# PINTO0309/human-instance-segmentation

Measured on AMD Instinct MI355X. Metric: ROI-masks/sec (fwd) + train step/s, B0 640×480×8-ROI, 1/2/4/8 MI355X, higher is better.
Workload: dtype bf16; 1 GPU; C2: B0 inference 640x480, batch 32/GPU x 8 ROIs/img, ROI 64x48, mask 128x96; global_batch=32, parallelism=dp1 (images sharded, model replicated, no collective), schedule=2-stream pipeline (UNet of step k+1 overlaps head of step k)

## Files before the change

### human-instance-segmentation_amd/csrc/conv_hwc.hip

```cpp
#include "conv_common.h"

namespace hiseg {

#ifndef HISEG_CONV_HWC_MT
#define HISEG_CONV_HWC_MT 3
#endif

typedef unsigned hc_u4 __attribute__((ext_vector_type(4)));
typedef unsigned hc_u2 __attribute__((ext_vector_type(2)));
typedef __attribute__((address_space(3))) void hc_lds_void;

__device__ __forceinline__ void hc_dma16(__amdgpu_buffer_rsrc_t rsrc, unsigned lds_addr, unsigned voff) {
  asm volatile("s_mov_b32 m0, %0\n\ts_nop 0\n\tbuffer_load_dwordx4 %1, %2, 0 offen lds"
               :: "s"(__builtin_amdgcn_readfirstlane(lds_addr)), "v"(voff), "s"(rsrc) : "memory");
}

template <int ACT, bool RES, int NW, bool UP = false, int ABL = 0, bool RP = false, bool ST = false, int TWB = 1,
          bool BR = false, bool R3 = false>
__global__ void __launch_bounds__(NW * 64, NW == 4 ? 2 : 1) conv_hwc_kernel(ConvArgs a) {
  constexpr int NCG = NW / TWB;
  constexpr int BCO = 32 * NCG, TM = 2, NR = 16;
  constexpr int TW = 16 * TWB, HWD = TW + 2;
  constexpr int NHR = 18 * HWD;
  constexpr int PPW = ((NHR + 15) / 16 + NW - 1) / NW;
  constexpr int PH = (ABL & 512) ? PPW : (PPW + 1) / 2;
  constexpr int PROW = (ABL & 1024) ? 0 : 3;
  constexpr int HB = PPW * NW * 1024;
  constexpr int NPX = 256 * TWB;
  static_assert((NW == 4 || NW == 8) && (TWB == 1 || (TWB == 2 && NW == 4 && !RP)), "configuration");
  static_assert(!R3 || (NW == 4 && !RP && TWB == 1 && !ST && !BR), "R3: the plain / residual 128-Cout form");
  constexpr int NPMIN = ((NHR + 15) / 16 - 1 - (NW - 1)) / NW + 1;
  extern __shared__ __attribute__((aligned(16))) uint4 smem[];
  const hiseg_conv2d_desc& d = a.d;
  const int t = threadIdx.x;
  const int lane = t & 63;
  const int w = __builtin_amdgcn_readfirstlane(t >> 6);
  const int wc = w % NCG, pb = w / NCG;

  const int nco = d.Cout_pad / BCO;
  const int ntx = (d.W + TW - 1) / TW, nty = (d.H + 15) >> 4;
  const int nwg = gridDim.x;
  const int orig = blockIdx.x;
  const int q8 = nwg >> 3, r8 = nwg & 7, xcd = orig & 7, loc = orig >> 3;
  const int wg = (xcd < r8 ? xcd * (q8 + 1) : r8 * (q8 + 1) + (xcd - r8) * q8) + loc;
  const int co0 = (wg % nco) * BCO;
  int tl = wg / nco;
  const int tx = tl % ntx;
  tl /= ntx;
  const int ty = tl % nty;
  const int n = tl / nty;
  const int y0 = ty * 16, x0 = tx * TW;

  const unsigned OOB = 0x80000000u;
  const int nsl = a.Cin >> 5;
  const int ncb = a.Cin >> 6;
  const __amdgpu_buffer_rsrc_t rF = __builtin_amdgcn_make_buffer_rsrc(
      const_cast<void*>(d.weight_frag), (short)0, d.Cout_pad * 9 * a.Cin * 2, 0x00020000);
  constexpr int USH = UP ? 1 : 0;
  const __amdgpu_buffer_rsrc_t rA = __builtin_amdgcn_make_buffer_rsrc(
      const_cast<void*>(d.srcA), (short)0, d.N * (d.H >> USH) * (d.W >> USH) * d.a_cstride * 2, 0x00020000);
  const __amdgpu_buffer_rsrc_t rB = __builtin_amdgcn_make_buffer_rsrc(
      const_cast<void*>(d.Cb ? d.srcB : d.srcA), (short)0, d.Cb ? d.N * d.H * d.W * d.b_cstride * 2 : 0, 0x00020000);

  const unsigned a_ct = (unsigned)((co0 + wc * 32) >> 4) * (unsigned)ncb * 18u * 1024u;
  const unsigned a_ct_step = (unsigned)ncb * 18u * 1024u;
  auto load_blk = [&](hc_u4 (&af)[3][TM], int sl, int kx) __attribute__((always_inline)) {
    int ln = lane;
    asm volatile("" : "+v"(ln));
    const unsigned a_lane = a_ct + (unsigned)ln * 16u;
#pragma unroll
    for (int ky = 0; ky < 3; ++ky) {
      const unsigned so = __builtin_amdgcn_readfirstlane(
          (((unsigned)(sl >> 1) * 9u + (unsigned)(ky * 3 + kx)) * 2u + (unsigned)(sl & 1)) * 1024u);
#pragma unroll
      for (int i = 0; i < TM; ++i)
        af[ky][i] = __builtin_amdgcn_raw_buffer_load_b128(rF, a_lane + (unsigned)i * a_ct_step, so, 0);
    }
  };

  const unsigned lds_base = (unsigned)(uintptr_t)(hc_lds_void*)smem;
  auto hbuf = [&](int sl) __attribute__((always_inline)) -> int {
    if constexpr (RP) return ((nsl - 1 - sl) & 1) ? 32 * 1024 : 56 * 1024;
    else if constexpr (R3) return (sl % 3) * HB;
    else return (sl & 1) * HB;
  };
  auto piece_off = [&](int p, int sl) __attribute__((always_inline)) -> unsigned {
    int ln = lane;
    asm volatile("" : "+v"(ln));
    const int hr = 16 * (NW * p + w) + (ln >> 2);
    const int hy = hr / HWD, hx = hr - HWD * hy;
    const int iy = y0 + hy - 1, ix = x0 + hx - 1;
    const bool ok = hr < NHR && (unsigned)iy < (unsigned)d.H && (unsigned)ix < (unsigned)d.W;
    const int chunk = (ln & 3) ^ (((hx >> 2) & 1) << 1);
    const bool fb = 32 * sl >= d.Ca;
    const int cs = fb ? d.b_cstride : d.a_cstride, coff = fb ? d.b_coff + 32 * sl - d.Ca : d.a_coff + 32 * sl;
    if constexpr (UP) {
      const int ush = fb ? 0 : 1;
      return ok ? (unsigned)((((n * (d.H >> ush) + (iy >> ush)) * (d.W >> ush) + (ix >> ush)) * cs + coff + chunk * 8) * 2)
                : OOB;
    } else {
      return ok ? (unsigned)((((n * d.H + iy) * d.W + ix) * cs + coff + chunk * 8) * 2) : OOB;
    }
  };
  unsigned pofA[PPW];
#pragma unroll
  for (int p = 0; p < PPW; ++p) pofA[p] = 16 * (NW * p + w) < NHR ? piece_off(p, 0) : OOB;
  auto halo_dma = [&](int p, int sl, int boff) __attribute__((always_inline)) {
    if (16 * (NW * p + w) >= NHR) return;
    const bool fb = 32 * sl >= d.Ca;
    const unsigned off = fb ? piece_off(p, sl) : pofA[p] + 64u * (unsigned)sl;
    hc_dma16(fb ? rB : rA, lds_base + (unsigned)(boff + 1024 * (NW * p + w)), off);
  };
  const char* lds_c = reinterpret_cast<const char*>(smem);
// ... 81 lines not shown
#pragma unroll
          for (int k = 8 + 3 * KX; k < 11 + 3 * KX; ++k) res_dma(k);
        }
      }
      if constexpr (RP && RES) {
        if (sl == 0) {
#pragma unroll
          for (int k = 3 * KX; k < (KX == 2 ? 8 : 3 * KX + 3); ++k) res_dma(k);
        }
      }
    };
    int ln = lane;
    asm volatile("" : "+v"(ln));
    hc_u4 bq[3];
    if constexpr ((ABL & 4) == 0) {
      bq[0] = rdB(ln, buf, KX, 0);
      bq[1] = rdB(ln, buf, KX, 1);
    } else {
      bq[0] = bq[1] = bq[2] = af[0][0];
    }
    __builtin_amdgcn_s_setprio(1);
#pragma unroll
    for (int r = 0; r < NR + 2; ++r) {
      if (r == PROW) {
        __builtin_amdgcn_s_setprio(0);
        pieces();
        __builtin_amdgcn_s_setprio(1);
      }
      if ((ABL & 4) == 0 && r + 2 < NR + 2) bq[(r + 2) % 3] = rdB(ln, buf, KX, r + 2);
      __builtin_amdgcn_sched_barrier(0);
#pragma unroll
      for (int ky = 0; ky < 3; ++ky) {
        const int j = r - ky;
        if (j >= 0 && j < NR) {
#pragma unroll
          for (int i = 0; i < TM; ++i) {
            if constexpr ((ABL & 16) == 0)
              acc[i][j] = __builtin_amdgcn_mfma_f32_16x16x32_bf16(__builtin_bit_cast(bf16x8_t, af[ky][i]),
                                                                   __builtin_bit_cast(bf16x8_t, bq[r % 3]), acc[i][j], 0,
                                                                   0, 0);
            else
              acc[i][j][0] += __builtin_bit_cast(float, af[ky][i][0]) + __builtin_bit_cast(float, bq[r % 3][1]);
          }
        }
      }
    }
    __builtin_amdgcn_s_setprio(0);
    if constexpr (KX == 2 && (ABL & 8) == 0) {
      if constexpr (R3) {
        if (sl + 2 < nsl) asm volatile("s_waitcnt vmcnt(%0)" :: "n"(18 + NPMIN) : "memory");
        else if (more) asm volatile("s_waitcnt vmcnt(6)" ::: "memory");
        else asm volatile("s_waitcnt vmcnt(0)" ::: "memory");
      } else {
        if (more) asm volatile("s_waitcnt vmcnt(6)" ::: "memory");
        else asm volatile("s_waitcnt vmcnt(0)" ::: "memory");
      }
      __syncthreads();
    }
    if constexpr ((ABL & 1) == 0) {
#pragma unroll
      for (int ky = 0; ky < 3; ++ky)
#pragma unroll
        for (int i = 0; i < TM; ++i) af[ky][i] = an[ky][i];
    }
  };
  using K0 = std::integral_constant<int, 0>;
  using K1 = std::integral_constant<int, 1>;
  using K2 = std::integral_constant<int, 2>;
  for (int sl = 0; sl < nsl; ++sl) {
    block(sl, K0{});
    block(sl, K1{});
    block(sl, K2{});
  }

  if constexpr ((ABL & 32) != 0) {
    float* o = reinterpret_cast<float*>(d.out) + (long long)wg * 64 * 64 * NW + t;
#pragma unroll
    for (int i = 0; i < TM; ++i)
#pragma unroll
      for (int j = 0; j < NR; ++j) o[(i * NR + j) * 64 * NW] = acc[i][j][0] + acc[i][j][1] + acc[i][j][2] + acc[i][j][3];
    return;
  }
  char* tile = reinterpret_cast<char*>(smem);
  if constexpr (RES && !RP) {
#pragma unroll
    for (int k = 0; k < NRI; ++k) res_dma(k);
    asm volatile("s_waitcnt vmcnt(0)" ::: "memory");
    __syncthreads();
  } else if constexpr (RES) {
    res_dma(14);
    res_dma(15);
  }
  constexpr int NSTZ = NPX * CPR / (NW * 64);
  uint4 zpre[BR ? NSTZ : 1];
  if constexpr (BR) {
#pragma unroll
    for (int k = 0; k < NSTZ; ++k) {
      const int idx = t + NW * 64 * k;
      const int r = idx / CPR, c = idx % CPR;
      const int px = px_of(r), co = co0 + 8 * c;
      zpre[k] = (px >= 0 && co < d.Cout)
                    ? *reinterpret_cast<const uint4*>(reinterpret_cast<const uint16_t*>(d.bnb_z) +
                                                      (long long)px * d.bnb_z_cstride + d.bnb_z_coff + co)
                    : make_uint4(0u, 0u, 0u, 0u);
    }
  }
  floatx4 sc[TM], sh[TM];
#pragma unroll
  for (int i = 0; i < TM; ++i) {
    const int cl = wc * 32 + i * 16 + (lane >> 4) * 4;
    const int cc = co0 + cl < d.Cout ? co0 + cl : 0;
    sc[i] = *reinterpret_cast<const floatx4*>(d.scale + cc);
    sh[i] = *reinterpret_cast<const floatx4*>(d.shift + cc);
  }
  auto convert = [&](auto j0c, auto j1c) __attribute__((always_inline)) {
    constexpr int J0 = decltype(j0c)::value, J1 = decltype(j1c)::value;
#pragma unroll
    for (int i = 0; i < TM; ++i)
#pragma unroll
      for (int j = J0; j < J1; ++j) {
        const int cl = wc * 32 + i * 16 + (lane >> 4) * 4;
        const int r = j * TW + 16 * pb + (lane & 15);
        char* q = tile + r * EROWB + ((((cl >> 3) ^ (r & SWM)) << 4) | ((cl & 4) << 1));
        const floatx4 ac = acc[i][j];
        float v[4];
        uint2 rv = make_uint2(0u, 0u);
        if constexpr (RES) rv = *reinterpret_cast<const uint2*>(q);
#pragma unroll
        for (int e = 0; e < 4; ++e) {
          v[e] = ac[e] * sc[i][e] + sh[i][e];
          if constexpr (RES) v[e] += Quad<bf16_t>::get(rv, e);
          if constexpr (ACT == HISEG_ACT_RELU) v[e] = v[e] > 0.f ? v[e] : 0.f;
        }
        uint2 o;
        o.x = f2bf2(v[0], v[1]);
        o.y = f2bf2(v[2], v[3]);
        *reinterpret_cast<uint2*>(q) = o;
      }
  };
  if constexpr (RES && RP) {
    convert(std::integral_constant<int, 0>{}, std::integral_constant<int, 14>{});
    asm volatile("s_waitcnt vmcnt(0)" ::: "memory");
    __syncthreads();
    convert(std::integral_constant<int, 14>{}, std::integral_constant<int, NR>{});
  } else {
    convert(std::integral_constant<int, 0>{}, std::integral_constant<int, NR>{});
  }
  __syncthreads();
  constexpr int NST = NPX * CPR / (NW * 64);
  float sk[8], s1[8], s2[8];
  int sn = 0;
  float bfs[8], bfh[8], bmu[8], binv[8];
  if constexpr (BR) {
    static_assert(!RES && !ST && ACT == HISEG_ACT_NONE && NW == 4 && (CPR == 16 || CPR == 8), "fused BN backward");
    const int cb = co0 + 8 * (t % CPR);
#pragma unroll
    for (int e = 0; e < 8; ++e) {
      const int ch = cb + e < d.Cout ? cb + e : 0;
      bfs[e] = d.bnb_scale[ch];
      bfh[e] = d.bnb_shift[ch];
      bmu[e] = d.bnb_mean[ch];
      binv[e] = d.bnb_invstd[ch];
      sk[e] = s1[e] = s2[e] = 0.f;
    }
  }
  if constexpr (ST) {
    static_assert(!RES && ACT == HISEG_ACT_NONE && NW == 4, "fused statistics: the conv feeding a BatchNorm");
    static_assert(CPR == 16 || CPR == 8, "fused statistics: a wave's threads of one chunk are lanes CPR apart");
#pragma unroll
    for (int e = 0; e < 8; ++e) sk[e] = s1[e] = s2[e] = 0.f;
  }
  uint4 sv[NST];
#pragma unroll
  for (int k = 0; k < NST; ++k) {
    const int idx = t + NW * 64 * k;
    const int r = idx / CPR, c = idx % CPR;
    sv[k] = *reinterpret_cast<const uint4*>(tile + r * EROWB + ((c ^ (r & SWM)) << 4));
  }
  const __amdgpu_buffer_rsrc_t rO = __builtin_amdgcn_make_buffer_rsrc(d.out, (short)0, 0x7fffffff, 0x00020000);
#pragma unroll
  for (int k = 0; k < NST; ++k) {
    const int idx = t + NW * 64 * k;
    const int r = idx / CPR, c = idx % CPR;
    const int px = px_of(r), co = co0 + 8 * c;
    const uint4 v = sv[k];
    __builtin_amdgcn_raw_buffer_store_b128(
        __builtin_bit_cast(hc_u4, v), rO,
        (px >= 0 && co < d.Cout) ? (unsigned)((px * d.o_cstride + d.o_coff + co) * 2) : OOB, 0, 0);
    if constexpr (BR) {
      if (px >= 0 && co < d.Cout) {
        const uint4 zq = zpre[BR ? k : 0];
        const unsigned wv[4] = {v.x, v.y, v.z, v.w}, zw[4] = {zq.x, zq.y, zq.z, zq.w};
#pragma unroll
        for (int e = 0; e < 8; ++e) {
          const float g0 = __builtin_bit_cast(float, (e & 1) ? (wv[e >> 1] & 0xffff0000u) : (wv[e >> 1] << 16));
          const float zf = __builtin_bit_cast(float, (e & 1) ? (zw[e >> 1] & 0xffff0000u) : (zw[e >> 1] << 16));
          const float g = (d.bnb_act == HISEG_ACT_RELU && !(zf * bfs[e] + bfh[e] > 0.f)) ? 0.f : g0;
          const float xh = (zf - bmu[e]) * binv[e];
          sk[e] += g;
          s1[e] = fmaf(g, xh, s1[e]);
          s2[e] += xh;
        }
      }
    }
    if constexpr (ST) {
      if (px >= 0) {
        const unsigned wv[4] = {v.x, v.y, v.z, v.w};
#pragma unroll
        for (int e = 0; e < 8; ++e) {
          const float x = __builtin_bit_cast(float, (e & 1) ? (wv[e >> 1] & 0xffff0000u) : (wv[e >> 1] << 16));
          if (sn == 0) sk[e] = x;
          const float dx = x - sk[e];
          s1[e] += dx;
          s2[e] = fmaf(dx, dx, s2[e]);
        }
        ++sn;
      }
    }
  }
  if constexpr (ST) {
    float nn = (float)sn, mu[8], q2[8];
#pragma unroll
    for (int e = 0; e < 8; ++e) {
      mu[e] = sn ? sk[e] + s1[e] / nn : 0.f;
      q2[e] = sn ? fmaxf(s2[e] - s1[e] * s1[e] / nn, 0.f) : 0.f;
    }
#pragma unroll
    for (int m = CPR; m < 64; m <<= 1) {
      const float nb = __shfl_xor(nn, m, 64);
      const float nt = nn + nb;
      const float fb = nt > 0.f ? nb / nt : 0.f, fab = nt > 0.f ? nn * nb / nt : 0.f;
#pragma unroll
      for (int e = 0; e < 8; ++e) {
        const float mb = __shfl_xor(mu[e], m, 64), qb = __shfl_xor(q2[e], m, 64);
        const float dd = mb - mu[e];
        mu[e] += dd * fb;
        q2[e] += qb + dd * dd * fab;
      }
      nn = nt;
    }
    if (lane < CPR) {
      const long long C = d.Cout;
      float* part = a.d.stats_partial + ((long long)((n * nty + ty) * ntx + tx) * NW + w) * 3 * C;
#pragma unroll
      for (int e = 0; e < 8; ++e) {
        const int ch = co0 + 8 * lane + e;
        part[ch] = nn;
        part[C + ch] = mu[e];
        part[2 * C + ch] = q2[e];
      }
    }
  }
  if constexpr (BR) {
#pragma unroll
    for (int m = CPR; m < 64; m <<= 1) {
#pragma unroll
      for (int e = 0; e < 8; ++e) {
        sk[e] += __shfl_xor(sk[e], m, 64);
        s1[e] += __shfl_xor(s1[e], m, 64);
        s2[e] += __shfl_xor(s2[e], m, 64);
      }
    }
    if (lane < CPR) {
      const long long C = d.Cout;
      float* part = a.d.bnb_partial + ((long long)((n * nty + ty) * ntx + tx) * NW + w) * 3 * C;
#pragma unroll
      for (int e = 0; e < 8; ++e) {
        const int ch = co0 + 8 * lane + e;
        if (ch < C) {
          part[ch] = sk[e];
          part[C + ch] = s1[e];
          part[2 * C + ch] = s2[e];
        }
      }
    }
  }
}

template <int ACT, bool RES, int NW, bool UP = false, int ABL = 0, bool RP = false, bool ST = false, int TWB = 1,
          bool BR = false, bool R3 = false>
static int launch_hwc(const ConvArgs& a, hipStream_t s) {
  const hiseg_conv2d_desc& d = a.d;
  constexpr int BCO = 32 * NW / TWB, TW = 16 * TWB;
  constexpr int PPW = ((18 * (TW + 2) + 15) / 16 + NW - 1) / NW;
  constexpr size_t halo2 = (size_t)2 * PPW * NW * 1024, epi = (size_t)256 * TWB * BCO * 2;
  const int tiles = d.N * ((d.H + 15) / 16) * ((d.W + TW - 1) / TW);
  const int nco = d.Cout_pad / BCO;
  const size_t halo = R3 ? halo2 / 2 * 3 : halo2;
  const size_t lds = RP ? (size_t)80 * 1024 : (halo > epi ? halo : epi);
  auto kern = conv_hwc_kernel<ACT, RES, NW, UP, ABL, RP, ST, TWB, BR, R3>;
  static bool attr = false;
  if (!attr) {
    (void)hipFuncSetAttribute((const void*)kern, hipFuncAttributeMaxDynamicSharedMemorySize, (int)lds);
    attr = true;
  }
  hipLaunchKernelGGL(kern, dim3(tiles * nco), dim3(NW * 64), lds, s, a);
  return hiseg_check_launch("conv_hwc");
}

template <int ACT, bool RES, int TWB, int MT>
__global__ void __launch_bounds__(256, 2) conv_hwc_mt_kernel(ConvArgs a) {
  constexpr int NW = 4, NCG = NW / TWB;
  constexpr int BCO = 32 * NCG, TM = 2, NR = 16;
  constexpr int TW = 16 * TWB, HWD = TW + 2;
  constexpr int NHR = 18 * HWD;
  constexpr int PPW = ((NHR + 15) / 16 + NW - 1) / NW;
  constexpr int PH = (PPW + 1) / 2;
  constexpr int HB = PPW * NW * 1024;
  constexpr int NPX = 256 * TWB, HALF = NPX / 2;
  constexpr int EOFF = HB;
  static_assert(MT >= 2 && (TWB == 1 || TWB == 2), "multi-tile configuration");
  extern __shared__ __attribute__((aligned(16))) uint4 smem[];
  const hiseg_conv2d_desc& d = a.d;
  const int t = threadIdx.x;
  const int lane = t & 63;
  const int w = __builtin_amdgcn_readfirstlane(t >> 6);
  const int wc = w % NCG, pb = w / NCG;

  const int nco = d.Cout_pad / BCO;
  const int ntx = (d.W + TW - 1) / TW, nty = (d.H + 15) >> 4;
  const int total = d.N * nty * ntx * nco;
  const int G = gridDim.x;
  const int orig = blockIdx.x;
  const int q8 = G >> 3, r8 = G & 7, xcd = orig & 7, loc = orig >> 3;
  const int wg = (xcd < r8 ? xcd * (q8 + 1) : r8 * (q8 + 1) + (xcd - r8) * q8) + loc;

  const unsigned OOB = 0x80000000u;
  const int nsl = a.Cin >> 5;
  const int ncb = a.Cin >> 6;
  const __amdgpu_buffer_rsrc_t rF = __builtin_amdgcn_make_buffer_rsrc(
      const_cast<void*>(d.weight_frag), (short)0, d.Cout_pad * 9 * a.Cin * 2, 0x00020000);
  const __amdgpu_buffer_rsrc_t rA = __builtin_amdgcn_make_buffer_rsrc(
      const_cast<void*>(d.srcA), (short)0, d.N * d.H * d.W * d.a_cstride * 2, 0x00020000);
  const __amdgpu_buffer_rsrc_t rB = __builtin_amdgcn_make_buffer_rsrc(
      const_cast<void*>(d.Cb ? d.srcB : d.srcA), (short)0, d.Cb ? d.N * d.H * d.W * d.b_cstride * 2 : 0, 0x00020000);
  const unsigned a_ct_step = (unsigned)ncb * 18u * 1024u;

  struct Geo { int co0, n, y0, x0; unsigned a_ct; };
  auto geo = [&](int i) __attribute__((always_inline)) -> Geo {
    Geo g;
    g.co0 = (i % nco) * BCO;
    int tl = i / nco;
    g.x0 = (tl % ntx) * TW;
    tl /= ntx;
    g.y0 = (tl % nty) * 16;
    g.n = tl / nty;
    g.a_ct = (unsigned)((g.co0 + wc * 32) >> 4) * (unsigned)ncb * 18u * 1024u;
    return g;
  };
  auto load_blk = [&](hc_u4 (&af)[3][TM], unsigned a_ct, int sl, int kx) __attribute__((always_inline)) {
    int ln = lane;
    asm volatile("" : "+v"(ln));
    const unsigned a_lane = a_ct + (unsigned)ln * 16u;
#pragma unroll
    for (int ky = 0; ky < 3; ++ky) {
      const unsigned so = __builtin_amdgcn_readfirstlane(
          (((unsigned)(sl >> 1) * 9u + (unsigned)(ky * 3 + kx)) * 2u + (unsigned)(sl & 1)) * 1024u);
#pragma unroll
      for (int i = 0; i < TM; ++i)
        af[ky][i] = __builtin_amdgcn_raw_buffer_load_b128(rF, a_lane + (unsigned)i * a_ct_step, so, 0);
    }
  };
  auto piece_off = [&](const Geo& g, int p, int sl) __attribute__((always_inline)) -> unsigned {
    int ln = lane;
    asm volatile("" : "+v"(ln));
    const int hr = 16 * (NW * p + w) + (ln >> 2);
    const int hy = hr / HWD, hx = hr - HWD * hy;
    const int iy = g.y0 + hy - 1, ix = g.x0 + hx - 1;
    const bool ok = hr < NHR && (unsigned)iy < (unsigned)d.H && (unsigned)ix < (unsigned)d.W;
    const int chunk = (ln & 3) ^ (((hx >> 2) & 1) << 1);
    const bool fb = 32 * sl >= d.Ca;
    const int cs = fb ? d.b_cstride : d.a_cstride, coff = fb ? d.b_coff + 32 * sl - d.Ca : d.a_coff + 32 * sl;
    return ok ? (unsigned)((((g.n * d.H + iy) * d.W + ix) * cs + coff + chunk * 8) * 2) : OOB;
// ... 203 lines not shown
#pragma unroll
    for (int i = 0; i < TM; ++i)
#pragma unroll
      for (int j = 0; j < NR; ++j) acc[i][j] = floatx4{0.f, 0.f, 0.f, 0.f};
  }
}

template <int ACT, bool RES, int TWB, int MT>
static int launch_hwc_mt(const ConvArgs& a, hipStream_t s) {
  const hiseg_conv2d_desc& d = a.d;
  constexpr int BCO = 128 / TWB, TW = 16 * TWB;
  constexpr int PPW = ((18 * (TW + 2) + 15) / 16 + 3) / 4;
  constexpr size_t hb = (size_t)PPW * 4 * 1024;
  constexpr size_t lds = 2 * hb > hb + 32 * 1024 ? 2 * hb : hb + 32 * 1024;
  const long long items = (long long)d.N * ((d.H + 15) / 16) * ((d.W + TW - 1) / TW) * (d.Cout_pad / BCO);
  const int grid = (int)((items + MT - 1) / MT);
  auto kern = conv_hwc_mt_kernel<ACT, RES, TWB, MT>;
  static bool attr = false;
  if (!attr) {
    (void)hipFuncSetAttribute((const void*)kern, hipFuncAttributeMaxDynamicSharedMemorySize, (int)lds);
    attr = true;
  }
  hipLaunchKernelGGL(kern, dim3(grid), dim3(256), lds, s, a);
  return hiseg_check_launch("conv_hwc_mt");
}

template <int TWB, int MT>
static int launch_hwc_mt_act(const ConvArgs& a, hipStream_t s) {
  const bool res = a.d.residual != nullptr, relu = a.d.act == HISEG_ACT_RELU;
  return res ? (relu ? launch_hwc_mt<HISEG_ACT_RELU, true, TWB, MT>(a, s) : launch_hwc_mt<HISEG_ACT_NONE, true, TWB, MT>(a, s))
             : (relu ? launch_hwc_mt<HISEG_ACT_RELU, false, TWB, MT>(a, s)
                     : launch_hwc_mt<HISEG_ACT_NONE, false, TWB, MT>(a, s));
}

template <int NW, bool RP = false, int TWB = 1, bool R3 = false>
static int launch_hwc_nw(const ConvArgs& a, hipStream_t s) {
  const hiseg_conv2d_desc& d = a.d;
  if (d.a_up == 2)
    return launch_hwc<HISEG_ACT_RELU, false, NW, true, 0, false, false, TWB, false, R3>(a, s);
  const bool res = d.residual != nullptr, relu = d.act == HISEG_ACT_RELU;
  return res ? (relu ? launch_hwc<HISEG_ACT_RELU, true, NW, false, 0, RP, false, TWB, false, R3>(a, s)
                     : launch_hwc<HISEG_ACT_NONE, true, NW, false, 0, RP, false, TWB, false, R3>(a, s))
             : (relu ? launch_hwc<HISEG_ACT_RELU, false, NW, false, 0, false, false, TWB, false, R3>(a, s)
                     : launch_hwc<HISEG_ACT_NONE, false, NW, false, 0, false, false, TWB, false, R3>(a, s));
}

static bool conv_hwc_applies(const ConvArgs& a, int variant) {
  const hiseg_conv2d_desc& d = a.d;
  if (((variant < 104 || variant > 109) && variant != 102) || d.weight_frag == nullptr) return false;
  if ((variant == 109 || variant == 102) && (d.a_up != 1 || d.stats_partial || d.bnb_partial)) return false;
  if (d.dtype != HISEG_BF16 || d.out_dtype != HISEG_BF16) return false;
  if ((d.a_up != 1 && d.a_up != 2) || d.in_scale != nullptr || d.convT || d.mul != nullptr || d.out2 != nullptr)
    return false;
  if (d.KH != 3 || d.KW != 3 || d.stride != 1 || d.pad != 1 || d.Ho != d.H || d.Wo != d.W) return false;
  if (d.act != HISEG_ACT_NONE && d.act != HISEG_ACT_RELU) return false;
  if (d.Ca % 32 != 0 || d.Cb % 32 != 0 || (d.Ca + d.Cb) % 64 != 0 || d.Ca < 64 || d.K_pad != 9 * (d.Ca + d.Cb))
    return false;
  if ((d.a_cstride | d.a_coff) & 7) return false;
  if (d.Cb && (d.srcB == nullptr || ((d.b_cstride | d.b_coff) & 7))) return false;
  if ((d.Cout & (variant == 105 ? 255 : (variant == 107 || variant == 102) ? 63 : 127)) || d.Cout_pad != d.Cout ||
      ((d.o_cstride | d.o_coff) & 7) ||
      (d.residual && ((d.r_cstride | d.r_coff) & 7)))
    return false;
  if ((((uintptr_t)d.scale | (uintptr_t)d.shift | (uintptr_t)d.out | (uintptr_t)d.residual |
        (uintptr_t)d.weight_frag) & 15))
    return false;
  const long long span_a = (long long)d.N * (d.H / d.a_up) * (d.W / d.a_up) * d.a_cstride * 2;
  const long long span_b = d.Cb ? (long long)d.N * d.H * d.W * d.b_cstride * 2 : 0;
  const long long span_w = (long long)d.Cout_pad * d.K_pad * 2;
  const long long span_r = d.residual ? (long long)a.M * d.r_cstride * 2 : 0;
  const long long span_o = (long long)a.M * d.o_cstride * 2;
  if (span_a >= 0x7fffffffll || span_b >= 0x7fffffffll || span_w >= 0x7fffffffll || span_r >= 0x7fffffffll ||
      span_o >= 0x7fffffffll)
    return false;
  if ((long long)d.N * d.H * d.W >= (1ll << 29)) return false;
  if (d.a_up == 2 && (d.residual || d.act != (d.stats_partial ? HISEG_ACT_NONE : HISEG_ACT_RELU))) return false;
  if (d.stats_partial && ((variant != 104 && variant != 107) || d.residual || d.act != HISEG_ACT_NONE)) return false;
  if (d.bnb_partial &&
      ((variant != 104 && variant != 107) || d.residual || d.act != HISEG_ACT_NONE || d.stats_partial || d.a_up != 1 ||
       d.bnb_z == nullptr || ((d.bnb_z_cstride | d.bnb_z_coff) & 7) || ((uintptr_t)d.bnb_z & 15) ||
       !d.bnb_scale || !d.bnb_shift || !d.bnb_mean || !d.bnb_invstd ||
       (d.bnb_act != HISEG_ACT_RELU && d.bnb_act != HISEG_ACT_NONE)))
    return false;
  return true;
}

int conv_hwc_stats_tiles(const ConvArgs& a) {
  ConvArgs b = a;
  float dummy;
  if (b.d.bnb_partial == nullptr) b.d.stats_partial = &dummy;
  const int tw = conv_hwc_applies(b, 104) ? 16 : conv_hwc_applies(b, 107) ? 32 : 0;
  if (tw == 0) return 0;
  return a.d.N * ((a.d.H + 15) / 16) * ((a.d.W + tw - 1) / tw) * 4;
}

int conv_hwc_try(const ConvArgs& a, hipStream_t s, int variant) {
  const hiseg_conv2d_desc& d = a.d;
#ifdef HISEG_DIAG
  if (variant >= 150 && variant < 4300) {
    if (d.weight_frag == nullptr || !d.residual || d.act != HISEG_ACT_RELU || d.a_up != 1 || d.Cout % 128) return 0;
    int r;
    switch (variant - 150) {
      case 1: r = launch_hwc<HISEG_ACT_RELU, true, 4, false, 1>(a, s); break;
      case 2: r = launch_hwc<HISEG_ACT_RELU, true, 4, false, 2>(a, s); break;
      case 3: r = launch_hwc<HISEG_ACT_RELU, true, 4, false, 3>(a, s); break;
      case 4: r = launch_hwc<HISEG_ACT_RELU, true, 4, false, 4>(a, s); break;
      case 8: r = launch_hwc<HISEG_ACT_RELU, true, 4, false, 8>(a, s); break;
      case 15: r = launch_hwc<HISEG_ACT_RELU, true, 4, false, 15>(a, s); break;
      case 16: r = launch_hwc<HISEG_ACT_RELU, true, 4, false, 16>(a, s); break;
      case 32: r = launch_hwc<HISEG_ACT_RELU, true, 4, false, 32>(a, s); break;
      case 47: r = launch_hwc<HISEG_ACT_RELU, true, 4, false, 47>(a, s); break;
      case 64: r = launch_hwc<HISEG_ACT_RELU, true, 4, false, 64>(a, s); break;
      case 128: r = launch_hwc<HISEG_ACT_RELU, true, 4, false, 128>(a, s); break;
      case 512: r = launch_hwc<HISEG_ACT_RELU, true, 4, false, 512>(a, s); break;
      case 1024: r = launch_hwc<HISEG_ACT_RELU, true, 4, false, 1024>(a, s); break;
      case 1536: r = launch_hwc<HISEG_ACT_RELU, true, 4, false, 1536>(a, s); break;
      case 2048: r = launch_hwc<HISEG_ACT_RELU, true, 4, false, 2048>(a, s); break;
      case 4096: r = launch_hwc<HISEG_ACT_RELU, true, 4, false, 4096>(a, s); break;
      default: return 0;
    }
    return r < 0 ? r : 1;
  }
#endif
  if (!conv_hwc_applies(a, variant)) return 0;
  if (d.bnb_partial) {
    const int r = variant == 107 ? launch_hwc<HISEG_ACT_NONE, false, 4, false, 0, false, false, 2, true>(a, s)
                                 : launch_hwc<HISEG_ACT_NONE, false, 4, false, 0, false, false, 1, true>(a, s);
    return r < 0 ? r : 1;
  }
  if (d.stats_partial) {
    int r;
    if (variant == 107)
      r = d.a_up == 2 ? launch_hwc<HISEG_ACT_NONE, false, 4, true, 0, false, true, 2>(a, s)
                      : launch_hwc<HISEG_ACT_NONE, false, 4, false, 0, false, true, 2>(a, s);
    else
      r = d.a_up == 2 ? launch_hwc<HISEG_ACT_NONE, false, 4, true, 0, false, true>(a, s)
                      : launch_hwc<HISEG_ACT_NONE, false, 4, false, 0, false, true>(a, s);
    return r < 0 ? r : 1;
  }
  const int r = variant == 109 ? launch_hwc_mt_act<1, HISEG_CONV_HWC_MT>(a, s)
              : variant == 102 ? launch_hwc_mt_act<2, HISEG_CONV_HWC_MT>(a, s)
              : variant == 107 ? launch_hwc_nw<4, false, 2>(a, s)
              : variant == 108 ? launch_hwc_nw<4, false, 1, true>(a, s)
              : variant == 105 ? launch_hwc_nw<8>(a, s)
              : variant == 106 ? launch_hwc_nw<4, true>(a, s)
                               : launch_hwc_nw<4>(a, s);
  return r < 0 ? r : 1;
}

}
```

### human-instance-segmentation_amd/csrc/conv_igemm.hip

```cpp
#include <cstdlib>
#include "conv_common.h"

namespace hiseg {

typedef unsigned ig_u4 __attribute__((ext_vector_type(4)));

template <typename T, typename TO, int BCO, int BPX, int WCO, int WPX, bool SPLIT = false, int LIN = 0>
__global__ void __launch_bounds__(256) conv_igemm_kernel(ConvArgs a) {
  constexpr int KCH = Chunk<T>::N;
  constexpr int BK = 8 * KCH;
  constexpr int TM = BCO / (WCO * 16);
  constexpr int TN = BPX / (WPX * 16);
  constexpr int A_CH = (BPX * 8 + 255) / 256;
  constexpr int W_CH = (BCO * 8 + 255) / 256;
  constexpr int STAGE = (BCO + BPX) * 8;
  constexpr bool A_FULL = (BPX * 8) % 256 == 0;
  constexpr bool W_FULL = (BCO * 8) % 256 == 0;
  static_assert(WCO * WPX == 4, "4 waves");
  static_assert(TM >= 1 && TN >= 1, "tile");

  extern __shared__ __attribute__((aligned(16))) uint4 smem[];

  const hiseg_conv2d_desc& d = a.d;
  const int t = threadIdx.x;
// ... 325 lines not shown
        if (r) return r;
        const long long n = (long long)a.M * (a.d.Cout_pad >> 2);
        hipLaunchKernelGGL((conv_splitk_reduce_kernel<T, TO>), dim3((unsigned)((n + 255) / 256)), dim3(256), 0, s, a, splits);
        return hiseg_check_launch("conv_splitk_reduce");
      }
      if (lin == 1) hipLaunchKernelGGL((conv_igemm_kernel<T, TO, BCO, BPX, WCO, WPX, false, 1>), grid, dim3(256), lds, s, a);
      else hipLaunchKernelGGL((conv_igemm_kernel<T, TO, BCO, BPX, WCO, WPX, false, 2>), grid, dim3(256), lds, s, a);
      return hiseg_check_launch("conv_igemm");
    }
  }
  if (splits > 1) {
    hipLaunchKernelGGL((conv_igemm_kernel<T, TO, BCO, BPX, WCO, WPX, true>), grid, dim3(256), lds, s, a);
    const int r = hiseg_check_launch("conv_igemm_splitk");
    if (r) return r;
    const long long n = (long long)a.M * (a.d.Cout_pad >> 2);
    hipLaunchKernelGGL((conv_splitk_reduce_kernel<T, TO>), dim3((unsigned)((n + 255) / 256)), dim3(256), 0, s, a, splits);
    return hiseg_check_launch("conv_splitk_reduce");
  }
  hipLaunchKernelGGL((conv_igemm_kernel<T, TO, BCO, BPX, WCO, WPX>), grid, dim3(256), lds, s, a);
  return hiseg_check_launch("conv_igemm");
}

static int igemm_bco(int cp) {
  auto fits = [&](int bco) { return ((cp + bco - 1) / bco) * bco * 6 <= cp * 7; };
  auto padded = [&](int bco) { return ((cp + bco - 1) / bco) * bco; };
  if (cp >= 96 && fits(128)) return 128;
  if (cp >= 48 && fits(64)) return 64;
  if (cp >= 48) return padded(64) < padded(128) ? 64 : 128;
  if (fits(32)) return 32;
  return 16;
}

static int splitk_bco(int cp) { return cp >= 96 && igemm_bco(cp) == 128 ? 128 : 64; }

template <typename T, typename TO>
static int launch_typed(const ConvArgs& a, hipStream_t s, int splits = 1) {
  static const bool gated_wide = [] { const char* e = getenv("HISEG_GATED_WIDE"); return !(e && atoi(e) == 0); }();
  if (splits > 1 || (gated_wide && a.d.in_scale != nullptr)) {
    if (splitk_bco(a.d.Cout_pad) == 128) return launch_cfg<T, TO, 128, 128, 2, 2>(a, s, splits);
    return launch_cfg<T, TO, 64, 128, 2, 2>(a, s, splits);
  }
  const char* eb = getenv("HISEG_IGEMM_BCO");
  switch (eb ? atoi(eb) : igemm_bco(a.d.Cout_pad)) {
    case 128: return launch_cfg<T, TO, 128, 128, 2, 2>(a, s, splits);
    case 64: return launch_cfg<T, TO, 64, 128, 2, 2>(a, s, splits);
    case 32: return launch_cfg<T, TO, 32, 256, 1, 4>(a, s, splits);
    default: return launch_cfg<T, TO, 16, 256, 1, 4>(a, s, splits);
  }
}

static int splitk_plan(const ConvArgs& a) {
  const hiseg_conv2d_desc& d = a.d;
  if (d.dtype != HISEG_BF16 || d.convT || a.nK < 6) return 1;
  if (d.KH == 3 && d.KW == 3 && d.stride == 1 && d.a_up == 1 && (long long)d.Ho * d.Wo <= 256 && a.nK >= 24 &&
      d.in_scale == nullptr) {
    int sp = a.nK / 4;
    return sp > 8 ? 8 : sp;
  }
  if (d.KH != 1 || d.KW != 1) return 1;
  if (d.in_scale == nullptr && a.nK < 24) return 1;
  static const int forced = [] { const char* e = getenv("HISEG_SPLITK"); return e ? atoi(e) : 0; }();
  if (forced > 0) return forced < a.nK ? forced : a.nK;
  if ((long long)d.Ho * d.Wo > 1600) return 1;
  int sp = a.nK / 4;
  if (sp > 8) sp = 8;
  return sp >= 2 ? sp : 2;
}

static long long splitk_bytes(const ConvArgs& a, int splits) {
  return splits > 1 ? (long long)splits * a.M * a.d.Cout_pad * 4 : 0;
}

}

namespace hiseg {
int conv_fast_try(const ConvArgs& a, hipStream_t s, int variant);
int conv_wide_try(const ConvArgs& a, hipStream_t s, int variant);
int conv_hw_try(const ConvArgs& a, hipStream_t s, int variant);
int conv_pw_try(const ConvArgs& a, hipStream_t s, int variant);
int conv_hwr_try(const ConvArgs& a, hipStream_t s, int variant);
int conv_hwt_try(const ConvArgs& a, hipStream_t s, int variant);
int conv_hwc_try(const ConvArgs& a, hipStream_t s, int variant);
int conv_hwc_stats_tiles(const ConvArgs& a);
int conv_small_try(const ConvArgs& a, hipStream_t s, int variant);
int conv_rows_try(const ConvArgs& a, hipStream_t s, int variant);
bool conv_pw_applies(const ConvArgs& a);
int conv_pw_gate_images(const ConvArgs& a);
bool conv_rows_form(const ConvArgs& a);
}

using namespace hiseg;


static int conv2d_impl(const hiseg_conv2d_desc* d, hiseg_stream_t stream, int variant);

extern "C" int hiseg_conv2d_fwd(const hiseg_conv2d_desc* d, hiseg_stream_t stream) {
  return conv2d_impl(d, stream, 0);
}

static bool hwc64_mode() {
  const char* e = getenv("HISEG_CONV_HWC64");
  return !(e && atoi(e) == 0);
}

static bool hwc_r3_mode() {
  const char* e = getenv("HISEG_CONV_HWC_R3");
  return !(e && atoi(e) == 0);
}

#ifndef HISEG_CONV_HWC_MT_DEFAULT
#define HISEG_CONV_HWC_MT_DEFAULT(bco) false
#endif
static bool hwc_mt_mode(int bco) {
  const char* e = getenv("HISEG_CONV_HWC_MTW");
  if (e) return atoi(e) != 0;
  return HISEG_CONV_HWC_MT_DEFAULT(bco);
}

static bool release_variant(int v) {
  return v == -1 || v == 0 || (v >= 1 && v <= 8) || v == 50 || v == 51 || v == 52 || v == 54 || v == 58 ||
         (v >= 60 && v <= 69) || v == 70 || v == 71 || v == 72 || v == 74 || v == 80 || v == 82 || v == 84 || v == 86 ||
         v == 88 || v == 89 || v == 90 || (v >= 92 && v <= 101) || v == 103 || v == 102 || (v >= 104 && v <= 109);
}

extern "C" long long hiseg_conv2d_workspace_bytes(const hiseg_conv2d_desc* d) {
  if (d == nullptr || d->dtype != HISEG_BF16 || d->convT || d->N <= 0) return 0;
  const long long M = (long long)d->N * d->Ho * d->Wo;
  if (M >= (1ll << 31) || d->K_pad % 64) return 0;
  ConvArgs a;
  a.d = *d;
  a.M = (int)M;
  a.Cin = d->Ca + d->Cb;
  a.nK = d->K_pad / 64;
  a.Hs = d->H / (d->a_up > 0 ? d->a_up : 1);
  a.Ws = d->W / (d->a_up > 0 ? d->a_up : 1);
  if (conv_pw_applies(a)) return 0;
  if (d->in_scale && d->KH == 1 && d->KW == 1 && conv_pw_gate_images(a) > 0) return 0;
  return splitk_bytes(a, splitk_plan(a));
}

extern "C" int hiseg_conv2d_stats_tiles(const hiseg_conv2d_desc* d) {
  if (d == nullptr || d->dtype != HISEG_BF16 || d->convT || d->N <= 0) return 0;
  const long long M = (long long)d->N * d->Ho * d->Wo;
  if (M >= (1ll << 31)) return 0;
  ConvArgs a;
  a.d = *d;
  a.M = (int)M;
  a.Cin = d->Ca + d->Cb;
  a.nK = d->K_pad / 64;
  a.Hs = d->H / (d->a_up > 0 ? d->a_up : 1);
  a.Ws = d->W / (d->a_up > 0 ? d->a_up : 1);
  return conv_hwc_stats_tiles(a);
}

extern "C" int hiseg_conv2d_fwd_variant(const hiseg_conv2d_desc* d, int variant, hiseg_stream_t stream) {
#ifndef HISEG_DIAG
  HISEG_REQUIRE(release_variant(variant), HISEG_ERR_BAD_ARG,
                "conv2d: variant %d is not a release variant (diagnostic kernels need a DIAG=1 build)", variant);
#endif
  return conv2d_impl(d, stream, variant);
}

static int conv2d_impl(const hiseg_conv2d_desc* d, hiseg_stream_t stream, int variant) {
  HISEG_REQUIRE(d != nullptr, HISEG_ERR_BAD_ARG, "conv2d: null descriptor");
  HISEG_REQUIRE(d->dtype == HISEG_F32 || d->dtype == HISEG_BF16, HISEG_ERR_BAD_DTYPE, "conv2d: dtype %d", d->dtype);
  HISEG_REQUIRE(d->out_dtype == HISEG_F32 || d->out_dtype == HISEG_BF16, HISEG_ERR_BAD_DTYPE, "conv2d: out_dtype %d", d->out_dtype);
  HISEG_REQUIRE(d->srcA && d->weight && d->scale && d->shift && d->out, HISEG_ERR_BAD_ARG, "conv2d: null pointer");
  HISEG_REQUIRE(d->N > 0 && d->H > 0 && d->W > 0 && d->Ho > 0 && d->Wo > 0, HISEG_ERR_BAD_SHAPE, "conv2d: empty grid");
  HISEG_REQUIRE(d->KH > 0 && d->KW > 0 && d->stride > 0 && d->pad >= 0, HISEG_ERR_BAD_SHAPE, "conv2d: bad window");
  HISEG_REQUIRE(d->a_up == 1 || d->a_up == 2, HISEG_ERR_BAD_SHAPE, "conv2d: a_up must be 1 or 2");
  HISEG_REQUIRE(d->a_up == 1 || (d->H % 2 == 0 && d->W % 2 == 0), HISEG_ERR_BAD_SHAPE, "conv2d: upsampled grid must be even");
  HISEG_REQUIRE(d->Cb == 0 || d->srcB, HISEG_ERR_BAD_ARG, "conv2d: Cb > 0 needs srcB");
  HISEG_REQUIRE(d->Cout > 0 && d->Cout_pad >= d->Cout && d->Cout_pad % 16 == 0, HISEG_ERR_BAD_SHAPE,
                "conv2d: Cout %d Cout_pad %d (must be multiple of 16)", d->Cout, d->Cout_pad);
  const int kch = d->dtype == HISEG_BF16 ? 8 : 4;
  const int bk = 8 * kch;
  const int Cin = d->Ca + d->Cb;
  HISEG_REQUIRE(d->Ca > 0 && d->Ca % kch == 0 && d->Cb % kch == 0 && d->a_cstride % kch == 0 &&
                    d->a_coff % kch == 0 && (d->Cb == 0 || (d->b_cstride % kch == 0 && d->b_coff % kch == 0)),
                HISEG_ERR_BAD_SHAPE, "conv2d: input channels/strides must be multiples of %d", kch);
  HISEG_REQUIRE(d->K_pad % bk == 0 && d->K_pad >= d->KH * d->KW * Cin, HISEG_ERR_BAD_SHAPE,
                "conv2d: K_pad %d must be a multiple of %d and >= %d", d->K_pad, bk, d->KH * d->KW * Cin);
  HISEG_REQUIRE(al16(d->srcA) && al16(d->srcB) && al16(d->weight), HISEG_ERR_BAD_SHAPE, "conv2d: operands must be 16-B aligned");
  HISEG_REQUIRE(!d->convT || (d->KH == 1 && d->KW == 1 && d->stride == 1 && d->pad == 0 && d->Cout % 16 == 0 &&
                              d->Ho == d->H && d->Wo == d->W),
                HISEG_ERR_BAD_SHAPE, "conv2d: convT requires a 1x1 GEMM with Cout = 4*C, C %% 4 == 0");
  if (d->stats_partial || d->bnb_partial) {
    HISEG_REQUIRE(variant == 0 || variant == 104 || variant == 107, HISEG_ERR_BAD_ARG,
                  "conv2d: stats_partial / bnb_partial with variant %d", variant);
    HISEG_REQUIRE(al16(d->out) && al16(d->scale) && al16(d->shift), HISEG_ERR_BAD_SHAPE, "conv2d: alignment");
    ConvArgs a;
    a.d = *d;
    a.M = (int)((long long)d->N * d->Ho * d->Wo);
    a.Cin = Cin;
    a.nK = d->K_pad / bk;
    a.Hs = d->H / d->a_up;
    a.Ws = d->W / d->a_up;
    HISEG_REQUIRE(conv_hwc_stats_tiles(a) > 0, HISEG_ERR_BAD_ARG,
                  "conv2d: stats_partial / bnb_partial set but the layer has no fused kernel (hiseg_conv2d_stats_tiles)");
    const int r = conv_hwc_try(a, (hipStream_t)stream, d->Cout % 128 == 0 ? 104 : 107);
    HISEG_REQUIRE(r != 0, HISEG_ERR_BAD_ARG, "conv2d: the fused-statistics kernel declined the layer");
    return r < 0 ? r : HISEG_OK;
  }
  {
    const long long ea = d->dtype == HISEG_BF16 ? 2 : 4, eo = d->out_dtype == HISEG_BF16 ? 2 : 4;
    const long long in_px = (long long)(d->H / d->a_up) * (d->W / d->a_up);
    const long long out_px = (long long)d->Ho * d->Wo * (d->convT ? 4 : 1);
    long long per = in_px * d->a_cstride * ea;
    auto upd = [&](long long v) { if (v > per) per = v; };
    if (d->srcB) upd((long long)d->H * d->W * d->b_cstride * ea);
    if (d->residual) upd(out_px * d->r_cstride * ea);
    if (d->mul) upd(out_px * d->m_cstride * ea);
    upd(out_px * d->o_cstride * eo);
    if (d->out2) upd(out_px * d->o2_cstride * ea);
    const long long lim = (1ll << 31) - (1ll << 20);
    int step = 0;
    if (per * d->N > lim) {
      HISEG_REQUIRE(per <= lim, HISEG_ERR_BAD_SHAPE, "conv2d: one image's operand exceeds 2 GiB");
      step = (int)(lim / per);
    }
    if (variant == 0 && d->in_scale && d->dtype == HISEG_BF16 && d->KH == 1 && d->KW == 1) {
      ConvArgs ga;
      ga.d = *d;
      ga.M = (int)((long long)d->N * d->Ho * d->Wo < (1ll << 31) ? (long long)d->N * d->Ho * d->Wo : 0);
      ga.Cin = d->Ca + d->Cb;
      ga.nK = d->K_pad / (8 * kch);
      ga.Hs = d->H / d->a_up;
      ga.Ws = d->W / d->a_up;
      const int g = conv_pw_gate_images(ga);
      if (g > 0 && (step == 0 || g < step)) step = g;
    }
    if (step > 0 && step < d->N) {
      for (int n0 = 0; n0 < d->N; n0 += step) {
        hiseg_conv2d_desc c = *d;
        c.N = d->N - n0 < step ? d->N - n0 : step;
        auto at = [&](const void* p, long long bytes_per_image) {
          return p ? (const void*)((const char*)p + bytes_per_image * n0) : p;
        };
        c.srcA = at(d->srcA, in_px * d->a_cstride * ea);
        c.srcB = at(d->srcB, (long long)d->H * d->W * d->b_cstride * ea);
        c.residual = at(d->residual, out_px * d->r_cstride * ea);
        c.mul = at(d->mul, out_px * d->m_cstride * ea);
        c.out = const_cast<void*>(at(d->out, out_px * d->o_cstride * eo));
        c.out2 = const_cast<void*>(at(d->out2, out_px * d->o2_cstride * ea));
        if (d->in_scale) c.in_scale = d->in_scale + (long long)n0 * d->Ca;
        const int r = conv2d_impl(&c, stream, variant);
        if (r) return r;
      }
      return HISEG_OK;
    }
  }
  const long long M = (long long)d->N * d->Ho * d->Wo;
  HISEG_REQUIRE(M < (1ll << 31), HISEG_ERR_BAD_SHAPE, "conv2d: too many pixels");
  ConvArgs a;
  a.d = *d;
  a.M = (int)M;
  a.Cin = Cin;
  a.nK = d->K_pad / bk;
  a.Hs = d->H / d->a_up;
  a.Ws = d->W / d->a_up;
  hipStream_t s = (hipStream_t)stream;
  a.ins_vec = d->in_scale != nullptr && ((uintptr_t)d->in_scale & 15) == 0 && (d->Ca & 3) == 0;
  a.ws = static_cast<float*>(d->workspace);
  a.kper = a.nK;
  if (variant == 99 || variant == 0) {
    const int sp = splitk_plan(a);
    if (sp > 1 && d->workspace != nullptr && d->workspace_bytes >= splitk_bytes(a, sp) &&
        !(variant == 0 && conv_pw_applies(a))) {
      a.kper = (a.nK + sp - 1) / sp;
      const int spl = (a.nK + a.kper - 1) / a.kper;
      return d->out_dtype == HISEG_BF16 ? launch_typed<bf16_t, bf16_t>(a, s, spl) : launch_typed<bf16_t, float>(a, s, spl);
    }
    HISEG_REQUIRE(variant == 0, HISEG_ERR_BAD_ARG, "conv2d: variant 99 (split-K) does not apply to this layer / workspace");
  }
  if (variant == 98) {
    const int r = conv_rows_try(a, s, variant);
    if (r != 0) return r < 0 ? r : HISEG_OK;
  } else if (variant == 90 || (variant >= 190 && variant < 222)) {
    const int r = conv_pw_try(a, s, variant);
    if (r != 0) return r < 0 ? r : HISEG_OK;
  } else if ((variant >= 92 && variant <= 97) || variant == 100 || variant == 101 || (variant >= 110 && variant < 142)) {
    const int r = conv_hwr_try(a, s, variant);
    if (r != 0) return r < 0 ? r : HISEG_OK;
  } else if (variant == 102 || (variant >= 104 && variant <= 109) || (variant >= 150 && variant < 4300)) {
    const int r = conv_hwc_try(a, s, variant);
    if (r != 0) return r < 0 ? r : HISEG_OK;
  } else if (variant == 103) {
    const int r = conv_hwt_try(a, s, variant);
    if (r != 0) return r < 0 ? r : HISEG_OK;
  } else if (variant >= 80 && variant < 90) {
    const int r = conv_hw_try(a, s, variant);
    if (r != 0) return r < 0 ? r : HISEG_OK;
  } else if (variant >= 70 && variant < 80) {
    const int r = conv_wide_try(a, s, variant);
    if (r != 0) return r < 0 ? r : HISEG_OK;
  } else if (variant >= 60 && variant < 70) {
    const int r = conv_fast_try(a, s, variant);
    if (r != 0) return r < 0 ? r : HISEG_OK;
  } else if (variant >= 50) {
    const int r = conv_small_try(a, s, variant);
    if (r != 0) return r < 0 ? r : HISEG_OK;
  } else if (variant >= 0) {
    int v = variant;
    static const bool four_waves = [] { const char* e = getenv("HISEG_CONV_WAVES"); return e && atoi(e) == 4; }();
    static const bool halo = [] { const char* e = getenv("HISEG_CONV_HALO"); return !(e && atoi(e) == 0); }();
    if (v == 0 && d->KH == 1 && d->KW == 1) {
      const int r = conv_pw_try(a, s, 90);
      if (r != 0) return r < 0 ? r : HISEG_OK;
    }
    if (v == 0 && d->KH == 3 && d->KW == 3 && d->Cout_pad <= 32) {
      const int r = conv_rows_try(a, s, 98);
      if (r != 0) return r < 0 ? r : HISEG_OK;
      if (conv_rows_form(a)) {
        const int r2 = conv_small_try(a, s, 0);
        if (r2 != 0) return r2 < 0 ? r2 : HISEG_OK;
      }
    }
    if (v == 0 && !four_waves && halo && d->weight_frag != nullptr && d->Cout % 128 == 0 && hwc_mt_mode(128)) {
      const int r = conv_hwc_try(a, s, 109);
      if (r != 0) return r < 0 ? r : HISEG_OK;
    }
    if (v == 0 && !four_waves && halo && d->weight_frag != nullptr && d->Cout % 128 == 0) {
      const int r = conv_hwc_try(a, s, hwc_r3_mode() ? 108 : 104);
      if (r != 0) return r < 0 ? r : HISEG_OK;
    }
    if (v == 0 && !four_waves && halo && d->weight_frag != nullptr && d->Cout % 128 == 0) {
      const int r = conv_hwr_try(a, s, 97);
      if (r != 0) return r < 0 ? r : HISEG_OK;
    }
    if (v == 0 && !four_waves && halo && d->weight_frag != nullptr && d->Cout % 64 == 0 && hwc64_mode() &&
        hwc_mt_mode(64)) {
      const int r = conv_hwc_try(a, s, 102);
      if (r != 0) return r < 0 ? r : HISEG_OK;
    }
    if (v == 0 && !four_waves && halo && d->weight_frag != nullptr && d->Cout % 64 == 0 && hwc64_mode()) {
      const int r = conv_hwc_try(a, s, 107);
      if (r != 0) return r < 0 ? r : HISEG_OK;
    }
    if (v == 0 && !four_waves && halo && d->weight_frag != nullptr && d->Cout % 64 == 0) {
      const int r = conv_hwr_try(a, s, 100);
      if (r != 0) return r < 0 ? r : HISEG_OK;
    }
    if (v == 0 && !four_waves && halo) {
      const int r = conv_hw_try(a, s, d->Cout % 128 ? 89 : 86);
      if (r != 0) return r < 0 ? r : HISEG_OK;
    }
    if (v == 0 && d->Cout % 256 == 0 && d->KH * d->KW > 1 && !four_waves) {
// ... 17 lines not shown
```

### human-instance-segmentation_amd/csrc/conv_pw.hip

```cpp
#include "conv_common.h"

#ifndef HISEG_PW_PART
#define HISEG_PW_PART 1
#endif

namespace hiseg {

constexpr int kPwBlk = 32;
constexpr int kPwActRt = -1;

typedef unsigned pw_u4 __attribute__((ext_vector_type(4)));
typedef unsigned pw_u2 __attribute__((ext_vector_type(2)));

template <int NKSA, int EPI, int ACT, bool CONVT, int RB, bool INS>
__global__ void __launch_bounds__(256, 1) conv_pw_kernel(ConvArgs a, int nct, int nks_arg) {
  constexpr int NKS = NKSA < 0 ? -NKSA : NKSA;
  const int nks = NKSA < 0 ? nks_arg : NKSA;
  constexpr bool RES = EPI == 1, MUL = EPI == 2, XOP = EPI != 0;
  constexpr int CT = 16 * RB;
  constexpr int ROWC = NKS * 4 + 1;
  constexpr int NA = NKS == 9 ? 8 : NKS;
  constexpr unsigned OOB = 0x80000000u;
  extern __shared__ __attribute__((aligned(16))) uint4 smem[];
  const hiseg_conv2d_desc& d = a.d;
  const int t = threadIdx.x, lane = t & 63, w = t >> 6;
  const int ct = blockIdx.x % nct;
  const int grp = blockIdx.x / nct, ngrp = gridDim.x / nct;
  const int c0 = ct * CT;
  const int act = ACT == kPwActRt ? d.act : ACT;
#ifdef HISEG_DIAG
  const int abl = a.abl;
#else
  constexpr int abl = 0;
#endif

  uint4* wl = smem;
  float* ssc = reinterpret_cast<float*>(smem + CT * ROWC);
  float* ssh = ssc + CT;
  float* gl = ssh + CT;
  constexpr int kPwStage = 8;
  const int kc = d.K_pad >> 3;
  const int wch = nks * 4;
  const int nchunk = CT * wch;
  {
    const __amdgpu_buffer_rsrc_t rW = __builtin_amdgcn_make_buffer_rsrc(
        const_cast<void*>(d.weight), (short)0, (int)((long long)d.Cout_pad * kc * 16), 0x00020000);
    for (int i0 = t; i0 < ((abl & 1) ? 0 : nchunk); i0 += 256 * kPwStage) {
      pw_u4 v[kPwStage];
#pragma unroll
      for (int u = 0; u < kPwStage; ++u) {
        const int i = i0 + 256 * u;
        const int r = i / wch, c = i - r * wch;
        const unsigned off = i < nchunk ? (unsigned)(((c0 + r) * kc + c) * 16) : 0x80000000u;
        v[u] = __builtin_amdgcn_raw_buffer_load_b128(rW, off, 0, 0);
      }
#pragma unroll
      for (int u = 0; u < kPwStage; ++u) {
        const int i = i0 + 256 * u;
        const int r = i / wch, c = i - r * wch;
        if (i < nchunk) wl[r * ROWC + c] = make_uint4(v[u].x, v[u].y, v[u].z, v[u].w);
      }
    }
  }
  for (int i = t; i < CT; i += 256) {
    const int j = c0 + i < d.Cout ? c0 + i : 0;
    ssc[i] = d.scale[j];
    ssh[i] = d.shift[j];
  }
  if constexpr (INS) {
    const int n4 = d.N * d.Ca / 4;
    const __amdgpu_buffer_rsrc_t rG = __builtin_amdgcn_make_buffer_rsrc(
        const_cast<float*>(d.in_scale), (short)0, (int)(n4 * 16), 0x00020000);
    float4* gl4 = reinterpret_cast<float4*>(gl);
    for (int i0 = t; i0 < n4; i0 += 256 * kPwStage) {
      pw_u4 v[kPwStage];
#pragma unroll
      for (int u = 0; u < kPwStage; ++u) {
        const int i = i0 + 256 * u;
        v[u] = __builtin_amdgcn_raw_buffer_load_b128(rG, i < n4 ? (unsigned)(i * 16) : 0x80000000u, 0, 0);
      }
#pragma unroll
      for (int u = 0; u < kPwStage; ++u) {
        const int i = i0 + 256 * u;
        if (i < n4) gl4[i] = __builtin_bit_cast(float4, v[u]);
      }
    }
  }
  __syncthreads();

  const int M = a.M;
  const int nblk = (M + kPwBlk - 1) / kPwBlk;
  const int g = lane >> 4, pl = lane & 15;
  const long long out_px = (long long)M * (CONVT ? 4 : 1);
  const __amdgpu_buffer_rsrc_t rA = __builtin_amdgcn_make_buffer_rsrc(
      const_cast<void*>(d.srcA), (short)0, (int)((long long)M * d.a_cstride * 2), 0x00020000);
  const __amdgpu_buffer_rsrc_t rB = __builtin_amdgcn_make_buffer_rsrc(
      const_cast<void*>(NKS == 9 ? d.srcB : d.srcA), (short)0, NKS == 9 ? (int)((long long)M * d.b_cstride * 2) : 0,
      0x00020000);
  const __amdgpu_buffer_rsrc_t rO = __builtin_amdgcn_make_buffer_rsrc(d.out, (short)0,
                                                                     (int)(out_px * d.o_cstride * 2), 0x00020000);
  const void* xp = RES ? d.residual : MUL ? d.mul : d.out;
  const int x_cs = RES ? d.r_cstride : d.m_cstride, x_coff = RES ? d.r_coff : d.m_coff;
  const __amdgpu_buffer_rsrc_t rR = __builtin_amdgcn_make_buffer_rsrc(
      const_cast<void*>(xp), (short)0, XOP ? (int)(out_px * x_cs * 2) : 0, 0x00020000);
  const bool bch_ok = NKS == 9 && 8 * g < d.Cb;

  auto load_ks = [&](int b, int ks, uint4 (&bk)[2]) __attribute__((always_inline)) {
    if (abl & 2) {
      bk[0] = bk[1] = make_uint4(0u, 0u, 0u, 0u);
      return;
    }
    const bool ch_ok = 32 * ks + 8 * g < d.Ca;
#pragma unroll
    for (int j = 0; j < 2; ++j) {
      const int p = b * kPwBlk + 16 * j + pl;
      pw_u4 v;
      if (ks < NA) {
        const unsigned off = (p < M && ch_ok) ? (unsigned)((p * d.a_cstride + d.a_coff + 32 * ks + 8 * g) * 2) : OOB;
        v = __builtin_amdgcn_raw_buffer_load_b128(rA, off, 0, 0);
      } else {
        const unsigned off = (p < M && bch_ok) ? (unsigned)((p * d.b_cstride + d.b_coff + 8 * g) * 2) : OOB;
        v = __builtin_amdgcn_raw_buffer_load_b128(rB, off, 0, 0);
      }
      bk[j] = make_uint4(v.x, v.y, v.z, v.w);
    }
  };

  int pbase[2];
  auto set_block = [&](int b) __attribute__((always_inline)) {
#pragma unroll
    for (int j = 0; j < 2; ++j) {
      const int p = b * kPwBlk + 16 * j + pl;
      if constexpr (CONVT) {
        const int x = p % d.Wo, tt = p / d.Wo, y = tt % d.Ho, n = tt / d.Ho;
        pbase[j] = p < M ? (n * (2 * d.Ho) + 2 * y) * (2 * d.Wo) + 2 * x : -1;
      } else {
        pbase[j] = p < M ? p : -1;
      }
    }
  };
  auto offset = [&](int j, int i, int cs, int coff) __attribute__((always_inline)) -> unsigned {
    const int col = c0 + 16 * i + 4 * g;
    if (pbase[j] < 0 || col >= d.Cout) return OOB;
    if constexpr (CONVT) {
      const int C = d.Cout >> 2, q = col / C, co = col - q * C;
      const int op = pbase[j] + (q >> 1) * (2 * d.Wo) + (q & 1);
      return (unsigned)((op * cs + coff + co) * 2);
    } else {
      return (unsigned)((pbase[j] * cs + coff + col) * 2);
    }
  };
  const int hw = d.H * d.W;

  const int stride = ngrp * 4;
  int b = grp * 4 + w;
  uint4 b0[NKS][2], b1[NKS][2];
#pragma unroll
  for (int ks = 0; ks < NKS; ++ks)
    if (ks < nks) load_ks(b, ks, b0[ks]);
  auto process = [&](int b, uint4 (&bf)[NKS][2], uint4 (&bn)[NKS][2]) __attribute__((always_inline)) {
    const int nb = b + stride;
    if constexpr (INS) {
      int gofs[2];
#pragma unroll
      for (int j = 0; j < 2; ++j) {
        const int p = b * kPwBlk + 16 * j + pl;
        const int n = p < M ? p / hw : 0;
        gofs[j] = n * d.Ca;
      }
#pragma unroll
      for (int ks = 0; ks < NKS; ++ks) {
        if (ks >= nks) continue;
        const int ch = 32 * ks + 8 * g < d.Ca ? 32 * ks + 8 * g : d.Ca - 8;
#pragma unroll
        for (int j = 0; j < 2; ++j) {
          const float4* gp = reinterpret_cast<const float4*>(gl + gofs[j] + ch);
          const float4 s0 = gp[0], s1 = gp[1];
          float f[8];
          Chunk<bf16_t>::unpack(bf[ks][j], f);
          f[0] *= s0.x; f[1] *= s0.y; f[2] *= s0.z; f[3] *= s0.w;
          f[4] *= s1.x; f[5] *= s1.y; f[6] *= s1.z; f[7] *= s1.w;
          bf[ks][j] = Chunk<bf16_t>::pack(f);
        }
      }
    }
#pragma unroll
    for (int ks = 0; ks < NKS; ++ks)
      if (ks < nks) load_ks(nb, ks, bn[ks]);
    set_block(b);
    pw_u2 rv[XOP ? RB : 1][2];
    if constexpr (XOP) {
#pragma unroll
      for (int i = 0; i < RB; ++i)
#pragma unroll
        for (int j = 0; j < 2; ++j) rv[i][j] = __builtin_amdgcn_raw_buffer_load_b64(rR, offset(j, i, x_cs, x_coff), 0, 0);
    }
    int wofs = pl * ROWC + g;
    asm volatile("" : "+v"(wofs));
    const uint4* wrow = smem + wofs;
    floatx4 acc[RB][2];
#pragma unroll
    for (int i = 0; i < RB; ++i) acc[i][0] = acc[i][1] = floatx4{0.f, 0.f, 0.f, 0.f};
#pragma unroll
    for (int ks = 0; ks < NKS; ++ks) {
      if (ks >= nks) continue;
#pragma unroll
      for (int i = 0; i < RB; ++i) {
        if (abl & 4) continue;
        const uint4 af = wrow[16 * i * ROWC + 4 * ks];
        acc[i][0] = __builtin_amdgcn_mfma_f32_16x16x32_bf16(__builtin_bit_cast(bf16x8_t, af),
                                                            __builtin_bit_cast(bf16x8_t, bf[ks][0]), acc[i][0], 0, 0, 0);
        acc[i][1] = __builtin_amdgcn_mfma_f32_16x16x32_bf16(__builtin_bit_cast(bf16x8_t, af),
                                                            __builtin_bit_cast(bf16x8_t, bf[ks][1]), acc[i][1], 0, 0, 0);
      }
    }
#pragma unroll
    for (int i = 0; i < RB; ++i) {
      const int cl = 16 * i + 4 * g;
      const floatx4 sc = *reinterpret_cast<const floatx4*>(ssc + cl);
      const floatx4 sh = *reinterpret_cast<const floatx4*>(ssh + cl);
#pragma unroll
      for (int j = 0; j < 2; ++j) {
        float v[4];
#pragma unroll
        for (int e = 0; e < 4; ++e) {
          if (abl & 8) {
            v[e] = acc[i][j][e];
            continue;
          }
          v[e] = acc[i][j][e] * sc[e] + sh[e];
          if constexpr (RES) v[e] += Quad<bf16_t>::get(make_uint2(rv[i][j].x, rv[i][j].y), e);
          v[e] = apply_act(v[e], act);
          if constexpr (MUL) v[e] *= Quad<bf16_t>::get(make_uint2(rv[i][j].x, rv[i][j].y), e);
        }
        pw_u2 q;
        q.x = f2bf2(v[0], v[1]);
        q.y = f2bf2(v[2], v[3]);
        if (!(abl & 16)) __builtin_amdgcn_raw_buffer_store_b64(q, rO, offset(j, i, d.o_cstride, d.o_coff), 0, 0);
      }
    }
  };
  for (; b < nblk; b += 2 * stride) {
    process(b, b0, b1);
    if (b + stride >= nblk) break;
    process(b + stride, b1, b0);
  }
}

static int cu_count() {
  static int n = 0;
  if (!n) {
    int dev = 0;
    (void)hipGetDevice(&dev);
    if (hipDeviceGetAttribute(&n, hipDeviceAttributeMultiprocessorCount, dev) != hipSuccess || n <= 0) n = 256;
  }
  return n;
}

static size_t pw_lds_bytes(int NKS, int RB, bool ins, const hiseg_conv2d_desc& d) {
  return (size_t)16 * RB * (NKS * 4 + 1) * 16 + 2 * 16 * RB * 4 + (ins ? (size_t)d.N * d.Ca * 4 : 0);
}

template <int NKSA, int EPI, int ACT, bool CONVT, int RB, bool INS>
static int launch_pw(const ConvArgs& a, hipStream_t s, int nks) {
  const hiseg_conv2d_desc& d = a.d;
  const size_t lds = pw_lds_bytes(NKSA < 0 ? -NKSA : NKSA, RB, INS, d);
  auto kern = conv_pw_kernel<NKSA, EPI, ACT, CONVT, RB, INS>;
  static int occ = 0;
  static size_t occ_lds = 0;
  if (lds > occ_lds) {
    (void)hipFuncSetAttribute((const void*)kern, hipFuncAttributeMaxDynamicSharedMemorySize, 160 * 1024);
    int nb = 0;
    if (hipOccupancyMaxActiveBlocksPerMultiprocessor(&nb, (const void*)kern, 256, lds) != hipSuccess || nb < 1) nb = 1;
    occ = nb > 4 ? 4 : nb;
    occ_lds = lds;
  }
  const int nct = (d.Cout_pad + 16 * RB - 1) / (16 * RB);
  const int nblk = (a.M + kPwBlk - 1) / kPwBlk;
  int groups = cu_count() * occ / nct;
  const int need = (nblk + 3) / 4;
  if (groups > need) groups = need;
  if (groups < 1) groups = 1;
  hipLaunchKernelGGL(kern, dim3(groups * nct), dim3(256), lds, s, a, nct, nks);
  return hiseg_check_launch("conv_pw");
}

int launch_pw_narrow(const ConvArgs& a, hipStream_t s, int rb, int nks_max, int nks);

#if HISEG_PW_PART == 2
template <int RB, int NKS>
static int launch_pw_n2(const ConvArgs& a, hipStream_t s, int nks) {
  const hiseg_conv2d_desc& d = a.d;
  constexpr int N = HISEG_ACT_NONE, R = HISEG_ACT_RELU, SI = HISEG_ACT_SILU, RT = kPwActRt;
  const bool ins = d.in_scale != nullptr;
  const int act = d.act;
  if (ins) {
    if (d.residual) return act == N ? launch_pw<-NKS, 1, N, false, RB, true>(a, s, nks)
                                    : launch_pw<-NKS, 1, RT, false, RB, true>(a, s, nks);
    return act == N ? launch_pw<-NKS, 0, N, false, RB, true>(a, s, nks)
                    : launch_pw<-NKS, 0, RT, false, RB, true>(a, s, nks);
  }
  if (d.residual) return act == N ? launch_pw<-NKS, 1, N, false, RB, false>(a, s, nks)
                       : act == R ? launch_pw<-NKS, 1, R, false, RB, false>(a, s, nks)
                                  : launch_pw<-NKS, 1, RT, false, RB, false>(a, s, nks);
  return act == N ? launch_pw<-NKS, 0, N, false, RB, false>(a, s, nks)
       : act == R ? launch_pw<-NKS, 0, R, false, RB, false>(a, s, nks)
       : act == SI ? launch_pw<-NKS, 0, SI, false, RB, false>(a, s, nks)
                   : launch_pw<-NKS, 0, RT, false, RB, false>(a, s, nks);
}
template <int RB>
static int launch_pw_n1(const ConvArgs& a, hipStream_t s, int nks_max, int nks) {
  if (nks_max == 2) return launch_pw_n2<RB, 2>(a, s, nks);
  if (nks_max == 4) return launch_pw_n2<RB, 4>(a, s, nks);
  if constexpr (RB <= 4) {
    if (nks_max == 10) return launch_pw_n2<RB, 10>(a, s, nks);
  }
  return launch_pw_n2<RB, 8>(a, s, nks);
}
int launch_pw_narrow(const ConvArgs& a, hipStream_t s, int rb, int nks_max, int nks) {
  switch (rb) {
    case 1: return launch_pw_n1<1>(a, s, nks_max, nks);
    case 2: return launch_pw_n1<2>(a, s, nks_max, nks);
    case 4: return launch_pw_n1<4>(a, s, nks_max, nks);
    default: return launch_pw_n1<8>(a, s, nks_max, nks);
  }
}
#else
template <int NKS>
static int launch_pw_k(const ConvArgs& a, hipStream_t s, int nks) {
  const hiseg_conv2d_desc& d = a.d;
  constexpr int N = HISEG_ACT_NONE, R = HISEG_ACT_RELU, S = HISEG_ACT_SIGMOID, SI = HISEG_ACT_SILU;
  const int act = d.act;
  if constexpr (NKS == 9) {
    return act == R ? launch_pw<NKS, 0, R, false, 16, false>(a, s, nks) : launch_pw<NKS, 0, N, false, 16, false>(a, s, nks);
  } else {
    if (nks != NKS) {
      HISEG_REQUIRE(!(d.convT || d.residual || d.mul), HISEG_ERR_BAD_ARG,
                    "conv_pw: residual / mul / ConvTranspose forms need 2, 4 or 8 k-steps (pw_plan declines them)");
      return act == R ? launch_pw<-NKS, 0, R, false, 16, false>(a, s, nks)
           : act == S ? launch_pw<-NKS, 0, S, false, 16, false>(a, s, nks)
           : act == SI ? launch_pw<-NKS, 0, SI, false, 16, false>(a, s, nks)
                       : launch_pw<-NKS, 0, N, false, 16, false>(a, s, nks);
    }
    if (d.convT) return act == R ? launch_pw<NKS, 0, R, true, 16, false>(a, s, nks)
                                 : launch_pw<NKS, 0, N, true, 16, false>(a, s, nks);
    if (d.residual) return act == R ? launch_pw<NKS, 1, R, false, 16, false>(a, s, nks)
                                    : launch_pw<NKS, 1, N, false, 16, false>(a, s, nks);
    if (d.mul) return act == S ? launch_pw<NKS, 2, S, false, 16, false>(a, s, nks)
                               : launch_pw<NKS, 2, N, false, 16, false>(a, s, nks);
    return act == R ? launch_pw<NKS, 0, R, false, 16, false>(a, s, nks)
         : act == S ? launch_pw<NKS, 0, S, false, 16, false>(a, s, nks)
         : act == SI ? launch_pw<NKS, 0, SI, false, 16, false>(a, s, nks)
                     : launch_pw<NKS, 0, N, false, 16, false>(a, s, nks);
  }
}

static constexpr long long kPwGateBytes = 64 * 1024;
static bool pw_plan(const ConvArgs& a, int& rb, int& nks, int& nks_max) {
  const hiseg_conv2d_desc& d = a.d;
  if (d.dtype != HISEG_BF16 || d.out_dtype != HISEG_BF16) return false;
  if (d.KH != 1 || d.KW != 1 || d.stride != 1 || d.pad != 0 || d.a_up != 1) return false;
  if (d.out2) return false;
  if (d.residual && d.mul) return false;
  if (d.Ca % 8 || d.Cb % 8 || d.Cout % 4) return false;
  if (d.convT && (d.Cout / 4) % 4) return false;
  if (d.convT && d.residual) return false;
  nks = (a.Cin + 31) / 32;
  if (d.K_pad < nks * 32 || nks > 10) return false;
  static const bool eff = [] { const char* e = getenv("HISEG_PW_EFF"); return !(e && atoi(e) == 0); }();
  if (!eff && (d.Cout_pad % 256 || d.Ca % 32 || d.in_scale || (nks != 4 && nks != 8 && nks != 9))) return false;
  rb = 16;
  if (d.Cout_pad <= 128) rb = d.Cout_pad <= 16 ? 1 : d.Cout_pad <= 32 ? 2 : d.Cout_pad <= 64 ? 4 : 8;
  {
    static const int force_rb = [] { const char* e = getenv("HISEG_PW_RB"); return e ? atoi(e) : 0; }();
    const bool narrow_ok = !d.convT && !d.mul && d.act != HISEG_ACT_SWISH && d.Cb == 0;
    if (rb == 16 && narrow_ok) {
      int want = force_rb ? force_rb : (a.M <= 131072 ? 4 : 16);
      if (want != 1 && want != 2 && want != 4 && want != 8) want = 16;
      if (!(want > 4 && nks > 8)) rb = want;
    }
  }
  const bool comb = rb == 16 && nks == 9;
  if ((rb == 16 && nks > 9) || (rb > 4 && nks > 8)) return false;
  if (comb ? (d.Ca != 256 || d.Cb > 32 || d.convT || d.residual || d.mul || d.in_scale ||
              (d.act != HISEG_ACT_NONE && d.act != HISEG_ACT_RELU))
           : d.Cb != 0)
    return false;
  if (rb == 16) {
    if (d.in_scale) return false;
    if (d.act == HISEG_ACT_SIGMOID ? (d.convT || d.residual)
                                   : (d.act != HISEG_ACT_NONE && d.act != HISEG_ACT_RELU &&
                                      !(d.act == HISEG_ACT_SILU && !d.convT && !d.residual && !d.mul)))
      return false;
    if (d.mul && (d.act == HISEG_ACT_RELU || d.convT || ((d.m_cstride | d.m_coff) & 3))) return false;
  } else {
    if (d.convT || d.mul || d.act == HISEG_ACT_SWISH) return false;
    if (d.in_scale && (((uintptr_t)d.in_scale & 15) || (long long)d.N * d.Ca * 4 > kPwGateBytes)) return false;
  }
  const long long out_px = (long long)a.M * (d.convT ? 4 : 1);
  const long long lim = 0x7fffffffll;
  if ((long long)a.M * d.a_cstride * 2 >= lim || (d.Cb && (long long)a.M * d.b_cstride * 2 >= lim) ||
      out_px * d.o_cstride * 2 >= lim || (d.residual && out_px * d.r_cstride * 2 >= lim) ||
      (d.mul && out_px * d.m_cstride * 2 >= lim))
    return false;
  if ((d.a_cstride | d.a_coff) & 7) return false;
  if (d.Cb && ((d.b_cstride | d.b_coff) & 7)) return false;
  if (((d.o_cstride | d.o_coff) & 3) || (d.residual && ((d.r_cstride | d.r_coff) & 3))) return false;
  if (((uintptr_t)d.out | (uintptr_t)d.residual | (uintptr_t)d.mul) & 7) return false;
  nks_max = comb ? 9 : nks <= 2 ? 2 : nks <= 4 ? 4 : nks <= 8 ? 8 : 10;
  if (rb == 16 && !comb && nks != nks_max && (d.convT || d.residual || d.mul)) return false;
  return true;
}

bool conv_pw_applies(const ConvArgs& a) {
  int rb, nks, nks_max;
  return pw_plan(a, rb, nks, nks_max);
}

int conv_pw_gate_images(const ConvArgs& a) {
  const hiseg_conv2d_desc& d = a.d;
  if (!d.in_scale || d.Ca <= 0 || (long long)d.N * d.Ca * 4 <= kPwGateBytes) return 0;
  const int per = (int)(kPwGateBytes / (4ll * d.Ca));
  if (per < 1) return 0;
  ConvArgs one = a;
  one.d.N = per;
  one.M = per * d.Ho * d.Wo;
  int rb, nks, nks_max;
  return pw_plan(one, rb, nks, nks_max) ? per : 0;
}

int conv_pw_try(const ConvArgs& a0, hipStream_t s, int variant) {
#ifdef HISEG_DIAG
  const bool diag = variant >= 190 && variant < 222;
#else
  const bool diag = false;
#endif
  if (variant != 90 && !diag) return 0;
  ConvArgs a = a0;
  a.abl = diag ? variant - 190 : 0;
  int rb, nks, nks_max;
  if (!pw_plan(a, rb, nks, nks_max)) return 0;
  int r;
  if (rb < 16) {
    r = launch_pw_narrow(a, s, rb, nks_max, nks);
  } else {
    switch (nks_max) {
      case 2: r = launch_pw_k<2>(a, s, nks); break;
      case 4: r = launch_pw_k<4>(a, s, nks); break;
      case 8: r = launch_pw_k<8>(a, s, nks); break;
      default: r = launch_pw_k<9>(a, s, nks); break;
    }
  }
  return r < 0 ? r : 1;
}
#endif

}
```

### human-instance-segmentation_amd/csrc/misc.hip

```cpp
#include <float.h>
#include "common.h"

namespace hiseg {

static inline unsigned nblocks(long long n, int bs) { return (unsigned)((n + bs - 1) / bs); }

template <typename T>
__global__ void __launch_bounds__(256) maxpool2x2_kernel(const void* in, int N, int H, int W, int C, void* out) {
  constexpr int K = Chunk<T>::N;
  const int nch = C / K;
  const int Ho = H / 2, Wo = W / 2;
  const long long gid = (long long)blockIdx.x * 256 + threadIdx.x;
  const long long total = (long long)N * Ho * Wo * nch;
  if (gid >= total) return;
  const int ch = (int)(gid % nch);
  long long p = gid / nch;
  const int x = (int)(p % Wo); p /= Wo;
  const int y = (int)(p % Ho);
  const int n = (int)(p / Ho);
  const uint4* src = reinterpret_cast<const uint4*>(in);
  float m[K], v[K];
  for (int e = 0; e < K; ++e) m[e] = -FLT_MAX;
#pragma unroll
  for (int dy = 0; dy < 2; ++dy)
#pragma unroll
    for (int dx = 0; dx < 2; ++dx) {
      const long long pix = ((long long)n * H + 2 * y + dy) * W + 2 * x + dx;
      Chunk<T>::unpack(src[pix * nch + ch], v);
#pragma unroll
      for (int e = 0; e < K; ++e) m[e] = fmaxf(m[e], v[e]);
    }
  reinterpret_cast<uint4*>(out)[gid] = Chunk<T>::pack(m);
}

template <typename T>
__global__ void __launch_bounds__(256) attn_stats_kernel(const void* x, long long P, int C, float* stats) {
  constexpr int K = Chunk<T>::N;
  constexpr int G = 16;
  const int nch = C / K;
  const long long gid = (long long)blockIdx.x * 256 + threadIdx.x;
  const long long pix = gid / G;
  const int l = (int)(gid % G);
  float s = 0.f, m = -FLT_MAX, v[K];
  if (pix < P) {
    const uint4* src = reinterpret_cast<const uint4*>(x) + pix * nch;
    for (int ch = l; ch < nch; ch += G) {
      Chunk<T>::unpack(src[ch], v);
#pragma unroll
      for (int e = 0; e < K; ++e) { s += v[e]; m = fmaxf(m, v[e]); }
    }
  }
#pragma unroll
  for (int off = G / 2; off > 0; off >>= 1) {
    s += __shfl_xor(s, off, G);
    m = fmaxf(m, __shfl_xor(m, off, G));
  }
  if (pix < P && l == 0) {
    stats[pix * 2] = s / (float)C;
    stats[pix * 2 + 1] = m;
  }
}

__global__ void __launch_bounds__(256) attn_map_kernel(const float* stats, int N, int H, int W, const float* w, int k,
                                                       float* att) {
  const long long gid = (long long)blockIdx.x * 256 + threadIdx.x;
  const long long total = (long long)N * H * W;
  if (gid >= total) return;
  const int x = (int)(gid % W);
  const long long t = gid / W;
  const int y = (int)(t % H);
  const int n = (int)(t / H);
  const int r = k / 2;
  float acc = 0.f;
  for (int c = 0; c < 2; ++c)
    for (int ky = 0; ky < k; ++ky) {
      const int yy = y + ky - r;
      if (yy < 0 || yy >= H) continue;
      for (int kx = 0; kx < k; ++kx) {
        const int xx = x + kx - r;
        if (xx < 0 || xx >= W) continue;
        acc += w[(c * k + ky) * k + kx] * stats[(((long long)n * H + yy) * W + xx) * 2 + c];
      }
    }
  att[gid] = sigmoidf_(acc);
// ... 649 lines not shown
  (void)nq;
  if (gap == nullptr) return;
  __syncthreads();
  float* red = reinterpret_cast<float*>(dws);
#pragma unroll
  for (int e = 0; e < CP; ++e) red[t * CP + e] = gs[e];
  __syncthreads();
  if (it == 0 && live) {
    for (int r = 1; r < NG; ++r)
#pragma unroll
      for (int e = 0; e < CP; ++e) gs[e] += red[(r * NQ + qd) * CP + e];
    float* gp = gap + ((long long)n * gridDim.x + bt) * C + c;
#pragma unroll
    for (int e = 0; e < CP; ++e) gp[e] = gs[e];
  }
}

static int dw_quads_per_block(int nq) {
  int best = nq < 256 ? nq : 256, best_fill = 0;
  for (int d = 1; d <= 16; ++d) {
    const int ct = (nq + d - 1) / d;
    if (ct > 256) continue;
    const int fill = (256 / ct) * ct;
    if (fill > best_fill) { best = ct; best_fill = fill; }
    if (fill >= 230) return ct;
  }
  return best;
}

__device__ __forceinline__ unsigned ord_enc(float f) {
  const unsigned u = __float_as_uint(f);
  return (u & 0x80000000u) ? ~u : (u | 0x80000000u);
}
__device__ __forceinline__ float ord_dec(unsigned e) {
  return __uint_as_float((e & 0x80000000u) ? (e & 0x7fffffffu) : ~e);
}

__global__ void reset_max_kernel(unsigned* buf) { *buf = 0u; }

__global__ void __launch_bounds__(256) image_max_kernel(const float* x, long long n, unsigned* buf) {
  float m = -FLT_MAX;
  const long long gid = (long long)blockIdx.x * 256 + threadIdx.x, stride = (long long)gridDim.x * 256;
  long long head = 0;
  if ((reinterpret_cast<uintptr_t>(x) & 15) == 0) {
    const float4* x4 = reinterpret_cast<const float4*>(x);
    const long long n4 = n >> 2;
    long long i = gid;
    for (; i + 3 * stride < n4; i += 4 * stride) {
      const float4 a = x4[i], b = x4[i + stride], c = x4[i + 2 * stride], d = x4[i + 3 * stride];
      m = fmaxf(m, fmaxf(fmaxf(fmaxf(a.x, a.y), fmaxf(a.z, a.w)), fmaxf(fmaxf(b.x, b.y), fmaxf(b.z, b.w))));
      m = fmaxf(m, fmaxf(fmaxf(fmaxf(c.x, c.y), fmaxf(c.z, c.w)), fmaxf(fmaxf(d.x, d.y), fmaxf(d.z, d.w))));
    }
    for (; i < n4; i += stride) {
      const float4 a = x4[i];
      m = fmaxf(m, fmaxf(fmaxf(a.x, a.y), fmaxf(a.z, a.w)));
    }
    head = n4 << 2;
  }
  for (long long i = head + gid; i < n; i += stride) m = fmaxf(m, x[i]);
#pragma unroll
  for (int off = 32; off > 0; off >>= 1) m = fmaxf(m, __shfl_xor(m, off, 64));
  if ((threadIdx.x & 63) == 0) atomicMax(buf, ord_enc(m));
}

template <typename T>
__global__ void __launch_bounds__(256) input_norm_kernel(const float* x, int B, int C, int H, int W, const unsigned* maxbuf,
                                                         const float* mean, const float* stdv, void* out, int cpad) {
  const long long gid = (long long)blockIdx.x * 256 + threadIdx.x;
  const long long plane = (long long)H * W;
  if (gid >= (long long)B * plane) return;
  const long long b = gid / plane, pp = gid % plane;
  const bool div255 = ord_dec(*maxbuf) > 1.0f;
  for (int c = 0; c < cpad; ++c) {
    float v = 0.f;
    if (c < C) {
      v = x[(b * C + c) * plane + pp];
      if (div255) v = __fdiv_rn(v, 255.0f);
      v = __fdiv_rn(__fsub_rn(v, mean[c]), stdv[c]);
    }
    Elem<T>::store(out, gid * cpad + c, v);
  }
}

template <typename T>
__global__ void __launch_bounds__(256) hier_combine_kernel(const float* low, int N, int h, int w, const void* tfeat, int Ct,
                                                           const float* ut_w, const float* ut_scale, const float* ut_shift,
                                                           int ut_act, float ut_beta, int ut_ns, const float* u1_w,
                                                           const float* u1_b, const float* t_w, const float* t_b,
                                                           float* logits, float* bgfg, float* tn) {
  __shared__ float s_ut[2 * 32 * 4], s_us[32], s_ush[32], s_u1[64], s_tw[2 * 512];
  const int t = threadIdx.x;
  for (int i = t; i < 256; i += 256) s_ut[i] = ut_w[i];
  if (t < 32 && !ut_ns) { s_us[t] = ut_scale[t]; s_ush[t] = ut_shift[t]; }
  if (t < 64) s_u1[t] = u1_w[t];
  for (int i = t; i < 2 * Ct; i += 256) s_tw[i] = t_w[i];
  __syncthreads();
  const int H = 2 * h, W = 2 * w;
  const long long gid = (long long)blockIdx.x * 256 + t;
  const long long total = (long long)N * H * W;
  if (gid >= total) return;
  const int X = (int)(gid % W);
  const long long tt = gid / W;
  const int Y = (int)(tt % H);
  const int n = (int)(tt / H);
  const int dy = Y & 1, dx = X & 1;
  const float* lo = low + (((long long)n * h + (Y >> 1)) * w + (X >> 1)) * 2;
  const float l0 = lo[0], l1 = lo[1];
  float b0 = u1_b[0], b1 = u1_b[1];
  const float* usc = ut_ns ? ut_scale + (long long)n * ut_ns : s_us;
  const float* ush = ut_ns ? ut_shift + (long long)n * ut_ns : s_ush;
  for (int co = 0; co < 32; ++co) {
    float hsum = l0 * s_ut[((0 * 32 + co) * 2 + dy) * 2 + dx] + l1 * s_ut[((1 * 32 + co) * 2 + dy) * 2 + dx];
    hsum = apply_act(hsum * usc[co] + ush[co], ut_act, ut_beta);
    b0 += s_u1[co] * hsum;
    b1 += s_u1[32 + co] * hsum;
  }
  constexpr int K = Chunk<T>::N;
  float t0 = t_b[0], t1 = t_b[1], v[K];
  const uint4* tf = reinterpret_cast<const uint4*>(tfeat) + gid * (Ct / K);
  for (int ch = 0; ch < Ct / K; ++ch) {
    Chunk<T>::unpack(tf[ch], v);
#pragma unroll
    for (int e = 0; e < K; ++e) {
      t0 += s_tw[ch * K + e] * v[e];
      t1 += s_tw[Ct + ch * K + e] * v[e];
    }
  }
  const float mx = fmaxf(b0, b1);
  const float e0 = __expf(b0 - mx), e1 = __expf(b1 - mx);
  const float pfg = e1 / (e0 + e1);
  const long long plane = (long long)H * W;
  const long long pp = (long long)Y * W + X;
  float* L = logits + (long long)n * 3 * plane + pp;
  L[0] = b0;
  L[plane] = b1 + t0 * pfg;
  L[2 * plane] = b1 + t1 * pfg;
  if (bgfg) {
    float* G = bgfg + (long long)n * 2 * plane + pp;
    G[0] = b0; G[plane] = b1;
  }
  if (tn) {
    float* Tn = tn + (long long)n * 2 * plane + pp;
    Tn[0] = t0; Tn[plane] = t1;
  }
}

template <typename T>
__global__ void __launch_bounds__(256) nhwc_to_nchw_kernel(const void* in, int N, int H, int W, int C, int cstride, int coff,
                                                           float* out) {
  const long long gid = (long long)blockIdx.x * 256 + threadIdx.x;
  const long long plane = (long long)H * W;
  const long long total = (long long)N * C * plane;
  if (gid >= total) return;
  const long long pp = gid % plane;
  const long long nc = gid / plane;
  const int c = (int)(nc % C);
  const long long n = nc / C;
  out[gid] = Elem<T>::load(in, (n * plane + pp) * cstride + coff + c);
}

template <typename T>
__global__ void __launch_bounds__(256) nchw_to_nhwc_kernel(const float* in, int N, int C, int H, int W, void* out, int cpad) {
  const long long gid = (long long)blockIdx.x * 256 + threadIdx.x;
  const long long plane = (long long)H * W;
  if (gid >= (long long)N * plane) return;
  const long long n = gid / plane, pp = gid % plane;
  for (int c = 0; c < cpad; ++c) Elem<T>::store(out, gid * cpad + c, c < C ? in[(n * C + c) * plane + pp] : 0.f);
}

__device__ __forceinline__ float p_target(const float* L, long long plane) {
  const float a = L[0], b = L[plane], c = L[2 * plane];
  const float m = fmaxf(a, fmaxf(b, c));
  const float ea = __expf(a - m), eb = __expf(b - m), ec = __expf(c - m);
  return eb / (ea + eb + ec);
}

__global__ void __launch_bounds__(256) instance_mask_kernel(const float* logits, int N, int mh, int mw, int dil, float* inst) {
  const long long gid = (long long)blockIdx.x * 256 + threadIdx.x;
  const long long plane = (long long)mh * mw;
  if (gid >= (long long)N * plane) return;
  const long long n = gid / plane, pp = gid % plane;
  const int y = (int)(pp / mw), x = (int)(pp % mw);
  const float* L = logits + n * 3 * plane;
  float l0 = L[pp], l1 = L[plane + pp], l2 = L[2 * plane + pp];
  if (dil > 0) {
    const float p1 = p_target(L + pp, plane);
    float mx = -FLT_MAX;
    for (int yy = y - dil; yy <= y + dil; ++yy)
      for (int xx = x - dil; xx <= x + dil; ++xx)
        if (yy >= 0 && yy < mh && xx >= 0 && xx < mw) mx = fmaxf(mx, p_target(L + (long long)yy * mw + xx, plane));
    if (mx - p1 > 0.1f) l1 += 2.0f;
  }
  int cls = 0;
  float best = l0;
  if (l1 > best) { cls = 1; best = l1; }
  if (l2 > best) { cls = 2; }
  inst[gid] = cls == 1 ? 1.f : 0.f;
}

__global__ void __launch_bounds__(256) binary_mask_kernel(const float* u, int cs, long long P, const float* w, const float* b,
                                                          float* out) {
  const long long gid = (long long)blockIdx.x * 256 + threadIdx.x;
  if (gid >= P) return;
  const float v = u[gid * cs];
  const float a0 = w[0] * v + b[0], a1 = w[1] * v + b[1];
  const float m = fmaxf(a0, a1);
  const float e0 = __expf(a0 - m), e1 = __expf(a1 - m);
  out[gid] = e0 / (e0 + e1);
}

__global__ void __launch_bounds__(256) resize_bilinear_kernel(const float* in, int NC, int H, int W, float* out, int Ho,
                                                              int Wo) {
  const long long gid = (long long)blockIdx.x * 256 + threadIdx.x;
  const long long total = (long long)NC * Ho * Wo;
  if (gid >= total) return;
  const int x = (int)(gid % Wo);
  const long long t = gid / Wo;
  const int y = (int)(t % Ho);
  const long long nc = t / Ho;
  const float sh = (float)H / (float)Ho, sw = (float)W / (float)Wo;
  float sy = (y + 0.5f) * sh - 0.5f;
  float sx = (x + 0.5f) * sw - 0.5f;
  sy = sy < 0.f ? 0.f : sy;
  sx = sx < 0.f ? 0.f : sx;
  const int y0 = (int)sy, x0 = (int)sx;
  const int y1 = y0 + (y0 < H - 1 ? 1 : 0), x1 = x0 + (x0 < W - 1 ? 1 : 0);
  const float ly = sy - y0, lx = sx - x0;
  const float* p = in + nc * H * W;
  const float v = (1.f - ly) * ((1.f - lx) * p[y0 * W + x0] + lx * p[y0 * W + x1]) +
                  ly * ((1.f - lx) * p[y1 * W + x0] + lx * p[y1 * W + x1]);
  out[gid] = v;
}

__global__ void __launch_bounds__(256) distance_mask_kernel(const float* x, long long n, const float* thr, float* out) {
  const long long gid = (long long)blockIdx.x * 256 + threadIdx.x;
  if (gid >= n) return;
  out[gid] = sigmoidf_((x[gid] - thr[0]) * 10.0f);
}

__global__ void __launch_bounds__(256) output_conv_kernel(const float* u, int B, long long plane, const float* w,
                                                          const float* b, float* out) {
  const long long gid = (long long)blockIdx.x * 256 + threadIdx.x;
  if (gid >= (long long)B * plane) return;
  const long long n = gid / plane, p = gid % plane;
  const float v = u[gid];
  out[(n * 2) * plane + p] = w[0] * v + b[0];
  out[(n * 2 + 1) * plane + p] = w[1] * v + b[1];
}

}

using namespace hiseg;

#define DISPATCH_T(dtype, KERNEL, ...)                                                        \
  do {                                                                                        \
    if ((dtype) == HISEG_BF16) hipLaunchKernelGGL(KERNEL<bf16_t>, __VA_ARGS__);               \
    else if ((dtype) == HISEG_F32) hipLaunchKernelGGL(KERNEL<float>, __VA_ARGS__);            \
    else { hiseg_set_error("unsupported dtype %d", (int)(dtype)); return HISEG_ERR_BAD_DTYPE; } \
  } while (0)

static int chunk_of(int dtype) { return dtype == HISEG_BF16 ? 8 : 4; }

extern "C" int hiseg_maxpool2x2_fwd(int dtype, const void* in, int N, int H, int W, int C, void* out, hiseg_stream_t stream) {
  HISEG_REQUIRE(in && out && N > 0 && H >= 2 && W >= 2 && C > 0, HISEG_ERR_BAD_SHAPE, "maxpool2x2: bad args");
  HISEG_REQUIRE(C % chunk_of(dtype) == 0, HISEG_ERR_BAD_SHAPE, "maxpool2x2: C must be chunk aligned");
  const long long total = (long long)N * (H / 2) * (W / 2) * (C / chunk_of(dtype));
  DISPATCH_T(dtype, maxpool2x2_kernel, dim3(nblocks(total, 256)), dim3(256), 0, (hipStream_t)stream, in, N, H, W, C, out);
  return hiseg_check_launch("maxpool2x2");
}

extern "C" int hiseg_attn_spatial_fwd(int dtype, const void* x, int N, int H, int W, int C, const float* w7, int k,
                                      float* stats, float* att, void* out, hiseg_stream_t stream) {
  HISEG_REQUIRE(x && w7 && stats && att && out && N > 0 && H > 0 && W > 0 && C > 0 && (k & 1), HISEG_ERR_BAD_ARG,
                "attn_spatial: bad args");
  HISEG_REQUIRE(C % chunk_of(dtype) == 0, HISEG_ERR_BAD_SHAPE, "attn_spatial: C must be chunk aligned");
  hipStream_t s = (hipStream_t)stream;
  const long long P = (long long)N * H * W;
  DISPATCH_T(dtype, attn_stats_kernel, dim3(nblocks(P * 16, 256)), dim3(256), 0, s, x, P, C, stats);
  hipLaunchKernelGGL(attn_map_kernel, dim3(nblocks(P, 256)), dim3(256), 0, s, stats, N, H, W, w7, k, att);
  const long long tot = P * (C / chunk_of(dtype));
  DISPATCH_T(dtype, pixel_scale_kernel, dim3(nblocks(tot, 256)), dim3(256), 0, s, x, P, C, att, out);
  return hiseg_check_launch("attn_spatial");
}

extern "C" int hiseg_gap_splits(int HW) {
  int s = HW / 32;
  if (s < 1) s = 1;
  if (s > 64) s = 64;
  return s;
}

extern "C" int hiseg_se_gate_fwd(int dtype, const void* x, int N, int HW, int C, const float* w1, const float* b1, int Cr,
                                 const float* w2, const float* b2, int act, float act_beta, float* partial, float* gate,
                                 hiseg_stream_t stream) {
  HISEG_REQUIRE(x && w1 && w2 && partial && gate && N > 0 && HW > 0 && C > 0 && Cr > 0, HISEG_ERR_BAD_ARG,
                "se_gate: bad args");
  const int K = chunk_of(dtype);
  HISEG_REQUIRE(C % K == 0, HISEG_ERR_BAD_SHAPE, "se_gate: C must be chunk aligned");
  const int nch = C / K;
  const int splits = hiseg_gap_splits(HW);
  HISEG_REQUIRE((long long)splits * C >= Cr, HISEG_ERR_BAD_SHAPE, "se_gate: partial buffer below N * Cr");
  const size_t lds = nch >= 256 ? 0 : (size_t)(256 / nch) * C * sizeof(float);
  hipStream_t s = (hipStream_t)stream;
  DISPATCH_T(dtype, gap_partial_kernel, dim3(N, splits), dim3(256), lds, s, x, HW, C, splits, partial);
  if (se2_enabled() && se2_fits(splits, C, Cr)) {
    se_two_launch(partial, splits, N, HW, C, w1, b1, Cr, w2, b2, act, act_beta, gate, s);
    return hiseg_check_launch("se_gate");
  }
  hipLaunchKernelGGL(gap_reduce_kernel, dim3(N, (C + 63) / 64), dim3(256), 0, s, partial, splits, C, gate);
  se_mlp(w1, b1, Cr, w2, b2, act, act_beta, N, HW, C, partial, gate, s);
  return hiseg_check_launch("se_gate");
}

extern "C" int hiseg_channel_scale_fwd(int dtype, const void* x, int N, int HW, int C, const float* gate, void* out,
                                       hiseg_stream_t stream) {
  HISEG_REQUIRE(x && gate && out && N > 0 && HW > 0 && C % chunk_of(dtype) == 0, HISEG_ERR_BAD_ARG, "channel_scale: bad args");
  const long long total = (long long)N * HW * (C / chunk_of(dtype));
  DISPATCH_T(dtype, channel_scale_kernel, dim3(nblocks(total, 256)), dim3(256), 0, (hipStream_t)stream, x, N, (long long)HW,
             C, gate, out);
  return hiseg_check_launch("channel_scale");
}

extern "C" int hiseg_dw_gap_tiles(int N, int Ho, int Wo) {
  const int strips = Ho * ((Wo + kDwXS - 1) / kDwXS);
  int t = 2048 / (N > 0 ? N : 1);
  if (t < 1) t = 1;
  int by_len = strips / 2;
  if (by_len < 1) by_len = 1;
  return t < by_len ? t : by_len;
}

static bool dw_q_enabled() {
  const char* e = getenv("HISEG_DWCONV_Q");
  return !(e && atoi(e) == 0);
}

static bool dw_use_tiles(int dtype, int C, int K, int stride) {
  const char* e = getenv("HISEG_DWCONV_T");
  const int m = e ? atoi(e) : 1;
  if (dtype != HISEG_BF16 || m == 0 || !dw_q_enabled()) return false;
  return m == 2 || (C < 2048 && ((stride == 1 && C >= 64) || (K == 5 && C >= 192)));
}

extern "C" int hiseg_dw_gap_parts(int dtype, int N, int Ho, int Wo, int C, int K, int stride) {
  if (dw_use_tiles(dtype, C, K, stride)) return ((Ho + kDwTH - 1) / kDwTH) * ((Wo + kDwTW - 1) / kDwTW);
  return hiseg_dw_gap_tiles(N, Ho, Wo);
}

static size_t dw_lds(int KS, int ST) {
  const size_t win = (size_t)((kDwTH - 1) * ST + KS) * ((kDwTW - 1) * ST + KS) * kDwPS;
  return win > 256 * 4 * sizeof(float) ? win : 256 * 4 * sizeof(float);
}

static int dw_xcd_remap() {
  const char* e = getenv("HISEG_DWCONV_XCD");
  return e ? atoi(e) : 2;
}

static bool dw_zero_pad_q(int K, int stride) {
  const char* e = getenv("HISEG_DWCONV_QZP");
  return !(e && e[0] == '0') && (K == 3 || stride == 2);
}

static int dw_xcd_remap_q() {
  const char* e = getenv("HISEG_DWCONV_QXCD");
// ... 80 lines not shown
      hipLaunchKernelGGL((dwconv_kernel<float, KS, ST>), grid, dim3(256), 0, s, in, H, W, C, w, scale, shift,  \
                         act, out, Ho, Wo, gap);                                                              \
    else                                                                                                      \
      hipLaunchKernelGGL((dwconv_kernel<bf16_t, KS, ST>), grid, dim3(256), 0, s, in, H, W, C, w, scale, shift, \
                         act, out, Ho, Wo, gap);                                                              \
  } while (0)
  if (K == 3 && stride == 1) DW_L(3, 1);
  else if (K == 3) DW_L(3, 2);
  else if (stride == 1) DW_L(5, 1);
  else DW_L(5, 2);
#undef DW_L
  return hiseg_check_launch("dwconv");
}

extern "C" int hiseg_dwconv_fwd(int dtype, const void* in, int N, int H, int W, int C, int K, int stride, const float* w,
                                const float* scale, const float* shift, int act, void* out, int Ho, int Wo,
                                hiseg_stream_t stream) {
  return dwconv_launch(dtype, in, N, H, W, C, K, stride, w, scale, shift, act, out, Ho, Wo, nullptr,
                       (hipStream_t)stream);
}

extern "C" int hiseg_dwconv_gap_fwd(int dtype, const void* in, int N, int H, int W, int C, int K, int stride,
                                    const float* w, const float* scale, const float* shift, int act, void* out, int Ho,
                                    int Wo, float* gap_partial, hiseg_stream_t stream) {
  HISEG_REQUIRE(gap_partial, HISEG_ERR_BAD_ARG, "dwconv_gap: null partial buffer");
  return dwconv_launch(dtype, in, N, H, W, C, K, stride, w, scale, shift, act, out, Ho, Wo, gap_partial,
                       (hipStream_t)stream);
}

extern "C" int hiseg_se_gate_partials_fwd(float* partial, int splits, int N, int HW, int C, const float* w1,
                                          const float* b1, int Cr, const float* w2, const float* b2, int act, float* gate,
                                          hiseg_stream_t stream) {
  HISEG_REQUIRE(partial && w1 && w2 && gate && splits > 0 && N > 0 && HW > 0 && C > 0 && Cr > 0, HISEG_ERR_BAD_ARG,
                "se_gate_partials: bad args");
  hipStream_t s = (hipStream_t)stream;
  HISEG_REQUIRE(act != HISEG_ACT_SWISH, HISEG_ERR_BAD_ARG, "se_gate_partials: Swish(beta) is not an EfficientNet act");
  if (se2_enabled() && se2_fits(splits, C, Cr)) {
    se_two_launch(partial, splits, N, HW, C, w1, b1, Cr, w2, b2, act, 1.f, gate, s);
    return hiseg_check_launch("se_gate_partials");
  }
  HISEG_REQUIRE((long long)splits * C >= Cr, HISEG_ERR_BAD_SHAPE, "se_gate_partials: partial buffer below N * Cr");
  hipLaunchKernelGGL(gap_reduce_kernel, dim3(N, (C + 63) / 64), dim3(256), 0, s, partial, splits, C, gate);
  se_mlp(w1, b1, Cr, w2, b2, act, 1.f, N, HW, C, partial, gate, s);
  return hiseg_check_launch("se_gate_partials");
}

extern "C" int hiseg_image_max_fwd(const float* x, long long n, float* maxbuf, hiseg_stream_t stream) {
  HISEG_REQUIRE(x && maxbuf && n > 0, HISEG_ERR_BAD_ARG, "image_max: bad args");
  hipStream_t s = (hipStream_t)stream;
  unsigned* buf = reinterpret_cast<unsigned*>(maxbuf);
  hipLaunchKernelGGL(reset_max_kernel, dim3(1), dim3(1), 0, s, buf);
  long long blocks = (n + 255) / 256;
  if (blocks > 2048) blocks = 2048;
  hipLaunchKernelGGL(image_max_kernel, dim3((unsigned)blocks), dim3(256), 0, s, x, n, buf);
  return hiseg_check_launch("image_max");
}

extern "C" int hiseg_input_norm_fwd(int dtype, const float* x, int B, int C, int H, int W, const float* maxbuf,
                                    const float* mean, const float* stdv, void* out, int cpad, hiseg_stream_t stream) {
  HISEG_REQUIRE(x && maxbuf && mean && stdv && out && B > 0 && C > 0 && cpad >= C, HISEG_ERR_BAD_ARG, "input_norm: bad args");
  const long long total = (long long)B * H * W;
  DISPATCH_T(dtype, input_norm_kernel, dim3(nblocks(total, 256)), dim3(256), 0, (hipStream_t)stream, x, B, C, H, W,
             reinterpret_cast<const unsigned*>(maxbuf), mean, stdv, out, cpad);
  return hiseg_check_launch("input_norm");
}

extern "C" int hiseg_hier_combine_fwd(int dtype, const float* low, int N, int h, int w, const void* tfeat, int Ct,
                                      const float* ut_w, const float* ut_scale, const float* ut_shift, int ut_act,
                                      float ut_beta, int ut_per_sample, const float* u1_w, const float* u1_b,
                                      const float* t_w, const float* t_b, float* logits, float* bgfg, float* tn,
                                      hiseg_stream_t stream) {
  HISEG_REQUIRE(low && tfeat && ut_w && ut_scale && ut_shift && u1_w && u1_b && t_w && t_b && logits, HISEG_ERR_BAD_ARG,
                "hier_combine: null pointer");
  HISEG_REQUIRE(N >= 0 && h > 0 && w > 0 && Ct > 0 && Ct <= 512 && Ct % chunk_of(dtype) == 0, HISEG_ERR_BAD_SHAPE,
                "hier_combine: bad shape (Ct %d)", Ct);
  if (N == 0) return HISEG_OK;
  const long long total = (long long)N * 4 * h * w;
  DISPATCH_T(dtype, hier_combine_kernel, dim3(nblocks(total, 256)), dim3(256), 0, (hipStream_t)stream, low, N, h, w, tfeat,
             Ct, ut_w, ut_scale, ut_shift, ut_act, ut_beta, ut_per_sample ? 32 : 0, u1_w, u1_b, t_w, t_b, logits, bgfg,
             tn);
  return hiseg_check_launch("hier_combine");
}

__global__ void __launch_bounds__(256) ubf_ln_tables_kernel(const float* low, int h, int w, const float* ut_w,
                                                            const float* ut_b, const float* gamma, const float* beta,
                                                            float eps, int fold_bias, float* mean, float* invstd,
                                                            float* scale, float* shift) {
  __shared__ double s1[256], s2[256];
  __shared__ float s_mi[2];
  const int n = blockIdx.x, t = threadIdx.x, c = t & 31, r = t >> 5;
  float wa[4], wb[4];
#pragma unroll
  for (int q = 0; q < 4; ++q) { wa[q] = ut_w[c * 4 + q]; wb[q] = ut_w[(32 + c) * 4 + q]; }
  const float bc = ut_b ? ut_b[c] : 0.f;
  double a1 = 0.0, a2 = 0.0;
  const int PL = h * w;
  const float* lo = low + (long long)n * PL * 2;
  for (int p = r; p < PL; p += 8) {
    const float l0 = lo[p * 2], l1 = lo[p * 2 + 1];
#pragma unroll
    for (int q = 0; q < 4; ++q) {
      const double z = (double)(l0 * wa[q] + l1 * wb[q] + bc);
      a1 += z; a2 += z * z;
    }
  }
  s1[t] = a1; s2[t] = a2;
  __syncthreads();
  for (int st = 128; st > 0; st >>= 1) {
    if (t < st) { s1[t] += s1[t + st]; s2[t] += s2[t + st]; }
    __syncthreads();
  }
  if (t == 0) {
    const double M = 128.0 * PL;
    const double m = s1[0] / M;
    double var = s2[0] / M - m * m;
    if (var < 0.0) var = 0.0;
    const float inv = (float)(1.0 / sqrt(var + (double)eps));
    s_mi[0] = (float)m; s_mi[1] = inv;
    if (mean) mean[n] = (float)m;
    if (invstd) invstd[n] = inv;
  }
  __syncthreads();
  if (t < 32) {
    const float k = (gamma ? gamma[t] : 1.f) * s_mi[1];
    const float m = fold_bias && ut_b ? s_mi[0] - ut_b[t] : s_mi[0];
    scale[n * 32 + t] = k;
    shift[n * 32 + t] = (beta ? beta[t] : 0.f) - m * k;
  }
}

extern "C" int hiseg_ubf_ln_tables(const float* low, int N, int h, int w, const float* ut_w, const float* ut_b,
                                   const float* gamma, const float* beta, float eps, int fold_bias, float* mean,
                                   float* invstd, float* scale, float* shift, hiseg_stream_t stream) {
  HISEG_REQUIRE(low && ut_w && scale && shift && N >= 0 && h > 0 && w > 0, HISEG_ERR_BAD_ARG, "ubf_ln_tables: bad args");
  if (N == 0) return HISEG_OK;
  hipLaunchKernelGGL(ubf_ln_tables_kernel, dim3(N), dim3(256), 0, (hipStream_t)stream, low, h, w, ut_w, ut_b, gamma,
                     beta, eps, fold_bias, mean, invstd, scale, shift);
  return hiseg_check_launch("ubf_ln_tables");
}

extern "C" int hiseg_nhwc_to_nchw_fwd(int dtype, const void* in, int N, int H, int W, int C, int cstride, int coff, float* out,
                                      hiseg_stream_t stream) {
  HISEG_REQUIRE(in && out && N >= 0 && C > 0 && cstride >= coff + C, HISEG_ERR_BAD_ARG, "nhwc_to_nchw: bad args");
  const long long total = (long long)N * C * H * W;
  if (total == 0) return HISEG_OK;
  DISPATCH_T(dtype, nhwc_to_nchw_kernel, dim3(nblocks(total, 256)), dim3(256), 0, (hipStream_t)stream, in, N, H, W, C, cstride,
             coff, out);
  return hiseg_check_launch("nhwc_to_nchw");
}

extern "C" int hiseg_nchw_to_nhwc_fwd(int dtype, const float* in, int N, int C, int H, int W, void* out, int cpad,
                                      hiseg_stream_t stream) {
  HISEG_REQUIRE(in && out && N >= 0 && C > 0 && cpad >= C, HISEG_ERR_BAD_ARG, "nchw_to_nhwc: bad args");
  const long long total = (long long)N * H * W;
  if (total == 0) return HISEG_OK;
  DISPATCH_T(dtype, nchw_to_nhwc_kernel, dim3(nblocks(total, 256)), dim3(256), 0, (hipStream_t)stream, in, N, C, H, W, out, cpad);
  return hiseg_check_launch("nchw_to_nhwc");
}

extern "C" int hiseg_instance_masks_fwd(const float* logits, int N, int mh, int mw, int dilation, float* instance,
                                        hiseg_stream_t stream) {
  HISEG_REQUIRE(logits && instance && N >= 0 && mh > 0 && mw > 0 && dilation >= 0, HISEG_ERR_BAD_ARG, "instance_masks: bad args");
  const long long total = (long long)N * mh * mw;
  if (total == 0) return HISEG_OK;
  hipLaunchKernelGGL(instance_mask_kernel, dim3(nblocks(total, 256)), dim3(256), 0, (hipStream_t)stream, logits, N, mh, mw,
                     dilation, instance);
// ... 63 lines not shown
```

### human-instance-segmentation_amd/hiseg/_lib.py

```python
from __future__ import annotations

import contextlib
import ctypes
import os

import torch

_HERE = os.path.dirname(os.path.abspath(__file__))
LIB_PATH = os.environ.get("HISEG_LIB", os.path.join(_HERE, "libhiseg.so"))

HISEG_F32 = 0
HISEG_BF16 = 1
ACT_NONE, ACT_RELU, ACT_SIGMOID, ACT_SILU, ACT_GELU, ACT_SWISH = 0, 1, 2, 3, 4, 5


class ActCode(int):

    def __new__(cls, code: int, beta: float = 1.0):
        o = int.__new__(cls, code)
        o.beta = float(beta)
        return o

    def __repr__(self):
        return f"ActCode({int(self)}, beta={self.beta})"
# ... 11 lines not shown
STRICT_PTRS = os.environ.get("HISEG_STRICT_PTRS", "0") == "1"


class Desc(ctypes.Structure):

    _ptr_fields = frozenset()

    def __init_subclass__(cls, **kw):
        super().__init_subclass__(**kw)
        cls._ptr_fields = frozenset(n for n, t in cls.__dict__.get("_fields_", ()) if t is c_void_p)

    def __setattr__(self, name, value):
        if name in self._ptr_fields and value is not None and not isinstance(value, int):
            t = value if isinstance(value, torch.Tensor) else getattr(value, "t", None)
            if not isinstance(t, torch.Tensor):
                raise TypeError(f"{type(self).__name__}.{name}: expected a tensor / activation view, got {type(value)}")
            self.__dict__.setdefault("_held", {})[name] = value
            value = t.data_ptr()
        elif name in self._ptr_fields:
            if STRICT_PTRS and value:
                raise TypeError(f"{type(self).__name__}.{name}: raw address assigned (strict pointer mode): pass the "
                                "tensor so the descriptor keeps it alive")
            held = self.__dict__.get("_held")
            if held is not None:
                held.pop(name, None)
        super().__setattr__(name, value)

    def held(self):
        return dict(self.__dict__.get("_held", {}))

    def copy(self):
        c = type(self).from_buffer_copy(self)
        c.__dict__["_held"] = dict(self.__dict__.get("_held", {}))
        return c


@contextlib.contextmanager
def raw_pointers():
    global STRICT_PTRS
    old, STRICT_PTRS = STRICT_PTRS, False
    try:
        yield
    finally:
        STRICT_PTRS = old


class RoiAlignDesc(Desc):
    _fields_ = [
        ("feat", c_void_p), ("B", c_int), ("C", c_int), ("H", c_int), ("W", c_int),
        ("rois", c_void_p), ("N", c_int),
        ("oh", c_int), ("ow", c_int),
        ("scale_h", c_float), ("scale_w", c_float),
        ("aligned", c_int),
        ("aff_w", c_void_p), ("aff_b", c_void_p), ("n_aff", c_int),
        ("out", c_void_p), ("out_dtype", c_int), ("o_cstride", c_int), ("o_coff", c_int),
        ("o_nchw", c_int), ("zero_to", c_int),
    ]


class Conv2dDesc(Desc):
    _fields_ = [
        ("dtype", c_int), ("out_dtype", c_int),
        ("N", c_int), ("H", c_int), ("W", c_int),
        ("Ho", c_int), ("Wo", c_int),
        ("KH", c_int), ("KW", c_int), ("stride", c_int), ("pad", c_int),
        ("srcA", c_void_p), ("a_cstride", c_int), ("a_coff", c_int), ("Ca", c_int), ("a_up", c_int),
        ("srcB", c_void_p), ("b_cstride", c_int), ("b_coff", c_int), ("Cb", c_int),
        ("in_scale", c_void_p),
        ("weight", c_void_p), ("Cout", c_int), ("Cout_pad", c_int), ("K_pad", c_int),
        ("scale", c_void_p), ("shift", c_void_p),
        ("act", c_int),
        ("residual", c_void_p), ("r_cstride", c_int), ("r_coff", c_int),
        ("mul", c_void_p), ("m_cstride", c_int), ("m_coff", c_int),
        ("out", c_void_p), ("o_cstride", c_int), ("o_coff", c_int),
        ("out2", c_void_p), ("o2_cstride", c_int), ("o2_coff", c_int),
        ("convT", c_int),
        ("weight_frag", c_void_p),
        ("act_beta", c_float),
        ("workspace", c_void_p), ("workspace_bytes", ctypes.c_longlong),
        ("stats_partial", c_void_p),
        ("bnb_partial", c_void_p), ("bnb_z", c_void_p), ("bnb_z_cstride", c_int), ("bnb_z_coff", c_int),
        ("bnb_scale", c_void_p), ("bnb_shift", c_void_p), ("bnb_mean", c_void_p), ("bnb_invstd", c_void_p),
        ("bnb_act", c_int),
    ]


class WgradMap(Desc):
    _fields_ = [(n, c_int) for n in ("Cout", "KH", "KW", "ca", "ca_real", "cb", "cb_real", "convT", "Cg", "Kg",
                                     "want_bias")]


HISEG_PACK_FRAG = 8
HISEG_PACK_BIAS = 4


class PackEntry(Desc):
    _fields_ = [("src", c_void_p), ("dst", c_void_p), ("dtype", c_int), ("mode", c_int),
                ("Cout", c_int), ("Cin_real", c_int), ("KH", c_int), ("KW", c_int),
                ("ca", c_int), ("ca_real", c_int), ("cb", c_int), ("cb_real", c_int),
                ("rows", c_int), ("K_pad", c_int), ("cop", c_int), ("total", c_int)]


class BnApplyDesc(Desc):
    _fields_ = [("dtype", c_int), ("P", c_ll), ("HW", c_int), ("C", c_int),
                ("z", c_void_p), ("z_cstride", c_int), ("z_coff", c_int),
                ("scale", c_void_p), ("shift", c_void_p),
                ("residual", c_void_p), ("r_cstride", c_int), ("r_coff", c_int),
                ("act", c_int), ("chan_mul", c_void_p),
                ("y", c_void_p), ("y_cstride", c_int), ("y_coff", c_int),
                ("act_beta", c_float), ("per_sample", c_int)]


class BnBwdDesc(Desc):
    _fields_ = [("dtype", c_int), ("P", c_ll), ("HW", c_int), ("C", c_int),
                ("dy", c_void_p), ("dy_cstride", c_int), ("dy_coff", c_int),
                ("y", c_void_p), ("y_cstride", c_int), ("y_coff", c_int),
                ("z", c_void_p), ("z_cstride", c_int), ("z_coff", c_int),
                ("chan_mul", c_void_p), ("act", c_int),
                ("mean", c_void_p), ("invstd", c_void_p), ("gamma", c_void_p),
                ("partial", c_void_p),
                ("dgamma", c_void_p), ("dbeta", c_void_p), ("dconv_bias", c_void_p), ("accumulate_params", c_int),
                ("dz", c_void_p), ("dz_cstride", c_int), ("dz_coff", c_int),
                ("dres", c_void_p), ("dres_cstride", c_int), ("dres_coff", c_int), ("dres_accumulate", c_int),
                ("beta", c_void_p), ("fwd_scale", c_void_p), ("fwd_shift", c_void_p),
                ("act_beta", c_float), ("residual", c_void_p), ("r_cstride", c_int), ("r_coff", c_int),
                ("partial_splits", c_int)]


class LnBwdDesc(Desc):
    _fields_ = [("dtype", c_int), ("N", c_int), ("HW", c_int), ("C", c_int),
                ("dy", c_void_p), ("dy_cstride", c_int), ("dy_coff", c_int),
                ("z", c_void_p), ("z_cstride", c_int), ("z_coff", c_int),
                ("residual", c_void_p), ("r_cstride", c_int), ("r_coff", c_int),
                ("chan_mul", c_void_p), ("act", c_int), ("act_beta", c_float),
                ("mean", c_void_p), ("invstd", c_void_p), ("scale", c_void_p), ("shift", c_void_p),
                ("gamma", c_void_p),
                ("dgamma", c_void_p), ("dbeta", c_void_p), ("dconv_bias", c_void_p), ("accumulate_params", c_int),
                ("dz", c_void_p), ("dz_cstride", c_int), ("dz_coff", c_int),
                ("dres", c_void_p), ("dres_cstride", c_int), ("dres_coff", c_int), ("dres_accumulate", c_int),
                ("ws", c_void_p)]


class EwView(Desc):
    _fields_ = [("p", c_void_p), ("cstride", c_int), ("coff", c_int)]


class UbfDesc(Desc):
    _fields_ = [("dtype", c_int), ("low", c_void_p), ("N", c_int), ("h", c_int), ("w", c_int),
                ("ut_w", c_void_p), ("ut_b", c_void_p), ("gamma", c_void_p), ("beta", c_void_p),
                ("mean", c_void_p), ("invstd", c_void_p), ("scale", c_void_p), ("shift", c_void_p),
                ("u1_w", c_void_p), ("u1_b", c_void_p),
                ("tfeat", c_void_p), ("Ct", c_int), ("t_w", c_void_p), ("t_b", c_void_p),
                ("logits", c_void_p), ("bgfg", c_void_p), ("tn", c_void_p),
                ("act", c_int), ("act_beta", c_float), ("layernorm", c_int)]


class UbfGrads(Desc):
    _fields_ = [(n, c_void_p) for n in ("dut_w", "dut_b", "dgamma", "dbeta", "du1_w", "du1_b")]


class LossCfg(ctypes.Structure):
    _fields_ = [(n, c_float) for n in ("bg_weight", "fg_weight", "target_weight", "consistency_weight", "dice_weight",
                                       "ce_weight", "boundary_aware_weight", "contour_weight", "distance_weight")] + \
               [(n, c_int) for n in ("use_dynamic_weights", "use_boundary_aware", "use_contour", "use_distance",
                                     "contour_ks")]


class DistillCfg(ctypes.Structure):
    _fields_ = [(n, c_float) for n in ("temperature", "kl_weight", "task_weight", "pos_weight")] + \
               [(n, c_int) for n in ("distill_terms", "distill_in_total", "use_dice", "has_target")] + \
               [("dev_scalars", c_void_p)]


DISTILL_NOUT = 5


class RoiTargetDesc(ctypes.Structure):
    _fields_ = [("mask_offset", c_ll)] + [(n, c_int) for n in ("n_inst", "target", "h0", "w0", "x1", "y1", "x2",
                                                                 "y2", "img_w", "img_h")]


class HisegError(RuntimeError):
    """Raised when a libhiseg entry point returns a non-zero status."""


_lib = None
_load_error = None


def _declare(lib):
    P = c_void_p
    sigs = {
        "hiseg_version": ([], c_int),
        "hiseg_last_error_string": ([], ctypes.c_char_p),
        "hiseg_built_for_gfx950": ([], c_int),
        "hiseg_stream_create_cu_mask": ([ctypes.POINTER(ctypes.c_uint), c_int, ctypes.POINTER(c_void_p)], c_int),
        "hiseg_stream_destroy": ([P], c_int),
        "hiseg_comm_load": ([ctypes.c_char_p], c_int),
        "hiseg_comm_unique_id": ([P], c_int),
        "hiseg_comm_init": ([ctypes.POINTER(c_void_p), c_int, P, c_int, c_int], c_int),
        "hiseg_comm_all_reduce": ([P, P, c_ll, c_int, c_int, P], c_int),
        "hiseg_comm_destroy": ([P], c_int),
        "hiseg_roi_align_fwd": ([ctypes.POINTER(RoiAlignDesc), P], c_int),
        "hiseg_conv2d_fwd": ([ctypes.POINTER(Conv2dDesc), P], c_int),
        "hiseg_conv2d_fwd_variant": ([ctypes.POINTER(Conv2dDesc), c_int, P], c_int),
        "hiseg_conv2d_workspace_bytes": ([ctypes.POINTER(Conv2dDesc)], c_ll),
        "hiseg_maxpool2x2_fwd": ([c_int, P, c_int, c_int, c_int, c_int, P, P], c_int),
        "hiseg_attn_spatial_fwd": ([c_int, P, c_int, c_int, c_int, c_int, P, c_int, P, P, P, P], c_int),
        "hiseg_gap_splits": ([c_int], c_int),
        "hiseg_se_gate_fwd": ([c_int, P, c_int, c_int, c_int, P, P, c_int, P, P, c_int, c_float, P, P, P], c_int),
        "hiseg_channel_scale_fwd": ([c_int, P, c_int, c_int, c_int, P, P, P], c_int),
        "hiseg_dwconv_fwd": ([c_int, P, c_int, c_int, c_int, c_int, c_int, c_int, P, P, P, c_int, P,
                              c_int, c_int, P], c_int),
        "hiseg_dw_gap_tiles": ([c_int, c_int, c_int], c_int),
        "hiseg_dw_gap_parts": ([c_int, c_int, c_int, c_int, c_int, c_int, c_int], c_int),
        "hiseg_dwconv_gap_fwd": ([c_int, P, c_int, c_int, c_int, c_int, c_int, c_int, P, P, P, c_int, P,
                                  c_int, c_int, P, P], c_int),
        "hiseg_se_gate_partials_fwd": ([P, c_int, c_int, c_int, c_int, P, P, c_int, P, P, c_int, P, P], c_int),
        "hiseg_image_max_fwd": ([P, c_ll, P, P], c_int),
        "hiseg_input_norm_fwd": ([c_int, P, c_int, c_int, c_int, c_int, P, P, P, P, c_int, P], c_int),
        "hiseg_hier_combine_fwd": ([c_int, P, c_int, c_int, c_int, P, c_int, P, P, P, c_int, c_float, c_int, P, P,
                                    P, P, P, P, P, P], c_int),
        "hiseg_ubf_ln_tables": ([P, c_int, c_int, c_int, P, P, P, P, c_float, c_int, P, P, P, P, P], c_int),
        "hiseg_nhwc_to_nchw_fwd": ([c_int, P, c_int, c_int, c_int, c_int, c_int, c_int, P, P], c_int),
        "hiseg_nchw_to_nhwc_fwd": ([c_int, P, c_int, c_int, c_int, c_int, P, c_int, P], c_int),
        "hiseg_instance_masks_fwd": ([P, c_int, c_int, c_int, c_int, P, P], c_int),
        "hiseg_binary_masks_fwd": ([c_int, P, c_int, c_int, c_int, c_int, P, P, P, P], c_int),
        "hiseg_resize_bilinear_fwd": ([P, c_int, c_int, c_int, P, c_int, c_int, P], c_int),
        "hiseg_distance_mask_fwd": ([P, c_ll, P, P, P], c_int),
        "hiseg_output_conv_fwd": ([P, c_int, c_int, c_int, P, P, P, P], c_int),
        "hiseg_conv2d_wgrad_dims": ([ctypes.POINTER(Conv2dDesc), c_int, P, P, P], c_int),
        "hiseg_conv2d_wgrad": ([ctypes.POINTER(Conv2dDesc), P, c_int, c_int, c_int, P, c_int, P], c_int),
        "hiseg_wgrad_path_stats": ([ctypes.POINTER(c_ll), c_int], c_int),
        "hiseg_struct_sizes": ([ctypes.POINTER(c_ll), c_int], c_int),
        "hiseg_conv2d_stats_tiles": ([ctypes.POINTER(Conv2dDesc)], c_int),
        "hiseg_bn_finalize_n": ([P, c_int, c_int, c_ll, P, P, c_float, c_float, P, P, P, P, P, P, P], c_int),
        "hiseg_wgrad_last_path": ([], c_int),
        "hiseg_conv2d_wgrad_reduce": ([P, c_int, ctypes.POINTER(WgradMap), P, P, c_int, P], c_int),
        "hiseg_pack_weights": ([P, c_int, c_int, P], c_int),
        "hiseg_bn_partials": ([], c_int),
        "hiseg_bn_stats": ([c_int, P, c_ll, c_int, c_int, c_int, P, P], c_int),
        "hiseg_bn_finalize": ([P, c_int, c_ll, P, P, c_float, c_float, P, P, P, P, P, P, P], c_int),
        "hiseg_bn_apply": ([ctypes.POINTER(BnApplyDesc), P], c_int),
        "hiseg_bn_bwd": ([ctypes.POINTER(BnBwdDesc), P], c_int),
        "hiseg_dropout2d_mask": ([c_int, c_int, c_float, ctypes.c_ulonglong, P, P], c_int),
        "hiseg_dropout2d_mask_dev": ([c_int, c_int, c_float, P, ctypes.c_ulonglong, P, P], c_int),
        "hiseg_seed_advance": ([P, P], c_int),
        "hiseg_relu_bwd": ([c_int, c_ll, c_int, c_int, EwView, EwView, P, EwView, P], c_int),
        "hiseg_sigmoid_bwd": ([c_int, c_ll, c_int, EwView, EwView, EwView, P], c_int),
        "hiseg_gate_fwd": ([c_int, c_ll, c_int, EwView, EwView, EwView, P], c_int),
        "hiseg_gate_bwd": ([c_int, c_ll, c_int, EwView, EwView, EwView, EwView, c_int, EwView, P], c_int),
        "hiseg_add_inplace": ([c_int, c_ll, c_int, EwView, EwView, P], c_int),
        "hiseg_act_bwd_cvt": ([c_int, c_ll, c_int, EwView, EwView, c_int, EwView, c_int, P], c_int),
        "hiseg_act_bwd_pre": ([c_int, c_ll, c_int, EwView, EwView, c_int, c_float, EwView, c_int, P], c_int),
        "hiseg_ln_ws": ([c_int, c_int, c_int], c_ll),
        "hiseg_ln_fwd_stats": ([c_int, P, c_int, c_int, c_int, c_int, c_int, P, P, c_float, P, P, P, P, P, P],
                               c_int),
        "hiseg_ln_bwd": ([ctypes.POINTER(LnBwdDesc), P], c_int),
        "hiseg_maxpool2x2_bwd": ([c_int, P, c_int, c_int, c_int, c_int, P, P, c_int, P], c_int),
        "hiseg_resize_bilinear_bwd": ([P, c_int, c_int, c_int, c_int, c_int, P, P], c_int),
        "hiseg_upsample2x_bwd": ([c_int, c_ll, c_int, c_int, c_int, EwView, EwView, c_int, P], c_int),
        "hiseg_dw_train_fwd": ([c_int, P, c_int, c_int, c_int, c_int, c_int, c_int, P, P, c_int, c_int, P], c_int),
        "hiseg_dw_bwd_data": ([c_int, P, c_int, c_int, c_int, c_int, c_int, c_int, P, c_int, c_int, P, c_int, P],
                              c_int),
        "hiseg_dw_bwd_weight_ws": ([c_int, c_int, c_int, c_int, c_int, c_int], c_ll),
        "hiseg_dw_bwd_weight": ([c_int, P, P, c_int, c_int, c_int, c_int, c_int, c_int, c_int, c_int, P, P, P],
                                c_int),
        "hiseg_se_train_ws": ([c_int, c_int, c_int], c_ll),
        "hiseg_se_train_fwd": ([c_int, P, c_int, c_int, c_int, P, P, c_int, P, P, c_int, P, P, P, P, P, P], c_int),
        "hiseg_se_train_bwd": ([c_int, P, c_int, c_int, c_int, P, c_int, P, c_int, P, P, P, P, P, P, P, P, P, P, P],
                               c_int),
        "hiseg_attn_spatial_train_fwd": ([c_int, P, c_int, c_int, c_int, c_int, P, c_int, P, P, P, P, P, P], c_int),
        "hiseg_attn_spatial_ws": ([c_int, c_int, c_int, c_int], c_int),
        "hiseg_attn_spatial_bwd": ([c_int, P, c_int, c_int, c_int, c_int, P, c_int, P, P, P, P, P, P, P, P, P], c_int),
        "hiseg_attn_channel_ws": ([c_int, c_int, c_int], c_int),
        "hiseg_attn_channel_train_fwd": ([c_int, P, c_int, c_int, c_int, P, c_int, P, c_int, c_float, P, P, P, P, P,
                                          P, P], c_int),
        "hiseg_attn_channel_bwd": ([c_int, P, c_int, c_int, c_int, P, c_int, P, c_int, c_float, P, P, P, P, P, P, P,
                                    P, P, P], c_int),
        "hiseg_ubf_ws": ([c_int], c_int),
        "hiseg_ubf_train_fwd": ([ctypes.POINTER(UbfDesc), c_float, c_float, P, P, P, P], c_int),
        "hiseg_ubf_train_bwd": ([ctypes.POINTER(UbfDesc), P, P, P, P, P, P, P, ctypes.POINTER(UbfGrads), P], c_int),
        "hiseg_pw2_ws": ([c_int], c_int),
        "hiseg_pw2_bwd": ([c_int, P, c_ll, c_int, P, P, P, P, P, P, P], c_int),
        "hiseg_roi_align_ws": ([c_int], c_int),
        "hiseg_roi_align_bwd_affine": ([ctypes.POINTER(RoiAlignDesc), P, c_int, c_int, c_int, P, P, P, P], c_int),
        "hiseg_loss_state_init": ([P, P], c_int),
        "hiseg_loss_ws": ([c_int, c_int, c_int], c_ll),
        "hiseg_loss_fwd": ([ctypes.POINTER(LossCfg), c_int, c_int, c_int, P, P, P, P, P, P, P, P, P, P], c_int),
        "hiseg_loss_fwd_begin": ([ctypes.POINTER(LossCfg), c_int, c_int, c_int, P, P, P, P], c_int),
        "hiseg_loss_fwd_end": ([ctypes.POINTER(LossCfg), c_int, c_int, c_int, P, P, P, P, P, P, P, P, P, P, P],
# ... 100 lines not shown
```

### human-instance-segmentation_amd/hiseg/engine.py

```python
from __future__ import annotations

from typing import Dict, Optional, Tuple

import torch
import torch.nn as nn

from . import _lib as L
from . import ops
from .effunet import DepthwiseSeparableConv, InvertedResidual
from .layers import LayerNorm2d, Swish
from .ops import Act, round_up

ACT_NONE, ACT_RELU, ACT_SIGMOID, ACT_SILU = L.ACT_NONE, L.ACT_RELU, L.ACT_SIGMOID, L.ACT_SILU
ACT_GELU, ACT_SWISH = L.ACT_GELU, L.ACT_SWISH


def act_code(m: nn.Module) -> int:
    if isinstance(m, nn.ReLU):
        return ACT_RELU
    if isinstance(m, nn.SiLU):
        return ACT_SILU
    if isinstance(m, Swish):
        return ACT_SILU if float(m.beta) == 1.0 else L.ActCode(ACT_SWISH, float(m.beta))
    if isinstance(m, nn.GELU):
# ... 22 lines not shown
def _signature(tensors):
    return tuple((t.data_ptr(), t._version) for t in tensors if t is not None)


def _bn_tensors(bn):
    if bn is None:
        return ()
    return (getattr(bn, "weight", None), getattr(bn, "bias", None), getattr(bn, "running_mean", None),
            getattr(bn, "running_var", None))


class Ctx:

    def __init__(self, root: nn.Module, dtype: torch.dtype, device: torch.device):
        if dtype not in (torch.float32, torch.bfloat16):
            raise TypeError(f"hiseg compute dtype must be float32 or bfloat16, got {dtype}")
        self.dtype, self.device = dtype, device
        cache = root.__dict__.get("_hiseg_plans")
        if cache is None or cache["dtype"] != dtype or cache["device"] != device:
            cache = {"dtype": dtype, "device": device, "plans": {}}
            root.__dict__["_hiseg_plans"] = cache
        self.plans: Dict = cache["plans"]

    def _get(self, key, build, deps=()):
        sig = _signature(deps)
        ent = self.plans.get(key)
        if ent is None or ent[0] != sig:
            ent = (sig, build())
            self.plans[key] = ent
        return ent[1]

    def conv(self, conv: nn.Conv2d, bn=None, act: int = ACT_NONE, split=None) -> ops.ConvPlan:
        def build():
            assert conv.groups == 1 and conv.dilation in ((1, 1), 1)
            assert conv.kernel_size[0] == conv.kernel_size[1] and conv.stride[0] == conv.stride[1]
            return ops.pack_conv(conv.weight, conv.bias, _bn(bn), act, self.dtype, self.device,
                                 stride=conv.stride[0], pad=conv.padding[0], split=split)
        return self._get(("conv", id(conv), act, split), build, (conv.weight, conv.bias) + _bn_tensors(bn))

    def convT(self, conv: nn.ConvTranspose2d, bn=None, act: int = ACT_NONE) -> ops.ConvPlan:
        def build():
            assert conv.kernel_size == (2, 2) and conv.stride == (2, 2) and conv.padding == (0, 0)
            return ops.pack_convT2x2(conv.weight, conv.bias, _bn(bn), act, self.dtype, self.device)
        return self._get(("convT", id(conv), act), build, (conv.weight, conv.bias) + _bn_tensors(bn))

    def f32(self, t: torch.Tensor, shape=None) -> torch.Tensor:
        def build():
            v = t.detach().to(device=self.device, dtype=torch.float32).contiguous()
            return v.view(shape) if shape is not None else v
        return self._get(("f32", id(t), shape), build, (t,))

    def affine(self, key, cout, bias, bn):
        def build():
            s, h = ops.fold_affine(cout, bias, _bn(bn), self.device)
            return s.contiguous(), h.contiguous()
        return self._get(("aff", key), build, (bias,) + _bn_tensors(bn))

    def dw(self, conv: nn.Conv2d, bn):
        def build():
            c, _, k, _ = conv.weight.shape
            w = conv.weight.detach().float().to(self.device).view(c, k * k).t().contiguous()
            s, h = ops.fold_affine(c, conv.bias, _bn(bn), self.device)
            return w, s.contiguous(), h.contiguous(), k, conv.stride[0]
        return self._get(("dw", id(conv)), build, (conv.weight, conv.bias) + _bn_tensors(bn))


def cna(E: Ctx, conv: nn.Module, norm: Optional[nn.Module], act: int, x: Act, xb: Optional[Act] = None, *,
        split=None, residual: Optional[Act] = None, out: Optional[Act] = None, convT: bool = False) -> Act:
    if isinstance(norm, LayerNorm2d):
        plan = E.convT(conv, None, ACT_NONE) if convT else E.conv(conv, None, ACT_NONE, split=split)
        z = ops.conv2d(plan, x, xb)
        C = z.C
        return ops.layernorm2d(z, E.f32(norm.weight, (C,)), E.f32(norm.bias, (C,)), norm.eps, act,
                               residual=residual, out=out)
    plan = E.convT(conv, norm, act) if convT else E.conv(conv, norm, act, split=split)
    return ops.conv2d(plan, x, xb, residual=residual, out=out)


def _check_input(x: torch.Tensor, what: str):
    if not x.is_cuda:
        raise RuntimeError(f"{what}: hiseg runs on the GPU only (got a CPU tensor); there is no CPU fallback")


def residual_block(E: Ctx, blk: nn.Module, x: Act, out: Optional[Act] = None) -> Act:
    a1 = act_code(blk.activation1 if hasattr(blk, "activation1") else blk.activation)
    a2 = act_code(blk.activation2 if hasattr(blk, "activation2") else blk.activation)
    h = cna(E, blk.conv1, blk.norm1, a1, x)
    return cna(E, blk.conv2, blk.norm2, a2, h, residual=x, out=out)


def rgb_feature_extractor(E: Ctx, seq: nn.Sequential, x: Act) -> Act:
    h = cna(E, seq[0], seq[1], act_code(seq[2]), x)
    h = residual_block(E, seq[3], h)
    h = cna(E, seq[4], seq[5], act_code(seq[6]), h)
    h = residual_block(E, seq[7], h)
    h = cna(E, seq[8], seq[9], act_code(seq[10]), h)
    h = residual_block(E, seq[11], h)
    return cna(E, seq[12], seq[13], act_code(seq[14]), h)


def enhanced_unet(E: Ctx, u: nn.Module, x: Act) -> Tuple[Act, Act]:
    d = u.depth
    if x.H % (1 << (d - 1)) or x.W % (1 << (d - 1)):
        raise NotImplementedError(
            f"ROI size {x.H}x{x.W} is not divisible by 2^{d - 1}: the reference's bilinear resize of the up-conv "
            "output (unet.py:408) is then not the identity; not supported on the hiseg path")
    feats = []
    for i in range(d):
        enc = u.encoders[i]
        if i == 0:
            x = cna(E, enc[0], enc[1], act_code(enc[2]), x)
            x = residual_block(E, enc[3], x)
            x = residual_block(E, enc[4], x)
        else:
            x = residual_block(E, enc[0], x)
            x = residual_block(E, enc[1], x)
            x = cna(E, enc[2], enc[3], act_code(enc[4]), x)
        feats.append(x)
        if i < d - 1:
            x = ops.maxpool2x2(x)
    b = u.bottleneck
    a = residual_block(E, b[0], x)
    a = residual_block(E, b[1], a)
    a = cna(E, b[2], b[3], act_code(b[4]), a)
    att = ops.conv2d(E.conv(b[5], None, ACT_SIGMOID), a)
    x = ops.conv2d(E.conv(u.bottleneck_conv), x, mul=att)
    for i in range(d - 1):
        up = ops.conv2d(E.convT(u.upconvs[i]), x)
        skip = feats[d - 2 - i]
        dec = u.decoders[i]
        x = cna(E, dec[0], dec[1], act_code(dec[2]), up, skip, split=(up.C, skip.C))
        x = residual_block(E, dec[3], x)
        x = residual_block(E, dec[4], x)
    f = u.final
    h = cna(E, f[0], f[1], act_code(f[2]), x)
    low = Act.new(h.N, h.H, h.W, 2, torch.float32, E.device, cpad=2, zero=False)
    low_t = Act.new(h.N, h.H, h.W, 2, E.dtype, E.device)
    ops.conv2d(E.conv(f[3]), h, out=low, out2=low_t)
    return low, low_t


def hier_head(E: Ctx, head: nn.Module, feat: Act, aux: str) -> Tuple[torch.Tensor, Dict[str, torch.Tensor]]:
    bh = head.base_head
    sf = bh.shared_features
    s = cna(E, sf[0], sf[1], act_code(sf[2]), feat)
    s = residual_block(E, sf[4], s)
    s = residual_block(E, sf[6], s)
    low, low_t = enhanced_unet(E, bh.bg_vs_fg_unet, s)
    fg = bh.fg_gate
    g = cna(E, fg[0], None, act_code(fg[1]), low_t)
    g = cna(E, fg[3], None, act_code(fg[4]), g)
    gated = ops.conv2d(E.conv(fg[5], None, ACT_SIGMOID), g, mul=s)
    tb = bh.target_vs_nontarget_branch
    if bh.use_attention_module:
        t = residual_block(E, tb[0], gated)
        t = ops.attn_spatial(t, E.f32(tb[1].conv.weight))
        t = cna(E, tb[3], tb[4], act_code(tb[5]), t, convT=True)
        ca = tb[6]
        gate = ops.se_gate(t, E.f32(ca.fc1.weight, (ca.fc1.out_channels, ca.fc1.in_channels)), None,
                           E.f32(ca.fc2.weight, (ca.fc2.out_channels, ca.fc2.in_channels)), None,
                           act_code(ca.activation))
        t = ops.channel_scale(t, gate)
        t = residual_block(E, tb[8], t)
        last = tb[9]
    else:
        t = residual_block(E, tb[0], gated)
        t = cna(E, tb[2], tb[3], act_code(tb[4]), t, convT=True)
        t = residual_block(E, tb[6], t)
        last = tb[7]
    mh, mw = bh.mask_height, bh.mask_width
    if (t.H, t.W) != (mh, mw) or (2 * low.H, 2 * low.W) != (mh, mw):
        raise NotImplementedError(f"mask size {mh}x{mw} must be 2x the ROI size {low.H}x{low.W} on the hiseg path")
    up = bh.upsample_bg_fg
    per_sample = isinstance(up[1], LayerNorm2d)
    if per_sample:
        ut_s = torch.empty(low.N * 32, dtype=torch.float32, device=E.device)
        ut_h = torch.empty_like(ut_s)
        L.check(L.lib().hiseg_ubf_ln_tables(low.t.data_ptr(), low.N, low.H, low.W, E.f32(up[0].weight).data_ptr(),
                                            E.f32(up[0].bias).data_ptr(), E.f32(up[1].weight, (32,)).data_ptr(),
                                            E.f32(up[1].bias, (32,)).data_ptr(), float(up[1].eps), 1, None, None,
                                            ut_s.data_ptr(), ut_h.data_ptr(), L.stream_ptr()), "ubf_ln_tables")
    else:
        ut_s, ut_h = E.affine(("ut", id(up[0])), up[0].out_channels, up[0].bias, up[1])
    want = aux == "full"
    logits, bgfg, tn = ops.hier_combine(
        low.t, low.N, low.H, low.W, t, E.f32(up[0].weight), ut_s, ut_h, act_code(up[2]),
        E.f32(up[3].weight, (2, up[3].in_channels)), E.f32(up[3].bias),
        E.f32(last.weight, (2, last.in_channels)), E.f32(last.bias), want, per_sample=per_sample)
    if head.use_boundary_refinement:
        logits = boundary_refine(E, head.boundary_refiner, logits)
    auxd: Dict[str, torch.Tensor] = {}
    if not want:
        return logits, auxd
    fg_att = ops.conv2d(E.conv(fg[5], None, ACT_SIGMOID), g)
    auxd.update({
        "bg_fg_logits": bgfg, "bg_fg_logits_low": low.to_nchw(), "target_nontarget_logits": tn,
        "fg_attention": fg_att.to_nchw(), "shared_features": s.to_nchw(),
    })
    lib = L.lib()
    if head.use_contour_detection:
        cb = head.contour_branch.contour_branch
        c = cna(E, cb[0], cb[1], act_code(cb[2]), s)
        c = cna(E, cb[3], cb[4], act_code(cb[5]), c)
        cm = Act.new(c.N, c.H, c.W, 1, torch.float32, E.device, cpad=1, zero=False)
        ops.conv2d(E.conv(cb[6], None, ACT_SIGMOID), c, out=cm)
        auxd["contours"] = _resize(cm.t.view(c.N, 1, c.H, c.W), mh, mw, lib)
    if head.use_distance_transform:
        dd = head.distance_decoder
        dh = dd.distance_head
        dx = cna(E, dh[0], dh[1], act_code(dh[2]), s)
        dx = residual_block(E, dh[3], dx)
        dm = Act.new(dx.N, dx.H, dx.W, 1, torch.float32, E.device, cpad=1, zero=False)
        ops.conv2d(E.conv(dh[4]), dx, out=dm)
        dmap = dm.t.view(dx.N, 1, dx.H, dx.W)
        dmask = torch.empty_like(dmap)
        L.check(lib.hiseg_distance_mask_fwd(dmap.data_ptr(), dmap.numel(), E.f32(dd.threshold).data_ptr(),
                                            dmask.data_ptr(), L.stream_ptr()), "distance_mask")
        auxd["distance_mask"] = _resize(dmask, mh, mw, lib)
        auxd["distance_map"] = _resize(dmap, mh, mw, lib)
    return logits, auxd


def refine_fused_eligible(mod: nn.Module, dtype: torch.dtype) -> bool:
    import os
    ec = mod.edge_conv
    return (dtype == torch.bfloat16 and not mod.training and os.environ.get("HISEG_REFINE_FUSED", "1") != "0"
            and isinstance(ec[1], nn.BatchNorm2d) and isinstance(ec[4], nn.BatchNorm2d)
            and isinstance(ec[2], nn.ReLU) and isinstance(ec[5], nn.ReLU)
            and tuple(ec[0].weight.shape) == (32, 3, 3, 3) and tuple(ec[3].weight.shape) == (32, 32, 3, 3)
            and tuple(ec[6].weight.shape) == (3, 32, 1, 1) and ec[6].bias is not None)


def boundary_refine(E: Ctx, mod: nn.Module, logits: torch.Tensor, want_edges: bool = False):
    if mod.training:
        raise NotImplementedError("hiseg executes the inference (eval-mode) forward; call .eval()")
    ec = mod.edge_conv
    if not want_edges and refine_fused_eligible(mod, E.dtype):
        em = ops.edge_map(logits)
        s1, t1 = E.affine(("refine1", id(ec[0])), 32, ec[0].bias, ec[1])
        s2, t2 = E.affine(("refine2", id(ec[3])), 32, ec[3].bias, ec[4])
        w2f = E._get(("refine_w2", id(ec[3])), lambda: ops.pack_refine_conv2(ec[3].weight, E.device),
                     (ec[3].weight,))
        return ops.boundary_refine_fused(em, E.f32(mod.blend_weight, (1,)), E.f32(ec[0].weight, (32, 27)), s1, t1,
                                         w2f, s2, t2, E.f32(ec[6].weight, (3, 32)), E.f32(ec[6].bias))
    em = ops.edge_map(logits, cl_dtype=E.dtype)
    h = cna(E, ec[0], ec[1], act_code(ec[2]), em.x_cl)
    h = cna(E, ec[3], ec[4], act_code(ec[5]), h)
    R = Act.new(h.N, h.H, h.W, 3, torch.float32, E.device)
    ops.conv2d(E.conv(ec[6]), h, out=R)
    out, edges = ops.boundary_blend(em, R, E.f32(mod.blend_weight, (1,)), want_edges)
    return (out, edges) if want_edges else out


def _resize(x: torch.Tensor, H: int, W: int, lib) -> torch.Tensor:
    N, C, h, w = x.shape
    if (h, w) == (H, W):
        return x
    out = torch.empty(N, C, H, W, dtype=torch.float32, device=x.device)
    L.check(lib.hiseg_resize_bilinear_fwd(x.data_ptr(), N * C, h, w, out.data_ptr(), H, W, L.stream_ptr()),
            "resize_bilinear")
    return out


def _se(E: Ctx, se: nn.Module, h: Act) -> torch.Tensor:
    rd, c = se.conv_reduce.out_channels, se.conv_reduce.in_channels
    return ops.se_gate(h, E.f32(se.conv_reduce.weight, (rd, c)), E.f32(se.conv_reduce.bias),
                       E.f32(se.conv_expand.weight, (c, rd)), E.f32(se.conv_expand.bias), ACT_SILU)


def _dw(E: Ctx, conv: nn.Conv2d, bn, x: Act, act: int) -> Act:
    w, s, h, k, stride = E.dw(conv, bn)
# ... 211 lines not shown
```

### human-instance-segmentation_amd/hiseg/ops.py

```python
from __future__ import annotations

import ctypes
from dataclasses import dataclass
from typing import Optional

import torch

from . import _lib as L

_TORCH_TO_HISEG = {torch.float32: L.HISEG_F32, torch.bfloat16: L.HISEG_BF16}


def chunk_elems(dtype: torch.dtype) -> int:
    return 8 if dtype == torch.bfloat16 else 4


def round_up(x: int, m: int) -> int:
    return (x + m - 1) // m * m


def hdtype(dtype: torch.dtype) -> int:
    try:
        return _TORCH_TO_HISEG[dtype]
    except KeyError:
# ... 131 lines not shown
    pad: int
    ca: int
    cb: int
    cout: int
    gemm_cols: int
    cout_pad: int
    k_pad: int
    act: int
    convT: bool = False
    weight_frag: Optional[torch.Tensor] = None


def pack_conv(weight: torch.Tensor, bias: Optional[torch.Tensor], bn: Optional[torch.nn.BatchNorm2d], act: int,
              dtype: torch.dtype, device, stride: int = 1, pad: int = 0, split=None) -> ConvPlan:
    ce = chunk_elems(dtype)
    w = weight.detach().float()
    cout, cin, kh, kw = w.shape
    ca_r, cb_r = split[:2] if split is not None else (cin, 0)
    assert ca_r + cb_r == cin
    ca, cb = round_up(ca_r, ce), round_up(cb_r, ce)
    if split is not None and len(split) > 2:
        cb = max(cb, int(split[2]))
    wk = torch.zeros(cout, kh, kw, ca + cb, dtype=torch.float32, device=w.device)
    wt = w.permute(0, 2, 3, 1)
    wk[..., :ca_r] = wt[..., :ca_r]
    if cb_r:
        wk[..., ca:ca + cb_r] = wt[..., ca_r:]
    k = kh * kw * (ca + cb)
    k_pad = round_up(k, 64)
    cout_pad = round_up(cout, 16)
    wp = torch.zeros(cout_pad, k_pad, dtype=torch.float32, device=w.device)
    wp[:cout, :k] = wk.reshape(cout, k)
    scale, shift = fold_affine(cout, bias, bn, w.device)
    sc = torch.zeros(cout_pad, dtype=torch.float32, device=w.device)
    sh = torch.zeros(cout_pad, dtype=torch.float32, device=w.device)
    sc[:cout], sh[:cout] = scale, shift
    frag = None
    if dtype == torch.bfloat16 and kh == 3 and kw == 3 and stride == 1 and ca % 64 == 0 and cb % 64 == 0 and k == k_pad:
        frag = frag_pack(wp, kh * kw, ca + cb).to(device=device, dtype=dtype).contiguous()
    return ConvPlan(wp.to(device=device, dtype=dtype).contiguous(), sc.to(device), sh.to(device), kh, kw, stride, pad,
                    ca, cb, cout, cout, cout_pad, k_pad, act, weight_frag=frag)


def frag_pack(wp: torch.Tensor, taps: int, cin: int) -> torch.Tensor:
    cp = wp.shape[0]
    v = wp.reshape(cp // 16, 16, taps, cin // 64, 2, 4, 8)
    v = v.permute(0, 3, 2, 4, 5, 1, 6)
    return v.reshape(-1)


def pack_convT2x2(weight: torch.Tensor, bias: Optional[torch.Tensor], bn, act: int, dtype, device) -> ConvPlan:
    ce = chunk_elems(dtype)
    w = weight.detach().float()
    cin, cout, kh, kw = w.shape
    assert kh == 2 and kw == 2 and cout % 4 == 0
    ca = round_up(cin, ce)
    cols = 4 * cout
    k_pad = round_up(ca, 64)
    cout_pad = round_up(cols, 16)
    wp = torch.zeros(cout_pad, k_pad, dtype=torch.float32, device=w.device)
    wp[:cols, :cin] = w.permute(2, 3, 1, 0).reshape(cols, cin)
    scale, shift = fold_affine(cout, bias, bn, w.device)
    sc = torch.zeros(cout_pad, dtype=torch.float32, device=w.device)
    sh = torch.zeros(cout_pad, dtype=torch.float32, device=w.device)
    sc[:cols], sh[:cols] = scale.repeat(4), shift.repeat(4)
    return ConvPlan(wp.to(device=device, dtype=dtype).contiguous(), sc.to(device), sh.to(device), 1, 1, 1, 0,
                    ca, 0, cout, cols, cout_pad, k_pad, act, convT=True)


def fold_affine(cout: int, bias: Optional[torch.Tensor], bn, device):
    scale = torch.ones(cout, dtype=torch.float32, device=device)
    shift = torch.zeros(cout, dtype=torch.float32, device=device)
    if bias is not None:
        shift = bias.detach().float().to(device).clone()
    if bn is not None:
        g = bn.weight.detach().float() if bn.weight is not None else torch.ones(cout, device=device)
        b = bn.bias.detach().float() if bn.bias is not None else torch.zeros(cout, device=device)
        inv = g / torch.sqrt(bn.running_var.detach().float() + bn.eps)
        shift = (shift - bn.running_mean.detach().float()) * inv + b
        scale = inv
    return scale, shift


def conv2d(p: ConvPlan, xa: Act, xb: Optional[Act] = None, out: Optional[Act] = None, *, a_up: int = 1,
           residual: Optional[Act] = None, mul: Optional[Act] = None, out2: Optional[Act] = None,
           in_scale: Optional[torch.Tensor] = None, out_dtype: Optional[torch.dtype] = None,
           variant: int = 0, out_cpad: Optional[int] = None, split_k_3x3: bool = False) -> Act:
    dt = xa.dtype
    H, W = xa.H * a_up, xa.W * a_up
    if xb is not None:
        assert xb.dtype == dt and (xb.H, xb.W, xb.N) == (H, W, xa.N)
    if p.convT:
        Ho, Wo = H, W
        oH, oW = 2 * H, 2 * W
    else:
        Ho = (H + 2 * p.pad - p.kh) // p.stride + 1
        Wo = (W + 2 * p.pad - p.kw) // p.stride + 1
        oH, oW = Ho, Wo
    if out is None:
        out = Act.new(xa.N, oH, oW, p.cout, out_dtype or dt, xa.t.device, cpad=out_cpad,
                      zero=None if out_cpad is None else out_cpad != p.cout)
    assert (out.N, out.H, out.W) == (xa.N, oH, oW), ((out.N, out.H, out.W), (xa.N, oH, oW))
    assert xa.C <= p.ca and (xb is None or xb.C <= p.cb)
    d = L.Conv2dDesc()
    d.dtype, d.out_dtype = hdtype(dt), hdtype(out.dtype)
    d.N, d.H, d.W, d.Ho, d.Wo = xa.N, H, W, Ho, Wo
    d.KH, d.KW, d.stride, d.pad = p.kh, p.kw, p.stride, p.pad
    d.srcA, d.a_cstride, d.a_coff, d.Ca, d.a_up = xa, xa.cstride, xa.coff, p.ca, a_up
    if xb is not None:
        d.srcB, d.b_cstride, d.b_coff, d.Cb = xb, xb.cstride, xb.coff, p.cb
    if in_scale is not None:
        d.in_scale = in_scale
    d.weight, d.Cout, d.Cout_pad, d.K_pad = p.weight, p.gemm_cols, p.cout_pad, p.k_pad
    d.scale, d.shift, d.act, d.act_beta = p.scale, p.shift, int(p.act), L.act_beta(p.act)
    if residual is not None:
        d.residual, d.r_cstride, d.r_coff = residual, residual.cstride, residual.coff
    if mul is not None:
        d.mul, d.m_cstride, d.m_coff = mul, mul.cstride, mul.coff
    d.out, d.o_cstride, d.o_coff = out, out.cstride, out.coff
    if out2 is not None:
        assert out2.dtype == dt
        d.out2, d.o2_cstride, d.o2_coff = out2, out2.cstride, out2.coff
    d.convT = int(p.convT)
    if p.weight_frag is not None:
        d.weight_frag = p.weight_frag
    ws = None
    if dt == torch.bfloat16 and not p.convT and ((p.kh * p.kw == 1 and p.k_pad >= 384) or
                                                 (split_k_3x3 and p.kh * p.kw == 9)):
        nbytes = L.lib().hiseg_conv2d_workspace_bytes(ctypes.byref(d))
        if nbytes > 0:
            ws = torch.empty(nbytes, dtype=torch.uint8, device=xa.t.device)
            d.workspace, d.workspace_bytes = ws, nbytes
    if RECORD is not None:
        dc = d.copy()
        keep = [t for t in (xa, xb, out, residual, mul, out2, ws) if t is not None]
        flops = 2.0 * d.N * d.Ho * d.Wo * p.gemm_cols * p.kh * p.kw * (xa.C + (xb.C if xb is not None else 0))
        RECORD.append((dc, keep, p, flops))
    gate = GATE
    if gate is not None:
        flops = 2.0 * d.N * d.Ho * d.Wo * p.gemm_cols * p.kh * p.kw * (xa.C + (xb.C if xb is not None else 0))
        if flops >= gate.min_flops and not variant:
            gate.before()
            _launch_conv(d, p, xa, xb)
            gate.after()
            return out
        gate.light()
    _launch_conv(d, p, xa, xb, variant)
    return out


def _launch_conv(d, p, xa, xb, variant=0):
    if PROBE is not None:
        key = PROBE.select(d)
        if key is not None:
            flops = 2.0 * d.N * d.Ho * d.Wo * p.gemm_cols * p.kh * p.kw * (xa.C + (xb.C if xb is not None else 0))
            L.check(PROBE.around(key, flops, lambda: L.lib().hiseg_conv2d_fwd(ctypes.byref(d), L.stream_ptr())),
                    "conv2d")
            return
    if variant:
        L.check(L.lib().hiseg_conv2d_fwd_variant(ctypes.byref(d), variant, L.stream_ptr()), "conv2d")
    else:
        L.check(L.lib().hiseg_conv2d_fwd(ctypes.byref(d), L.stream_ptr()), "conv2d")


def maxpool2x2(x: Act) -> Act:
    assert x.coff == 0 and x.cstride == x.cpad
    out = Act.new(x.N, x.H // 2, x.W // 2, x.C, x.dtype, x.t.device, cpad=x.cstride, zero=False)
    L.check(L.lib().hiseg_maxpool2x2_fwd(hdtype(x.dtype), x.ptr(), x.N, x.H, x.W, x.cstride, out.ptr(),
                                         L.stream_ptr()), "maxpool2x2")
    return out


def attn_spatial(x: Act, w7: torch.Tensor) -> Act:
    assert x.coff == 0 and x.cstride == x.C
    P = x.N * x.H * x.W
    stats = torch.empty(P * 2, dtype=torch.float32, device=x.t.device)
    att = torch.empty(P, dtype=torch.float32, device=x.t.device)
    out = Act.new(x.N, x.H, x.W, x.C, x.dtype, x.t.device, zero=False)
    k = w7.shape[-1]
    L.check(L.lib().hiseg_attn_spatial_fwd(hdtype(x.dtype), x.ptr(), x.N, x.H, x.W, x.C, w7.data_ptr(), k,
                                           stats.data_ptr(), att.data_ptr(), out.ptr(), L.stream_ptr()),
            "attn_spatial")
    return out


def se_gate(x: Act, w1, b1, w2, b2, act: int) -> torch.Tensor:
    assert x.coff == 0 and x.cstride == x.C
    HW = x.H * x.W
    lib = L.lib()
    splits = lib.hiseg_gap_splits(HW)
    partial = torch.empty(x.N * splits * x.C, dtype=torch.float32, device=x.t.device)
    gate = torch.empty(x.N, x.C, dtype=torch.float32, device=x.t.device)
    cr = w1.shape[0]
    L.check(lib.hiseg_se_gate_fwd(hdtype(x.dtype), x.ptr(), x.N, HW, x.C, w1.data_ptr(), _ptr(b1), cr,
                                  w2.data_ptr(), _ptr(b2), int(act), L.act_beta(act), partial.data_ptr(), gate.data_ptr(),
                                  L.stream_ptr()), "se_gate")
    return gate


def channel_scale(x: Act, gate: torch.Tensor) -> Act:
    assert x.coff == 0 and x.cstride == x.C
    out = Act.new(x.N, x.H, x.W, x.C, x.dtype, x.t.device, zero=False)
    L.check(L.lib().hiseg_channel_scale_fwd(hdtype(x.dtype), x.ptr(), x.N, x.H * x.W, x.C, gate.data_ptr(),
                                            out.ptr(), L.stream_ptr()), "channel_scale")
    return out


def dwconv(x: Act, w: torch.Tensor, scale: torch.Tensor, shift: torch.Tensor, k: int, stride: int, act: int) -> Act:
    assert x.coff == 0 and x.cstride == x.C
    pad = k // 2
    Ho = (x.H + 2 * pad - k) // stride + 1
    Wo = (x.W + 2 * pad - k) // stride + 1
    out = Act.new(x.N, Ho, Wo, x.C, x.dtype, x.t.device, zero=False)
    L.check(L.lib().hiseg_dwconv_fwd(hdtype(x.dtype), x.ptr(), x.N, x.H, x.W, x.C, k, stride, w.data_ptr(),
                                     scale.data_ptr(), shift.data_ptr(), act, out.ptr(), Ho, Wo, L.stream_ptr()),
            "dwconv")
    return out


def dwconv_se_gate(x: Act, w: torch.Tensor, scale: torch.Tensor, shift: torch.Tensor, k: int, stride: int, act: int,
                   w1, b1, w2, b2, se_act: int):
    assert x.coff == 0 and x.cstride == x.C
    pad = k // 2
    Ho = (x.H + 2 * pad - k) // stride + 1
    Wo = (x.W + 2 * pad - k) // stride + 1
    lib = L.lib()
    out = Act.new(x.N, Ho, Wo, x.C, x.dtype, x.t.device, zero=False)
    tiles = lib.hiseg_dw_gap_parts(hdtype(x.dtype), x.N, Ho, Wo, x.C, k, stride)
    partial = torch.empty(x.N * tiles * x.C, dtype=torch.float32, device=x.t.device)
    L.check(lib.hiseg_dwconv_gap_fwd(hdtype(x.dtype), x.ptr(), x.N, x.H, x.W, x.C, k, stride, w.data_ptr(),
                                     scale.data_ptr(), shift.data_ptr(), act, out.ptr(), Ho, Wo, partial.data_ptr(),
                                     L.stream_ptr()), "dwconv_gap")
    gate = torch.empty(x.N, x.C, dtype=torch.float32, device=x.t.device)
    L.check(lib.hiseg_se_gate_partials_fwd(partial.data_ptr(), tiles, x.N, Ho * Wo, x.C, w1.data_ptr(), _ptr(b1),
                                           w1.shape[0], w2.data_ptr(), _ptr(b2), se_act, gate.data_ptr(),
                                           L.stream_ptr()), "se_gate_partials")
    return out, gate


def input_norm(images: torch.Tensor, mean: torch.Tensor, std: torch.Tensor, dtype: torch.dtype) -> Act:
    _require_gpu(images)
    x = images.contiguous().float()
    B, C, H, W = x.shape
    lib = L.lib()
    maxbuf = torch.empty(1, dtype=torch.float32, device=x.device)
    L.check(lib.hiseg_image_max_fwd(x.data_ptr(), x.numel(), maxbuf.data_ptr(), L.stream_ptr()), "image_max")
    out = Act.new(B, H, W, C, dtype, x.device, zero=False)
    L.check(lib.hiseg_input_norm_fwd(hdtype(dtype), x.data_ptr(), B, C, H, W, maxbuf.data_ptr(), mean.data_ptr(),
                                     std.data_ptr(), out.ptr(), out.cstride, L.stream_ptr()), "input_norm")
    return out


def hier_combine(low: torch.Tensor, N: int, h: int, w: int, tfeat: Act, ut_w, ut_scale, ut_shift, ut_act, u1_w, u1_b,
                 t_w, t_b, want_aux: bool, per_sample: bool = False):
    assert tfeat.coff == 0 and tfeat.cstride == tfeat.C and (tfeat.H, tfeat.W) == (2 * h, 2 * w)
    dev = low.device
    logits = torch.empty(N, 3, 2 * h, 2 * w, dtype=torch.float32, device=dev)
    bgfg = torch.empty(N, 2, 2 * h, 2 * w, dtype=torch.float32, device=dev) if want_aux else None
    tn = torch.empty(N, 2, 2 * h, 2 * w, dtype=torch.float32, device=dev) if want_aux else None
    L.check(L.lib().hiseg_hier_combine_fwd(hdtype(tfeat.dtype), low.data_ptr(), N, h, w, tfeat.ptr(), tfeat.C,
                                           ut_w.data_ptr(), ut_scale.data_ptr(), ut_shift.data_ptr(), int(ut_act),
                                           L.act_beta(ut_act), int(per_sample), u1_w.data_ptr(), u1_b.data_ptr(), t_w.data_ptr(), t_b.data_ptr(),
                                           logits.data_ptr(), _ptr(bgfg), _ptr(tn), L.stream_ptr()), "hier_combine")
    return logits, bgfg, tn


def layernorm2d(z: Act, weight: torch.Tensor, bias: torch.Tensor, eps: float, act: int,
                residual: Optional[Act] = None, out: Optional[Act] = None) -> Act:
    lib = L.lib()
    dev = z.t.device
    N, HW, C = z.N, z.H * z.W, z.C
    ws = torch.empty(int(lib.hiseg_ln_ws(N, HW, C)), dtype=torch.float32, device=dev)
    mean = torch.empty(N, dtype=torch.float32, device=dev)
    invstd = torch.empty_like(mean)
    scale = torch.empty(N * C, dtype=torch.float32, device=dev)
    shift = torch.empty_like(scale)
    L.check(lib.hiseg_ln_fwd_stats(hdtype(z.dtype), z.ptr(), N, HW, C, z.cstride, z.coff, weight.data_ptr(),
                                   bias.data_ptr(), float(eps), ws.data_ptr(), mean.data_ptr(), invstd.data_ptr(),
                                   scale.data_ptr(), shift.data_ptr(), L.stream_ptr()), "ln_fwd_stats")
    y = out if out is not None else Act.new(N, z.H, z.W, C, z.dtype, dev, cpad=z.cstride)
    d = L.BnApplyDesc()
    d.dtype, d.P, d.HW, d.C = hdtype(z.dtype), N * HW, HW, C
    d.z, d.z_cstride, d.z_coff = z, z.cstride, z.coff
    d.scale, d.shift, d.per_sample = scale, shift, 1
    if residual is not None:
        d.residual, d.r_cstride, d.r_coff = residual, residual.cstride, residual.coff
    d.act, d.act_beta = int(act), L.act_beta(act)
    d.y, d.y_cstride, d.y_coff = y, y.cstride, y.coff
    L.check(lib.hiseg_bn_apply(ctypes.byref(d), L.stream_ptr()), "ln_apply")
    return y


def instance_masks(logits: torch.Tensor, dilation: int = 0) -> torch.Tensor:
    N, _, mh, mw = logits.shape
    out = torch.empty(N, 1, mh, mw, dtype=torch.float32, device=logits.device)
    L.check(L.lib().hiseg_instance_masks_fwd(logits.contiguous().data_ptr(), N, mh, mw, int(dilation), out.data_ptr(),
                                             L.stream_ptr()), "instance_masks")
    return out


def binary_masks(u: torch.Tensor, oc_w: torch.Tensor, oc_b: torch.Tensor) -> torch.Tensor:
    B, _, H, W = u.shape
    out = torch.empty(B, 1, H, W, dtype=torch.float32, device=u.device)
    L.check(L.lib().hiseg_binary_masks_fwd(L.HISEG_F32, u.data_ptr(), 1, B, H, W, oc_w.data_ptr(), oc_b.data_ptr(),
                                           out.data_ptr(), L.stream_ptr()), "binary_masks")
    return out




def _post_planes(x: torch.Tensor, what: str):
    _require_gpu(x)
    if x.dim() < 2:
        raise ValueError(f"{what}: expected [..., H, W] planes, got shape {tuple(x.shape)}")
    x = x.to(torch.float32).contiguous()
    H, W = x.shape[-2:]
    return x, (x.numel() // (H * W) if H * W else 0), H, W


def _post_chunks(iterations: int, H: int, W: int, radius: int, force_tiled: bool):
    if iterations < 1:
        raise ValueError(f"iterations must be >= 1, got {iterations}")
    cap = L.lib().hiseg_post_max_iterations(H, W, radius, int(force_tiled))
    out = []
    while iterations > 0:
        out.append(min(iterations, cap))
        iterations -= out[-1]
    return out


def edge_smooth(x: torch.Tensor, threshold: float = 0.5, blur_strength: float = 3.0, iterations: int = 1, *,
                binarize_input: bool = False, _force_tiled: bool = False) -> torch.Tensor:
    x, NC, H, W = _post_planes(x, "edge_smooth")
    for n in _post_chunks(iterations, H, W, 1, _force_tiled):
        out = torch.empty_like(x)
        L.check(L.lib().hiseg_edge_smooth_fwd(x.data_ptr(), out.data_ptr(), NC, H, W, threshold, blur_strength, n,
                                              int(binarize_input), int(_force_tiled), L.stream_ptr()), "edge_smooth")
        x, binarize_input = out, False
    return x


def class_edge_smooth(scores: torch.Tensor, threshold: float = 0.5, blur_strength: float = 3.0, iterations: int = 1,
# ... 112 lines not shown
```

### include/hiseg.h

```cpp
#ifndef HISEG_H_
#define HISEG_H_

#ifdef __cplusplus
extern "C" {
#endif

typedef void* hiseg_stream_t;

enum hiseg_dtype { HISEG_F32 = 0, HISEG_BF16 = 1 };

enum hiseg_act { HISEG_ACT_NONE = 0, HISEG_ACT_RELU = 1, HISEG_ACT_SIGMOID = 2, HISEG_ACT_SILU = 3,
                 HISEG_ACT_GELU = 4, HISEG_ACT_SWISH = 5 };

enum hiseg_status {
  HISEG_OK = 0,
  HISEG_ERR_BAD_ARG = -1,
  HISEG_ERR_BAD_SHAPE = -2,
  HISEG_ERR_BAD_DTYPE = -3,
  HISEG_ERR_LAUNCH = -4
};

int hiseg_version(void);
const char* hiseg_last_error_string(void);
int hiseg_built_for_gfx950(void);
int hiseg_debug_fill_lds(unsigned pattern, int rounds, hiseg_stream_t stream);
int hiseg_placement_stats(long long* declined, long long* far, int reset);

int hiseg_stream_create_cu_mask(const unsigned* mask, int nwords, hiseg_stream_t* out);
int hiseg_stream_destroy(hiseg_stream_t s);

typedef struct hiseg_roi_align_desc {
  const float* feat; int B, C, H, W;
  const float* rois; int N;
  int oh, ow;
  float scale_h, scale_w;
  int aligned;
  const float* aff_w; const float* aff_b; int n_aff;
  void* out; int out_dtype; int o_cstride; int o_coff; int o_nchw; int zero_to;
} hiseg_roi_align_desc;
int hiseg_roi_align_fwd(const hiseg_roi_align_desc* d, hiseg_stream_t stream);

typedef struct hiseg_conv2d_desc {
  int dtype, out_dtype;
  int N, H, W;
  int Ho, Wo;
  int KH, KW, stride, pad;
  const void* srcA; int a_cstride, a_coff, Ca, a_up;
  const void* srcB; int b_cstride, b_coff, Cb;
  const float* in_scale;
  const void* weight; int Cout, Cout_pad, K_pad;
  const float* scale; const float* shift;
  int act;
  const void* residual; int r_cstride, r_coff;
  const void* mul; int m_cstride, m_coff;
  void* out; int o_cstride, o_coff;
  void* out2; int o2_cstride, o2_coff;
  int convT;
  const void* weight_frag;
  float act_beta;
  void* workspace; long long workspace_bytes;
  float* stats_partial;
  float* bnb_partial; const void* bnb_z; int bnb_z_cstride, bnb_z_coff;
  const float* bnb_scale; const float* bnb_shift; const float* bnb_mean; const float* bnb_invstd; int bnb_act;
} hiseg_conv2d_desc;
int hiseg_conv2d_fwd(const hiseg_conv2d_desc* d, hiseg_stream_t stream);
int hiseg_struct_sizes(long long* out, int n);
long long hiseg_conv2d_workspace_bytes(const hiseg_conv2d_desc* d);
int hiseg_conv2d_stats_tiles(const hiseg_conv2d_desc* d);
int hiseg_conv2d_fwd_variant(const hiseg_conv2d_desc* d, int variant, hiseg_stream_t stream);

int hiseg_maxpool2x2_fwd(int dtype, const void* in, int N, int H, int W, int C, void* out,
                         hiseg_stream_t stream);

int hiseg_attn_spatial_fwd(int dtype, const void* x, int N, int H, int W, int C, const float* w7,
                           int k, float* stats, float* att, void* out, hiseg_stream_t stream);

int hiseg_gap_splits(int HW);
int hiseg_se_gate_fwd(int dtype, const void* x, int N, int HW, int C, const float* w1,
                      const float* b1, int Cr, const float* w2, const float* b2, int act, float act_beta,
                      float* partial, float* gate, hiseg_stream_t stream);

int hiseg_channel_scale_fwd(int dtype, const void* x, int N, int HW, int C, const float* gate,
                            void* out, hiseg_stream_t stream);

int hiseg_dwconv_fwd(int dtype, const void* in, int N, int H, int W, int C, int K, int stride,
                     const float* w, const float* scale, const float* shift, int act, void* out,
                     int Ho, int Wo, hiseg_stream_t stream);
int hiseg_dw_gap_tiles(int N, int Ho, int Wo);
int hiseg_dw_gap_parts(int dtype, int N, int Ho, int Wo, int C, int K, int stride);
int hiseg_dwconv_gap_fwd(int dtype, const void* in, int N, int H, int W, int C, int K, int stride,
                         const float* w, const float* scale, const float* shift, int act, void* out,
                         int Ho, int Wo, float* gap_partial, hiseg_stream_t stream);
int hiseg_se_gate_partials_fwd(float* partial, int splits, int N, int HW, int C, const float* w1,
                               const float* b1, int Cr, const float* w2, const float* b2, int act,
                               float* gate, hiseg_stream_t stream);

int hiseg_image_max_fwd(const float* x, long long n, float* maxbuf, hiseg_stream_t stream);
int hiseg_input_norm_fwd(int dtype, const float* x, int B, int C, int H, int W, const float* maxbuf,
                         const float* mean, const float* std, void* out, int cpad,
                         hiseg_stream_t stream);

int hiseg_hier_combine_fwd(int dtype, const float* low, int N, int h, int w, const void* tfeat,
                           int Ct, const float* ut_w, const float* ut_scale, const float* ut_shift,
                           int ut_act, float ut_beta, int ut_per_sample, const float* u1_w,
                           const float* u1_b, const float* t_w, const float* t_b, float* logits,
                           float* bgfg, float* tn, hiseg_stream_t stream);
int hiseg_ubf_ln_tables(const float* low, int N, int h, int w, const float* ut_w, const float* ut_b,
                        const float* gamma, const float* beta, float eps, int fold_bias, float* mean,
                        float* invstd, float* scale, float* shift, hiseg_stream_t stream);

int hiseg_nhwc_to_nchw_fwd(int dtype, const void* in, int N, int H, int W, int C, int cstride,
                           int coff, float* out, hiseg_stream_t stream);
int hiseg_nchw_to_nhwc_fwd(int dtype, const float* in, int N, int C, int H, int W, void* out,
                           int cpad, hiseg_stream_t stream);

int hiseg_instance_masks_fwd(const float* logits, int N, int mh, int mw, int dilation,
                             float* instance, hiseg_stream_t stream);
int hiseg_binary_masks_fwd(int dtype, const void* u, int u_cstride, int B, int H, int W,
                           const float* oc_w, const float* oc_b, float* binary,
                           hiseg_stream_t stream);

int hiseg_resize_bilinear_fwd(const float* in, int NC, int H, int W, float* out, int Ho, int Wo,
                              hiseg_stream_t stream);

int hiseg_distance_mask_fwd(const float* x, long long n, const float* threshold, float* out,
                            hiseg_stream_t stream);

int hiseg_output_conv_fwd(const float* u, int B, int H, int W, const float* w, const float* b, float* out,
                          hiseg_stream_t stream);

#ifdef __cplusplus
}
#endif
#endif
```

Baseline: 16100 ROI-masks/s.

## Fuse 2-channel head projection into residual conv epilogue and spatial attention into ConvTranspose

Adds a head2 epilogue to the 128-Cout residual HWC conv. It projects the bf16 tile onto two output channels and writes a float2 per pixel, so the 128-channel feature map is never stored and hier_combine reads the precomputed pair. It also adds a px_scale path to the pointwise ConvTranspose kernel, which multiplies the inputs by a per-pixel attention map on load in place of a separate pixel_scale pass. Both paths are gated by applicability checks and fall back otherwise, at the cost of more template variants and extra register use in the conv kernels.

```diff
diff --git a/human-instance-segmentation_amd/csrc/conv_hwc.hip b/human-instance-segmentation_amd/csrc/conv_hwc.hip
--- a/human-instance-segmentation_amd/csrc/conv_hwc.hip
+++ b/human-instance-segmentation_amd/csrc/conv_hwc.hip
@@ -1,4 +1,5 @@
 #include "conv_common.h"
+#include "head2.h"
 
 namespace hiseg {
 
@@ -16,7 +17,7 @@
 }
 
 template <int ACT, bool RES, int NW, bool UP = false, int ABL = 0, bool RP = false, bool ST = false, int TWB = 1,
-          bool BR = false, bool R3 = false>
+          bool BR = false, bool R3 = false, bool H2 = false>
 __global__ void __launch_bounds__(NW * 64, NW == 4 ? 2 : 1) conv_hwc_kernel(ConvArgs a) {
   constexpr int NCG = NW / TWB;
   constexpr int BCO = 32 * NCG, TM = 2, NR = 16;
@@ -29,6 +30,7 @@
   constexpr int NPX = 256 * TWB;
   static_assert((NW == 4 || NW == 8) && (TWB == 1 || (TWB == 2 && NW == 4 && !RP)), "configuration");
   static_assert(!R3 || (NW == 4 && !RP && TWB == 1 && !ST && !BR), "R3: the plain / residual 128-Cout form");
+  static_assert(!H2 || (NW == 4 && TWB == 1 && !ST && !BR && !UP && !RP && ABL == 0), "H2: the 128-Cout one-block form");
   constexpr int NPMIN = ((NHR + 15) / 16 - 1 - (NW - 1)) / NW + 1;
   extern __shared__ __attribute__((aligned(16))) uint4 smem[];
   const hiseg_conv2d_desc& d = a.d;
@@ -276,6 +278,8 @@
     return;
   }
   char* tile = reinterpret_cast<char*>(smem);
+  typedef const __attribute__((address_space(4))) float* h2_cptr;
+  h2_cptr h2w = (h2_cptr)(uintptr_t)d.head2_w;
   if constexpr (RES && !RP) {
 #pragma unroll
     for (int k = 0; k < NRI; ++k) res_dma(k);
@@ -341,6 +345,24 @@
     convert(std::integral_constant<int, 0>{}, std::integral_constant<int, NR>{});
   }
   __syncthreads();
+  if constexpr (H2) {
+    const int px = px_of(t);
+    float t0 = d.head2_b[0], t1 = d.head2_b[1];
+#pragma unroll
+    for (int c = 0; c < CPR; ++c) {
+      float v[8];
+      Chunk<bf16_t>::unpack(*reinterpret_cast<const uint4*>(tile + t * EROWB + ((c ^ (t & SWM)) << 4)), v);
+      float w0[8], w1[8];
+#pragma unroll
+      for (int e = 0; e < 8; ++e) {
+        w0[e] = h2w[8 * c + e];
+        w1[e] = h2w[BCO + 8 * c + e];
+      }
+      head2_acc<8>(t0, t1, w0, w1, v);
+    }
+    if (px >= 0) *reinterpret_cast<float2*>(d.head2_out + 2ll * px) = make_float2(t0, t1);
+    return;
+  }
   constexpr int NST = NPX * CPR / (NW * 64);
   float sk[8], s1[8], s2[8];
   int sn = 0;
@@ -472,7 +494,7 @@
 }
 
 template <int ACT, bool RES, int NW, bool UP = false, int ABL = 0, bool RP = false, bool ST = false, int TWB = 1,
-          bool BR = false, bool R3 = false>
+          bool BR = false, bool R3 = false, bool H2 = false>
 static int launch_hwc(const ConvArgs& a, hipStream_t s) {
   const hiseg_conv2d_desc& d = a.d;
   constexpr int BCO = 32 * NW / TWB, TW = 16 * TWB;
@@ -482,7 +504,7 @@
   const int nco = d.Cout_pad / BCO;
   const size_t halo = R3 ? halo2 / 2 * 3 : halo2;
   const size_t lds = RP ? (size_t)80 * 1024 : (halo > epi ? halo : epi);
-  auto kern = conv_hwc_kernel<ACT, RES, NW, UP, ABL, RP, ST, TWB, BR, R3>;
+  auto kern = conv_hwc_kernel<ACT, RES, NW, UP, ABL, RP, ST, TWB, BR, R3, H2>;
   static bool attr = false;
   if (!attr) {
     (void)hipFuncSetAttribute((const void*)kern, hipFuncAttributeMaxDynamicSharedMemorySize, (int)lds);
@@ -852,7 +874,15 @@
        !d.bnb_scale || !d.bnb_shift || !d.bnb_mean || !d.bnb_invstd ||
        (d.bnb_act != HISEG_ACT_RELU && d.bnb_act != HISEG_ACT_NONE)))
     return false;
+  if (d.head2_out &&
+      ((variant != 104 && variant != 108) || d.Cout != 128 || !d.residual || d.a_up != 1 || d.stats_partial ||
+       d.bnb_partial || !d.head2_w || !d.head2_b || ((uintptr_t)d.head2_out & 7)))
+    return false;
   return true;
+}
+
+bool conv_hwc_head2_applies(const ConvArgs& a, bool r3) {
+  return a.d.head2_out != nullptr && conv_hwc_applies(a, r3 ? 108 : 104);
 }
 
 int conv_hwc_stats_tiles(const ConvArgs& a) {
@@ -908,6 +938,16 @@
                       : launch_hwc<HISEG_ACT_NONE, false, 4, false, 0, false, true>(a, s);
     return r < 0 ? r : 1;
   }
+  if (d.head2_out) {
+    const bool relu = d.act == HISEG_ACT_RELU;
+    const int r =
+        variant == 108
+            ? (relu ? launch_hwc<HISEG_ACT_RELU, true, 4, false, 0, false, false, 1, false, true, true>(a, s)
+                    : launch_hwc<HISEG_ACT_NONE, true, 4, false, 0, false, false, 1, false, true, true>(a, s))
+            : (relu ? launch_hwc<HISEG_ACT_RELU, true, 4, false, 0, false, false, 1, false, false, true>(a, s)
+                    : launch_hwc<HISEG_ACT_NONE, true, 4, false, 0, false, false, 1, false, false, true>(a, s));
+    return r < 0 ? r : 1;
+  }
   const int r = variant == 109 ? launch_hwc_mt_act<1, HISEG_CONV_HWC_MT>(a, s)
               : variant == 102 ? launch_hwc_mt_act<2, HISEG_CONV_HWC_MT>(a, s)
               : variant == 107 ? launch_hwc_nw<4, false, 2>(a, s)
diff --git a/human-instance-segmentation_amd/csrc/conv_igemm.hip b/human-instance-segmentation_amd/csrc/conv_igemm.hip
--- a/human-instance-segmentation_amd/csrc/conv_igemm.hip
+++ b/human-instance-segmentation_amd/csrc/conv_igemm.hip
@@ -431,6 +431,7 @@
 int conv_hwt_try(const ConvArgs& a, hipStream_t s, int variant);
 int conv_hwc_try(const ConvArgs& a, hipStream_t s, int variant);
 int conv_hwc_stats_tiles(const ConvArgs& a);
+bool conv_hwc_head2_applies(const ConvArgs& a, bool r3);
 int conv_small_try(const ConvArgs& a, hipStream_t s, int variant);
 int conv_rows_try(const ConvArgs& a, hipStream_t s, int variant);
 bool conv_pw_applies(const ConvArgs& a);
@@ -502,6 +503,22 @@
   return conv_hwc_stats_tiles(a);
 }
 
+extern "C" int hiseg_conv2d_fused_ok(const hiseg_conv2d_desc* d) {
+  if (d == nullptr || d->dtype != HISEG_BF16 || d->N <= 0 || (!d->px_scale && !d->head2_out) ||
+      (d->px_scale && d->head2_out) || d->stats_partial || d->bnb_partial || d->a_up != 1 || d->K_pad % 64)
+    return 0;
+  const long long M = (long long)d->N * d->Ho * d->Wo;
+  if (M >= (1ll << 31)) return 0;
+  ConvArgs a;
+  a.d = *d;
+  a.M = (int)M;
+  a.Cin = d->Ca + d->Cb;
+  a.nK = d->K_pad / 64;
+  a.Hs = d->H;
+  a.Ws = d->W;
+  return d->px_scale ? (conv_pw_applies(a) ? 1 : 0) : (conv_hwc_head2_applies(a, hwc_r3_mode()) ? 1 : 0);
+}
+
 extern "C" int hiseg_conv2d_fwd_variant(const hiseg_conv2d_desc* d, int variant, hiseg_stream_t stream) {
 #ifndef HISEG_DIAG
   HISEG_REQUIRE(release_variant(variant), HISEG_ERR_BAD_ARG,
@@ -514,7 +531,11 @@
   HISEG_REQUIRE(d != nullptr, HISEG_ERR_BAD_ARG, "conv2d: null descriptor");
   HISEG_REQUIRE(d->dtype == HISEG_F32 || d->dtype == HISEG_BF16, HISEG_ERR_BAD_DTYPE, "conv2d: dtype %d", d->dtype);
   HISEG_REQUIRE(d->out_dtype == HISEG_F32 || d->out_dtype == HISEG_BF16, HISEG_ERR_BAD_DTYPE, "conv2d: out_dtype %d", d->out_dtype);
-  HISEG_REQUIRE(d->srcA && d->weight && d->scale && d->shift && d->out, HISEG_ERR_BAD_ARG, "conv2d: null pointer");
+  HISEG_REQUIRE(d->srcA && d->weight && d->scale && d->shift && (d->out || d->head2_out), HISEG_ERR_BAD_ARG,
+                "conv2d: null pointer");
+  HISEG_REQUIRE(!(d->px_scale || d->head2_out) || (variant == 0 && !d->stats_partial && !d->bnb_partial &&
+                                                   !(d->px_scale && d->head2_out)),
+                HISEG_ERR_BAD_ARG, "conv2d: px_scale / head2_out go with the automatic choice alone, one at a time");
   HISEG_REQUIRE(d->N > 0 && d->H > 0 && d->W > 0 && d->Ho > 0 && d->Wo > 0, HISEG_ERR_BAD_SHAPE, "conv2d: empty grid");
   HISEG_REQUIRE(d->KH > 0 && d->KW > 0 && d->stride > 0 && d->pad >= 0, HISEG_ERR_BAD_SHAPE, "conv2d: bad window");
   HISEG_REQUIRE(d->a_up == 1 || d->a_up == 2, HISEG_ERR_BAD_SHAPE, "conv2d: a_up must be 1 or 2");
@@ -593,6 +614,8 @@
         c.out = const_cast<void*>(at(d->out, out_px * d->o_cstride * eo));
         c.out2 = const_cast<void*>(at(d->out2, out_px * d->o2_cstride * ea));
         if (d->in_scale) c.in_scale = d->in_scale + (long long)n0 * d->Ca;
+        if (d->px_scale) c.px_scale = d->px_scale + n0 * in_px;
+        if (d->head2_out) c.head2_out = d->head2_out + 2 * n0 * out_px;
         const int r = conv2d_impl(&c, stream, variant);
         if (r) return r;
       }
@@ -612,6 +635,12 @@
   a.ins_vec = d->in_scale != nullptr && ((uintptr_t)d->in_scale & 15) == 0 && (d->Ca & 3) == 0;
   a.ws = static_cast<float*>(d->workspace);
   a.kper = a.nK;
+  if (d->px_scale || d->head2_out) {
+    const int r = d->px_scale ? conv_pw_try(a, s, 90) : conv_hwc_try(a, s, hwc_r3_mode() ? 108 : 104);
+    HISEG_REQUIRE(r != 0, HISEG_ERR_BAD_ARG,
+                  "conv2d: no kernel takes this layer with px_scale / head2_out (hiseg_conv2d_fused_ok)");
+    return r < 0 ? r : HISEG_OK;
+  }
   if (variant == 99 || variant == 0) {
     const int sp = splitk_plan(a);
     if (sp > 1 && d->workspace != nullptr && d->workspace_bytes >= splitk_bytes(a, sp) &&
diff --git a/human-instance-segmentation_amd/csrc/conv_pw.hip b/human-instance-segmentation_amd/csrc/conv_pw.hip
--- a/human-instance-segmentation_amd/csrc/conv_pw.hip
+++ b/human-instance-segmentation_amd/csrc/conv_pw.hip
@@ -12,7 +12,7 @@
 typedef unsigned pw_u4 __attribute__((ext_vector_type(4)));
 typedef unsigned pw_u2 __attribute__((ext_vector_type(2)));
 
-template <int NKSA, int EPI, int ACT, bool CONVT, int RB, bool INS>
+template <int NKSA, int EPI, int ACT, bool CONVT, int RB, bool INS, bool PXS = false>
 __global__ void __launch_bounds__(256, 1) conv_pw_kernel(ConvArgs a, int nct, int nks_arg) {
   constexpr int NKS = NKSA < 0 ? -NKSA : NKSA;
   const int nks = NKSA < 0 ? nks_arg : NKSA;
@@ -104,6 +104,15 @@
   const __amdgpu_buffer_rsrc_t rR = __builtin_amdgcn_make_buffer_rsrc(
       const_cast<void*>(xp), (short)0, XOP ? (int)(out_px * x_cs * 2) : 0, 0x00020000);
   const bool bch_ok = NKS == 9 && 8 * g < d.Cb;
+  const __amdgpu_buffer_rsrc_t rS = __builtin_amdgcn_make_buffer_rsrc(
+      const_cast<float*>(PXS ? d.px_scale : d.scale), (short)0, PXS ? (int)((long long)M * 4) : 0, 0x00020000);
+  auto load_ps = [&](int b, float (&ps)[2]) __attribute__((always_inline)) {
+#pragma unroll
+    for (int j = 0; j < 2; ++j) {
+      const int p = b * kPwBlk + 16 * j + pl;
+      ps[j] = __builtin_bit_cast(float, __builtin_amdgcn_raw_buffer_load_b32(rS, p < M ? (unsigned)(p * 4) : OOB, 0, 0));
+    }
+  };
 
   auto load_ks = [&](int b, int ks, uint4 (&bk)[2]) __attribute__((always_inline)) {
     if (abl & 2) {
@@ -155,11 +164,28 @@
   const int stride = ngrp * 4;
   int b = grp * 4 + w;
   uint4 b0[NKS][2], b1[NKS][2];
+  float ps0[2] = {0.f, 0.f}, ps1[2] = {0.f, 0.f};
 #pragma unroll
   for (int ks = 0; ks < NKS; ++ks)
     if (ks < nks) load_ks(b, ks, b0[ks]);
-  auto process = [&](int b, uint4 (&bf)[NKS][2], uint4 (&bn)[NKS][2]) __attribute__((always_inline)) {
+  if constexpr (PXS) load_ps(b, ps0);
+  auto process = [&](int b, uint4 (&bf)[NKS][2], uint4 (&bn)[NKS][2], float (&psf)[2], float (&psn)[2])
+      __attribute__((always_inline)) {
     const int nb = b + stride;
+    if constexpr (PXS) {
+#pragma unroll
+      for (int ks = 0; ks < NKS; ++ks) {
+        if (ks >= nks) continue;
+#pragma unroll
+        for (int j = 0; j < 2; ++j) {
+          float f[8];
+          Chunk<bf16_t>::unpack(bf[ks][j], f);
+#pragma unroll
+          for (int e = 0; e < 8; ++e) f[e] *= psf[j];
+          bf[ks][j] = Chunk<bf16_t>::pack(f);
+        }
+      }
+    }
     if constexpr (INS) {
       int gofs[2];
 #pragma unroll
@@ -187,6 +213,7 @@
 #pragma unroll
     for (int ks = 0; ks < NKS; ++ks)
       if (ks < nks) load_ks(nb, ks, bn[ks]);
+    if constexpr (PXS) load_ps(nb, psn);
     set_block(b);
     pw_u2 rv[XOP ? RB : 1][2];
     if constexpr (XOP) {
@@ -241,9 +268,9 @@
     }
   };
   for (; b < nblk; b += 2 * stride) {
-    process(b, b0, b1);
+    process(b, b0, b1, ps0, ps1);
     if (b + stride >= nblk) break;
-    process(b + stride, b1, b0);
+    process(b + stride, b1, b0, ps1, ps0);
   }
 }
 
@@ -261,11 +288,11 @@
   return (size_t)16 * RB * (NKS * 4 + 1) * 16 + 2 * 16 * RB * 4 + (ins ? (size_t)d.N * d.Ca * 4 : 0);
 }
 
-template <int NKSA, int EPI, int ACT, bool CONVT, int RB, bool INS>
+template <int NKSA, int EPI, int ACT, bool CONVT, int RB, bool INS, bool PXS = false>
 static int launch_pw(const ConvArgs& a, hipStream_t s, int nks) {
   const hiseg_conv2d_desc& d = a.d;
   const size_t lds = pw_lds_bytes(NKSA < 0 ? -NKSA : NKSA, RB, INS, d);
-  auto kern = conv_pw_kernel<NKSA, EPI, ACT, CONVT, RB, INS>;
+  auto kern = conv_pw_kernel<NKSA, EPI, ACT, CONVT, RB, INS, PXS>;
   static int occ = 0;
   static size_t occ_lds = 0;
   if (lds > occ_lds) {
@@ -342,6 +369,11 @@
            : act == SI ? launch_pw<-NKS, 0, SI, false, 16, false>(a, s, nks)
                        : launch_pw<-NKS, 0, N, false, 16, false>(a, s, nks);
     }
+    if constexpr (NKS == 8) {
+      if (d.convT && d.px_scale) return act == R ? launch_pw<NKS, 0, R, true, 16, false, true>(a, s, nks)
+                                                 : launch_pw<NKS, 0, N, true, 16, false, true>(a, s, nks);
+    }
+    HISEG_REQUIRE(!d.px_scale, HISEG_ERR_BAD_ARG, "conv_pw: px_scale needs the 8-k-step ConvTranspose form");
     if (d.convT) return act == R ? launch_pw<NKS, 0, R, true, 16, false>(a, s, nks)
                                  : launch_pw<NKS, 0, N, true, 16, false>(a, s, nks);
     if (d.residual) return act == R ? launch_pw<NKS, 1, R, false, 16, false>(a, s, nks)
@@ -380,6 +412,9 @@
       if (!(want > 4 && nks > 8)) rb = want;
     }
   }
+  if (d.px_scale && (!d.convT || rb != 16 || nks != 8 || d.Ca != 256 || d.in_scale || ((uintptr_t)d.px_scale & 3) ||
+                     (d.act != HISEG_ACT_NONE && d.act != HISEG_ACT_RELU)))
+    return false;
   const bool comb = rb == 16 && nks == 9;
   if ((rb == 16 && nks > 9) || (rb > 4 && nks > 8)) return false;
   if (comb ? (d.Ca != 256 || d.Cb > 32 || d.convT || d.residual || d.mul || d.in_scale ||
diff --git a/human-instance-segmentation_amd/csrc/head2.h b/human-instance-segmentation_amd/csrc/head2.h
--- /dev/null
+++ b/human-instance-segmentation_amd/csrc/head2.h
@@ -0,0 +1,15 @@
+#pragma once
+#include "common.h"
+
+namespace hiseg {
+
+template <int K>
+__device__ __forceinline__ void head2_acc(float& t0, float& t1, const float* w0, const float* w1, const float (&v)[K]) {
+#pragma unroll
+  for (int e = 0; e < K; ++e) {
+    t0 += w0[e] * v[e];
+    t1 += w1[e] * v[e];
+  }
+}
+
+}
diff --git a/human-instance-segmentation_amd/csrc/misc.hip b/human-instance-segmentation_amd/csrc/misc.hip
--- a/human-instance-segmentation_amd/csrc/misc.hip
+++ b/human-instance-segmentation_amd/csrc/misc.hip
@@ -1,5 +1,6 @@
 #include <float.h>
 #include "common.h"
+#include "head2.h"
 
 namespace hiseg {
 
@@ -815,7 +816,7 @@
   }
 }
 
-template <typename T>
+template <typename T, bool TN2 = false>
 __global__ void __launch_bounds__(256) hier_combine_kernel(const float* low, int N, int h, int w, const void* tfeat, int Ct,
                                                            const float* ut_w, const float* ut_scale, const float* ut_shift,
                                                            int ut_act, float ut_beta, int ut_ns, const float* u1_w,
@@ -826,7 +827,8 @@
   for (int i = t; i < 256; i += 256) s_ut[i] = ut_w[i];
   if (t < 32 && !ut_ns) { s_us[t] = ut_scale[t]; s_ush[t] = ut_shift[t]; }
   if (t < 64) s_u1[t] = u1_w[t];
-  for (int i = t; i < 2 * Ct; i += 256) s_tw[i] = t_w[i];
+  if constexpr (!TN2)
+    for (int i = t; i < 2 * Ct; i += 256) s_tw[i] = t_w[i];
   __syncthreads();
   const int H = 2 * h, W = 2 * w;
   const long long gid = (long long)blockIdx.x * 256 + t;
@@ -849,14 +851,19 @@
     b1 += s_u1[32 + co] * hsum;
   }
   constexpr int K = Chunk<T>::N;
-  float t0 = t_b[0], t1 = t_b[1], v[K];
-  const uint4* tf = reinterpret_cast<const uint4*>(tfeat) + gid * (Ct / K);
-  for (int ch = 0; ch < Ct / K; ++ch) {
-    Chunk<T>::unpack(tf[ch], v);
-#pragma unroll
-    for (int e = 0; e < K; ++e) {
-      t0 += s_tw[ch * K + e] * v[e];
-      t1 += s_tw[Ct + ch * K + e] * v[e];
+  float t0, t1;
+  if constexpr (TN2) {
+    const float2 tq = reinterpret_cast<const float2*>(tfeat)[gid];
+    t0 = tq.x;
+    t1 = tq.y;
+  } else {
+    t0 = t_b[0];
+    t1 = t_b[1];
+    float v[K];
+    const uint4* tf = reinterpret_cast<const uint4*>(tfeat) + gid * (Ct / K);
+    for (int ch = 0; ch < Ct / K; ++ch) {
+      Chunk<T>::unpack(tf[ch], v);
+      head2_acc<K>(t0, t1, s_tw + ch * K, s_tw + Ct + ch * K, v);
     }
   }
   const float mx = fmaxf(b0, b1);
@@ -1014,6 +1021,27 @@
   const long long tot = P * (C / chunk_of(dtype));
   DISPATCH_T(dtype, pixel_scale_kernel, dim3(nblocks(tot, 256)), dim3(256), 0, s, x, P, C, att, out);
   return hiseg_check_launch("attn_spatial");
+}
+
+extern "C" int hiseg_attn_map_fwd(int dtype, const void* x, int N, int H, int W, int C, const float* w7, int k,
+                                  float* stats, float* att, hiseg_stream_t stream) {
+  HISEG_REQUIRE(x && w7 && stats && att && N > 0 && H > 0 && W > 0 && C > 0 && (k & 1), HISEG_ERR_BAD_ARG,
+                "attn_map: bad args");
+  HISEG_REQUIRE(C % chunk_of(dtype) == 0, HISEG_ERR_BAD_SHAPE, "attn_map: C must be chunk aligned");
+  hipStream_t s = (hipStream_t)stream;
+  const long long P = (long long)N * H * W;
+  DISPATCH_T(dtype, attn_stats_kernel, dim3(nblocks(P * 16, 256)), dim3(256), 0, s, x, P, C, stats);
+  hipLaunchKernelGGL(attn_map_kernel, dim3(nblocks(P, 256)), dim3(256), 0, s, stats, N, H, W, w7, k, att);
+  return hiseg_check_launch("attn_map");
+}
+
+extern "C" int hiseg_pixel_scale_fwd(int dtype, const void* x, long long P, int C, const float* att, void* out,
+                                     hiseg_stream_t stream) {
+  HISEG_REQUIRE(x && att && out && P > 0 && C > 0, HISEG_ERR_BAD_ARG, "pixel_scale: bad args");
+  HISEG_REQUIRE(C % chunk_of(dtype) == 0, HISEG_ERR_BAD_SHAPE, "pixel_scale: C must be chunk aligned");
+  const long long tot = P * (C / chunk_of(dtype));
+  DISPATCH_T(dtype, pixel_scale_kernel, dim3(nblocks(tot, 256)), dim3(256), 0, (hipStream_t)stream, x, P, C, att, out);
+  return hiseg_check_launch("pixel_scale");
 }
 
 extern "C" int hiseg_gap_splits(int HW) {
@@ -1260,6 +1288,21 @@
   return hiseg_check_launch("hier_combine");
 }
 
+extern "C" int hiseg_hier_combine_tn_fwd(const float* low, int N, int h, int w, const float* tn2, const float* ut_w,
+                                         const float* ut_scale, const float* ut_shift, int ut_act, float ut_beta,
+                                         int ut_per_sample, const float* u1_w, const float* u1_b, float* logits,
+                                         float* bgfg, float* tn, hiseg_stream_t stream) {
+  HISEG_REQUIRE(low && tn2 && ut_w && ut_scale && ut_shift && u1_w && u1_b && logits, HISEG_ERR_BAD_ARG,
+                "hier_combine_tn: null pointer");
+  HISEG_REQUIRE(N >= 0 && h > 0 && w > 0 && ((uintptr_t)tn2 & 7) == 0, HISEG_ERR_BAD_SHAPE, "hier_combine_tn: bad shape");
+  if (N == 0) return HISEG_OK;
+  const long long total = (long long)N * 4 * h * w;
+  hipLaunchKernelGGL((hier_combine_kernel<float, true>), dim3(nblocks(total, 256)), dim3(256), 0, (hipStream_t)stream, low,
+                     N, h, w, (const void*)tn2, 0, ut_w, ut_scale, ut_shift, ut_act, ut_beta, ut_per_sample ? 32 : 0, u1_w,
+                     u1_b, (const float*)nullptr, (const float*)nullptr, logits, bgfg, tn);
+  return hiseg_check_launch("hier_combine_tn");
+}
+
 __global__ void __launch_bounds__(256) ubf_ln_tables_kernel(const float* low, int h, int w, const float* ut_w,
                                                             const float* ut_b, const float* gamma, const float* beta,
                                                             float eps, int fold_bias, float* mean, float* invstd,
diff --git a/human-instance-segmentation_amd/hiseg/_lib.py b/human-instance-segmentation_amd/hiseg/_lib.py
--- a/human-instance-segmentation_amd/hiseg/_lib.py
+++ b/human-instance-segmentation_amd/hiseg/_lib.py
@@ -117,6 +117,8 @@
         ("bnb_partial", c_void_p), ("bnb_z", c_void_p), ("bnb_z_cstride", c_int), ("bnb_z_coff", c_int),
         ("bnb_scale", c_void_p), ("bnb_shift", c_void_p), ("bnb_mean", c_void_p), ("bnb_invstd", c_void_p),
         ("bnb_act", c_int),
+        ("px_scale", c_void_p),
+        ("head2_w", c_void_p), ("head2_b", c_void_p), ("head2_out", c_void_p),
     ]
 
 
@@ -242,6 +244,11 @@
         "hiseg_conv2d_workspace_bytes": ([ctypes.POINTER(Conv2dDesc)], c_ll),
         "hiseg_maxpool2x2_fwd": ([c_int, P, c_int, c_int, c_int, c_int, P, P], c_int),
         "hiseg_attn_spatial_fwd": ([c_int, P, c_int, c_int, c_int, c_int, P, c_int, P, P, P, P], c_int),
+        "hiseg_attn_map_fwd": ([c_int, P, c_int, c_int, c_int, c_int, P, c_int, P, P, P], c_int),
+        "hiseg_pixel_scale_fwd": ([c_int, P, c_ll, c_int, P, P, P], c_int),
+        "hiseg_conv2d_fused_ok": ([ctypes.POINTER(Conv2dDesc)], c_int),
+        "hiseg_hier_combine_tn_fwd": ([P, c_int, c_int, c_int, P, P, P, P, c_int, c_float, c_int, P, P, P, P, P, P],
+                                      c_int),
         "hiseg_gap_splits": ([c_int], c_int),
         "hiseg_se_gate_fwd": ([c_int, P, c_int, c_int, c_int, P, P, c_int, P, P, c_int, c_float, P, P, P], c_int),
         "hiseg_channel_scale_fwd": ([c_int, P, c_int, c_int, c_int, P, P, P], c_int),
diff --git a/human-instance-segmentation_amd/hiseg/engine.py b/human-instance-segmentation_amd/hiseg/engine.py
--- a/human-instance-segmentation_amd/hiseg/engine.py
+++ b/human-instance-segmentation_amd/hiseg/engine.py
@@ -128,10 +128,13 @@
         raise RuntimeError(f"{what}: hiseg runs on the GPU only (got a CPU tensor); there is no CPU fallback")
 
 
-def residual_block(E: Ctx, blk: nn.Module, x: Act, out: Optional[Act] = None) -> Act:
+def residual_block(E: Ctx, blk: nn.Module, x: Act, out: Optional[Act] = None,
+                   head2: Optional[ops.Head2] = None) -> Optional[Act]:
     a1 = act_code(blk.activation1 if hasattr(blk, "activation1") else blk.activation)
     a2 = act_code(blk.activation2 if hasattr(blk, "activation2") else blk.activation)
     h = cna(E, blk.conv1, blk.norm1, a1, x)
+    if head2 is not None and out is None and not isinstance(blk.norm2, LayerNorm2d):
+        return ops.conv2d(E.conv(blk.conv2, blk.norm2, a2), h, residual=x, head2=head2)
     return cna(E, blk.conv2, blk.norm2, a2, h, residual=x, out=out)
 
 
@@ -200,22 +203,27 @@
     tb = bh.target_vs_nontarget_branch
     if bh.use_attention_module:
         t = residual_block(E, tb[0], gated)
-        t = ops.attn_spatial(t, E.f32(tb[1].conv.weight))
-        t = cna(E, tb[3], tb[4], act_code(tb[5]), t, convT=True)
+        if isinstance(tb[4], LayerNorm2d):
+            t = ops.attn_spatial(t, E.f32(tb[1].conv.weight))
+            t = cna(E, tb[3], tb[4], act_code(tb[5]), t, convT=True)
+        else:
+            att = ops.attn_map(t, E.f32(tb[1].conv.weight))
+            t = ops.conv2d(E.convT(tb[3], tb[4], act_code(tb[5])), t, px_scale=att)
         ca = tb[6]
         gate = ops.se_gate(t, E.f32(ca.fc1.weight, (ca.fc1.out_channels, ca.fc1.in_channels)), None,
                            E.f32(ca.fc2.weight, (ca.fc2.out_channels, ca.fc2.in_channels)), None,
                            act_code(ca.activation))
         t = ops.channel_scale(t, gate)
-        t = residual_block(E, tb[8], t)
-        last = tb[9]
+        blk, last = tb[8], tb[9]
     else:
         t = residual_block(E, tb[0], gated)
         t = cna(E, tb[2], tb[3], act_code(tb[4]), t, convT=True)
-        t = residual_block(E, tb[6], t)
-        last = tb[7]
+        blk, last = tb[6], tb[7]
+    h2 = ops.Head2(E.f32(last.weight, (2, last.in_channels)), E.f32(last.bias))
+    tH, tW = t.H, t.W
+    t = residual_block(E, blk, t, head2=h2)
     mh, mw = bh.mask_height, bh.mask_width
-    if (t.H, t.W) != (mh, mw) or (2 * low.H, 2 * low.W) != (mh, mw):
+    if (tH, tW) != (mh, mw) or (2 * low.H, 2 * low.W) != (mh, mw):
         raise NotImplementedError(f"mask size {mh}x{mw} must be 2x the ROI size {low.H}x{low.W} on the hiseg path")
     up = bh.upsample_bg_fg
     per_sample = isinstance(up[1], LayerNorm2d)
@@ -232,7 +240,7 @@
     logits, bgfg, tn = ops.hier_combine(
         low.t, low.N, low.H, low.W, t, E.f32(up[0].weight), ut_s, ut_h, act_code(up[2]),
         E.f32(up[3].weight, (2, up[3].in_channels)), E.f32(up[3].bias),
-        E.f32(last.weight, (2, last.in_channels)), E.f32(last.bias), want, per_sample=per_sample)
+        h2.w, h2.b, want, per_sample=per_sample, tn2=h2.out)
     if head.use_boundary_refinement:
         logits = boundary_refine(E, head.boundary_refiner, logits)
     auxd: Dict[str, torch.Tensor] = {}
diff --git a/human-instance-segmentation_amd/hiseg/ops.py b/human-instance-segmentation_amd/hiseg/ops.py
--- a/human-instance-segmentation_amd/hiseg/ops.py
+++ b/human-instance-segmentation_amd/hiseg/ops.py
@@ -237,10 +237,18 @@
     return scale, shift
 
 
+@dataclass
+class Head2:
+    w: torch.Tensor
+    b: torch.Tensor
+    out: Optional[torch.Tensor] = None
+
+
 def conv2d(p: ConvPlan, xa: Act, xb: Optional[Act] = None, out: Optional[Act] = None, *, a_up: int = 1,
            residual: Optional[Act] = None, mul: Optional[Act] = None, out2: Optional[Act] = None,
            in_scale: Optional[torch.Tensor] = None, out_dtype: Optional[torch.dtype] = None,
-           variant: int = 0, out_cpad: Optional[int] = None, split_k_3x3: bool = False) -> Act:
+           variant: int = 0, out_cpad: Optional[int] = None, split_k_3x3: bool = False,
+           px_scale: Optional[torch.Tensor] = None, head2: Optional[Head2] = None) -> Optional[Act]:
     dt = xa.dtype
     H, W = xa.H * a_up, xa.W * a_up
     if xb is not None:
@@ -252,13 +260,21 @@
         Ho = (H + 2 * p.pad - p.kh) // p.stride + 1
         Wo = (W + 2 * p.pad - p.kw) // p.stride + 1
         oH, oW = Ho, Wo
-    if out is None:
+    fused = (px_scale is not None or head2 is not None) and not variant and out is None and out2 is None
+    if fused:
+        assert px_scale is None or head2 is None
+        fused = _fused_ok(p, xa, xb, residual, mul, in_scale, px_scale, head2, out_dtype or dt, a_up)
+    if px_scale is not None and not fused:
+        xa = pixel_scale(xa, px_scale)
+    if head2 is not None:
+        head2.out = None
+    if out is None and not (fused and head2 is not None):
         out = Act.new(xa.N, oH, oW, p.cout, out_dtype or dt, xa.t.device, cpad=out_cpad,
                       zero=None if out_cpad is None else out_cpad != p.cout)
-    assert (out.N, out.H, out.W) == (xa.N, oH, oW), ((out.N, out.H, out.W), (xa.N, oH, oW))
+    assert out is None or (out.N, out.H, out.W) == (xa.N, oH, oW), ((out.N, out.H, out.W), (xa.N, oH, oW))
     assert xa.C <= p.ca and (xb is None or xb.C <= p.cb)
     d = L.Conv2dDesc()
-    d.dtype, d.out_dtype = hdtype(dt), hdtype(out.dtype)
+    d.dtype, d.out_dtype = hdtype(dt), hdtype(out.dtype if out is not None else (out_dtype or dt))
     d.N, d.H, d.W, d.Ho, d.Wo = xa.N, H, W, Ho, Wo
     d.KH, d.KW, d.stride, d.pad = p.kh, p.kw, p.stride, p.pad
     d.srcA, d.a_cstride, d.a_coff, d.Ca, d.a_up = xa, xa.cstride, xa.coff, p.ca, a_up
@@ -272,7 +288,14 @@
         d.residual, d.r_cstride, d.r_coff = residual, residual.cstride, residual.coff
     if mul is not None:
         d.mul, d.m_cstride, d.m_coff = mul, mul.cstride, mul.coff
-    d.out, d.o_cstride, d.o_coff = out, out.cstride, out.coff
+    if out is not None:
+        d.out, d.o_cstride, d.o_coff = out, out.cstride, out.coff
+    else:
+        d.o_cstride, d.o_coff = p.cout, 0
+        head2.out = torch.empty(xa.N * oH * oW, 2, dtype=torch.float32, device=xa.t.device)
+        d.head2_w, d.head2_b, d.head2_out = head2.w, head2.b, head2.out
+    if fused and px_scale is not None:
+        d.px_scale = px_scale
     if out2 is not None:
         assert out2.dtype == dt
         d.out2, d.o2_cstride, d.o2_coff = out2, out2.cstride, out2.coff
@@ -288,7 +311,7 @@
             d.workspace, d.workspace_bytes = ws, nbytes
     if RECORD is not None:
         dc = d.copy()
-        keep = [t for t in (xa, xb, out, residual, mul, out2, ws) if t is not None]
+        keep = [t for t in (xa, xb, out, residual, mul, out2, ws, px_scale) if t is not None]
         flops = 2.0 * d.N * d.Ho * d.Wo * p.gemm_cols * p.kh * p.kw * (xa.C + (xb.C if xb is not None else 0))
         RECORD.append((dc, keep, p, flops))
     gate = GATE
@@ -304,6 +327,43 @@
     return out
 
 
+def _fused_ok(p, xa, xb, residual, mul, in_scale, px_scale, head2, out_dtype, a_up) -> bool:
+    if xa.dtype != torch.bfloat16 or out_dtype != torch.bfloat16 or xb is not None or mul is not None or \
+            in_scale is not None or a_up != 1:
+        return False
+    if px_scale is not None:
+        assert px_scale.dtype == torch.float32 and px_scale.is_contiguous() and px_scale.numel() == xa.N * xa.H * xa.W
+    if head2 is not None:
+        if p.convT or residual is None:
+            return False
+        assert head2.w.dtype == torch.float32 and head2.w.is_contiguous() and tuple(head2.w.shape) == (2, p.cout)
+        assert head2.b.dtype == torch.float32 and head2.b.numel() == 2
+    d = L.Conv2dDesc()
+    d.dtype = d.out_dtype = L.HISEG_BF16
+    d.N, d.H, d.W = xa.N, xa.H, xa.W
+    if p.convT:
+        d.Ho, d.Wo = xa.H, xa.W
+    else:
+        d.Ho = (xa.H + 2 * p.pad - p.kh) // p.stride + 1
+        d.Wo = (xa.W + 2 * p.pad - p.kw) // p.stride + 1
+    d.KH, d.KW, d.stride, d.pad = p.kh, p.kw, p.stride, p.pad
+    d.srcA, d.a_cstride, d.a_coff, d.Ca, d.a_up = xa, xa.cstride, xa.coff, p.ca, 1
+    d.weight, d.Cout, d.Cout_pad, d.K_pad = p.weight, p.gemm_cols, p.cout_pad, p.k_pad
+    d.scale, d.shift, d.act, d.act_beta = p.scale, p.shift, int(p.act), L.act_beta(p.act)
+    d.o_cstride, d.o_coff = p.cout, 0
+    d.convT = int(p.convT)
+    if p.weight_frag is not None:
+        d.weight_frag = p.weight_frag
+    if residual is not None:
+        d.residual, d.r_cstride, d.r_coff = residual, residual.cstride, residual.coff
+    if px_scale is not None:
+        d.px_scale = px_scale
+        d.out = xa
+    if head2 is not None:
+        d.head2_w, d.head2_b, d.head2_out = head2.w, head2.b, head2.w
+    return bool(L.lib().hiseg_conv2d_fused_ok(ctypes.byref(d)))
+
+
 def _launch_conv(d, p, xa, xb, variant=0):
     if PROBE is not None:
         key = PROBE.select(d)
@@ -336,6 +396,24 @@
     L.check(L.lib().hiseg_attn_spatial_fwd(hdtype(x.dtype), x.ptr(), x.N, x.H, x.W, x.C, w7.data_ptr(), k,
                                            stats.data_ptr(), att.data_ptr(), out.ptr(), L.stream_ptr()),
             "attn_spatial")
+    return out
+
+
+def attn_map(x: Act, w7: torch.Tensor) -> torch.Tensor:
+    assert x.coff == 0 and x.cstride == x.C
+    P = x.N * x.H * x.W
+    stats = torch.empty(P * 2, dtype=torch.float32, device=x.t.device)
+    att = torch.empty(P, dtype=torch.float32, device=x.t.device)
+    L.check(L.lib().hiseg_attn_map_fwd(hdtype(x.dtype), x.ptr(), x.N, x.H, x.W, x.C, w7.data_ptr(), w7.shape[-1],
+                                       stats.data_ptr(), att.data_ptr(), L.stream_ptr()), "attn_map")
+    return att
+
+
+def pixel_scale(x: Act, att: torch.Tensor) -> Act:
+    assert x.coff == 0 and x.cstride == x.C and att.dtype == torch.float32 and att.numel() == x.N * x.H * x.W
+    out = Act.new(x.N, x.H, x.W, x.C, x.dtype, x.t.device, zero=False)
+    L.check(L.lib().hiseg_pixel_scale_fwd(hdtype(x.dtype), x.ptr(), x.N * x.H * x.W, x.C, att.data_ptr(), out.ptr(),
+                                          L.stream_ptr()), "pixel_scale")
     return out
 
 
@@ -406,13 +484,21 @@
     return out
 
 
-def hier_combine(low: torch.Tensor, N: int, h: int, w: int, tfeat: Act, ut_w, ut_scale, ut_shift, ut_act, u1_w, u1_b,
-                 t_w, t_b, want_aux: bool, per_sample: bool = False):
-    assert tfeat.coff == 0 and tfeat.cstride == tfeat.C and (tfeat.H, tfeat.W) == (2 * h, 2 * w)
+def hier_combine(low: torch.Tensor, N: int, h: int, w: int, tfeat: Optional[Act], ut_w, ut_scale, ut_shift, ut_act,
+                 u1_w, u1_b, t_w, t_b, want_aux: bool, per_sample: bool = False, tn2: Optional[torch.Tensor] = None):
     dev = low.device
     logits = torch.empty(N, 3, 2 * h, 2 * w, dtype=torch.float32, device=dev)
     bgfg = torch.empty(N, 2, 2 * h, 2 * w, dtype=torch.float32, device=dev) if want_aux else None
     tn = torch.empty(N, 2, 2 * h, 2 * w, dtype=torch.float32, device=dev) if want_aux else None
+    if tn2 is not None:
+        assert tn2.dtype == torch.float32 and tn2.is_contiguous() and tn2.numel() == N * 4 * h * w * 2
+        L.check(L.lib().hiseg_hier_combine_tn_fwd(low.data_ptr(), N, h, w, tn2.data_ptr(), ut_w.data_ptr(),
+                                                  ut_scale.data_ptr(), ut_shift.data_ptr(), int(ut_act),
+                                                  L.act_beta(ut_act), int(per_sample), u1_w.data_ptr(), u1_b.data_ptr(),
+                                                  logits.data_ptr(), _ptr(bgfg), _ptr(tn), L.stream_ptr()),
+                "hier_combine_tn")
+        return logits, bgfg, tn
+    assert tfeat.coff == 0 and tfeat.cstride == tfeat.C and (tfeat.H, tfeat.W) == (2 * h, 2 * w)
     L.check(L.lib().hiseg_hier_combine_fwd(hdtype(tfeat.dtype), low.data_ptr(), N, h, w, tfeat.ptr(), tfeat.C,
                                            ut_w.data_ptr(), ut_scale.data_ptr(), ut_shift.data_ptr(), int(ut_act),
                                            L.act_beta(ut_act), int(per_sample), u1_w.data_ptr(), u1_b.data_ptr(), t_w.data_ptr(), t_b.data_ptr(),
diff --git a/include/hiseg.h b/include/hiseg.h
--- a/include/hiseg.h
+++ b/include/hiseg.h
@@ -62,8 +62,11 @@
   float* stats_partial;
   float* bnb_partial; const void* bnb_z; int bnb_z_cstride, bnb_z_coff;
   const float* bnb_scale; const float* bnb_shift; const float* bnb_mean; const float* bnb_invstd; int bnb_act;
+  const float* px_scale;
+  const float* head2_w; const float* head2_b; float* head2_out;
 } hiseg_conv2d_desc;
 int hiseg_conv2d_fwd(const hiseg_conv2d_desc* d, hiseg_stream_t stream);
+int hiseg_conv2d_fused_ok(const hiseg_conv2d_desc* d);
 int hiseg_struct_sizes(long long* out, int n);
 long long hiseg_conv2d_workspace_bytes(const hiseg_conv2d_desc* d);
 int hiseg_conv2d_stats_tiles(const hiseg_conv2d_desc* d);
@@ -74,6 +77,10 @@
 
 int hiseg_attn_spatial_fwd(int dtype, const void* x, int N, int H, int W, int C, const float* w7,
                            int k, float* stats, float* att, void* out, hiseg_stream_t stream);
+int hiseg_attn_map_fwd(int dtype, const void* x, int N, int H, int W, int C, const float* w7,
+                       int k, float* stats, float* att, hiseg_stream_t stream);
+int hiseg_pixel_scale_fwd(int dtype, const void* x, long long P, int C, const float* att, void* out,
+                          hiseg_stream_t stream);
 
 int hiseg_gap_splits(int HW);
 int hiseg_se_gate_fwd(int dtype, const void* x, int N, int HW, int C, const float* w1,
@@ -105,6 +112,10 @@
                            int ut_act, float ut_beta, int ut_per_sample, const float* u1_w,
                            const float* u1_b, const float* t_w, const float* t_b, float* logits,
                            float* bgfg, float* tn, hiseg_stream_t stream);
+int hiseg_hier_combine_tn_fwd(const float* low, int N, int h, int w, const float* tn2, const float* ut_w,
+                              const float* ut_scale, const float* ut_shift, int ut_act, float ut_beta,
+                              int ut_per_sample, const float* u1_w, const float* u1_b, float* logits,
+                              float* bgfg, float* tn, hiseg_stream_t stream);
 int hiseg_ubf_ln_tables(const float* low, int N, int h, int w, const float* ut_w, const float* ut_b,
                         const float* gamma, const float* beta, float eps, int fold_bias, float* mean,
                         float* invstd, float* scale, float* shift, hiseg_stream_t stream);
```

Result: faster. 16340 ROI-masks/s, median of 6 (+1.5%).
